# yijingru/KG_Instance_Segmentation

Measured on AMD Instinct MI355X. Metric: imgs/s (train fwd+bwd) at 512x512, higher is better.
Workload: dtype forward: f32-tolerance, hi + lo f16 planes (22 significant bits), 3 MFMA products / backward: f16 single planes, 1 MFMA product; f16 MFMA, fp32 accumulate; 1 GPU; KGnet train step fwd(dec+seg)+4xDetectionLossAll+SEG_loss+bwd+Adam, batch 8/GPU 3x512x512, 300 boxes/img, full HIP path; precision_policy=fp32, global_batch=8, parallelism=dp1, loss_readback=every step (train.py:156), grad_overflow=False

## Files before the change

### include/kgnet_hip.h

```cpp
#ifndef KGNET_HIP_H
#define KGNET_HIP_H
#ifdef __cplusplus
extern "C" {
#endif

typedef struct kg_planes {
    int a_planes, a_pstride;
    int b_planes, b_pstride;
    int c_planes, c_pstride;
    int y_planes, y_pstride;
    int w_planes;
    int reserved_;
    const float* scale;
    const float* oscale;
} kg_planes_t;

int kg_rows_format(void);

const char* kg_last_error(void);
const char* kg_last_kernel(void);
int kg_version(void);
int kg_device_arch(char* out, int cap);
int kg_tr_probe(void* out_u16x256, void* stream);
int kg_f64_probe(const double* a, const double* b, double* out5n, int n, void* stream);

int kg_conv2d_igemm(const void* x, const void* w, const float* bias, void* y, float* y_f32, const void* res,
                    const void* mask, const int* rowdesc, int M, int H, int W, int OH, int OW, int cin_pad, int ldx,
                    int Cout, int ldy, int ldres, int ldmask, int K, int KH, int KW, int stride, int pad, int dil,
                    int mode, int relu, int f32_C, int tile, const kg_planes_t* planes, void* stream);
int kg_conv2d_halo(const void* x, const void* w, const float* bias, void* y, float* y_f32, const void* res,
                   const void* mask, int N, int H, int W, int cin_pad, int ldx, int Cout, int ldy, int ldres, int ldmask,
                   int K, int KS, int flip, int relu, int f32_C, int wc, const int* tiletab, int ntiles, int total_rows,
                   const kg_planes_t* planes, void* stream);
int kg_conv2d_halo_heads2(const void* x, const void* w, const float* bias64, const int* vmap, float* kp, float* sh, float* md,
                          int N, int H, int W, int C, int ldx, int K, int kp_sigmoid, const kg_planes_t* planes, void* stream);
int kg_conv3x3_c64(const void* x, const void* w, const float* bias, void* y, const void* res, const void* mask, int N, int H, int W,
                   int ldx, int Cout, int ldy, int ldres, int ldmask, int K, int flip, int relu, const int* tiletab16, int ntiles,
                   void* stream);
int kg_conv7_narrow(const void* x, const void* w, void* y, const void* mask, int N, int H, int W, int ldx, int chan_lo, int chan_slot, int Cout, int ldy,
                    int ldmask, int K, int flip, void* stream);
int kg_conv3x3_ws(const void* x, const void* w, const float* bias, void* y, int N, int H, int W, int ldx, int ldy, int K, int relu,
                  const int* tiletab8, int ntiles, const kg_planes_t* planes, void* stream);
int kg_conv1x1(const void* x, const void* w, const float* bias, void* y, const void* res, const void* mask, long M, int K,
               int wK, int ldx, int Cout, int ldy, int ldres, int ldmask, int relu, void* stream);
int kg_pack_weight(const float* w, void* dst, int Cout, int Cin, int KH, int KW, int K, int cin_pad, int row0, int c0,
                   int transposed, int x_planes, int w_planes, void* stream);
int kg_pack_weight_rows(const float* w, void* dst, int Cout, int Cin, int KH, int KW, int K, int cin_pad, const int* rowmap,
                        int c0, int x_planes, int w_planes, int tap_stride, void* stream);
int kg_pack_weight_narrow(const float* w, void* dst, int Cout, int Cin, int KH, int KW, int K, int row0, int c0, int tap_stride, int tap_pitch,
                          void* stream);
int kg_pack_weight_batch(const void* jobs, int njobs, int total_blocks, void* stream);
int kg_im2col_small(const void* x, void* out, int N, int H, int W, int OH, int OW, int KH, int KW, int stride, int pad, int cin,
                    int ldx, int Kpad, void* stream);
int kg_conv2d_wgrad(const void* x, const void* dy, float* dwp, const int* rowdesc, int M, int H, int W, int OH, int OW,
                    int ldx, int lddy, int Cin, int Cout, int cin_lim, int cout_lim, int KH, int KW, int stride, int pad,
                    int dil, int mode, int nsplit, long split_stride, const kg_planes_t* planes, void* stream);
int kg_conv2d_wgrad_halo(const void* x, const void* dy, float* dwp, int N, int H, int W, int ldx, int lddy, int Cin, int Cout,
                         int cin_lim, int cout_lim, int KS, int nsplit, long split_stride, const int* tiletab16, int ntiles,
                         float* dbp, const kg_planes_t* planes, void* stream);
int kg_bias_grad_final(const float* part, float* db, int nsplit, int C, int accumulate, void* stream);
int kg_wgrad_reduce(const float* part, float* grad_oihw, int Cout, int Cin, int KH, int KW, int nsplit, long split_stride,
                    int accumulate, void* stream);
int kg_wgrad_reduce_multi(const float* part, float* const* grads_oihw, const int* counts, int ngrads, int Cin, int KH, int KW,
                          int nsplit, long split_stride, int accumulate, void* stream);
int kg_wgrad_reduce_bias(const float* part, float* const* grads_oihw, const int* counts, int ngrads, int Cin, int KH, int KW,
                         int nsplit, long split_stride, int accumulate, const float* bias_part, float* db, int bias_C, void* stream);
int kg_wgrad_reduce_defer(int on);
int kg_wgrad_reduce_pending(void);
int kg_wgrad_reduce_flush(void* stream);
int kg_bias_grad(const void* dy, float* db, float* scratch, int scratch_floats, int M, int C, int ld, int accumulate,
                 void* stream);
int kg_set_wgrad_tr(int use_transpose_read);

int kg_img_pack(const float* img_nchw, void* out_rows8, int ldout, int N, int C, int H, int W, const kg_planes_t* planes, void* stream);
int kg_bn_stats_train(const void* x, int ldx, int M, int C, const float* gamma, const float* beta, float* running_mean,
                      float* running_var, float momentum, float eps, float* mean_out, float* invstd_out, float* scale,
                      float* shift, float* scratch, int scratch_floats, const kg_planes_t* planes, void* stream);
int kg_conv_stats_begin(float* part, long cap_floats);
int kg_conv_stats_end(int* nb);
int kg_bn_finalize_train(const float* part, int nb, int M, int C, const float* gamma, const float* beta, float* running_mean,
                         float* running_var, float momentum, float eps, float* mean_out, float* invstd_out, float* scale,
                         float* shift, void* stream);
int kg_bn_scale_shift_eval(int C, const float* gamma, const float* beta, const float* running_mean,
                           const float* running_var, float eps, float* scale, float* shift, void* stream);
int kg_bn_apply(const void* x, int ldx, const float* scale, const float* shift, const void* res, int ldres, void* y,
                int ldy, int M, int C, int relu, const kg_planes_t* planes, void* stream);
int kg_bn_bwd(const void* x, int ldx, const void* dy, int lddy, const float* gamma, const float* mean,
              const float* invstd, float* dgamma, float* dbeta, int accumulate, void* dx, int lddx, int M, int C,
              float* scratch, int scratch_floats, const float* parts, int nb_parts, const float* parts_scale,
              const kg_planes_t* planes, void* stream);
int kg_conv_bstats_begin(float* part, long cap_floats, const void* x, int ldx, int x_planes, int x_pstride, const float* mean,
                         const float* invstd);
int kg_maxpool3s2_fwd(const void* x, int ldx, void* y, int ldy, void* argmax_u8, int N, int H, int W, int C, const kg_planes_t* planes, void* stream);
int kg_maxpool3s2_bwd(const void* x, int ldx, const void* dy, int lddy, void* dx, int lddx, const void* argmax_u8, int N, int H, int W, int C,
                      const kg_planes_t* planes, void* stream);
int kg_bilinear_fwd(const void* x, int ldx, void* y, int ldy, int N, int IH, int IW, int OH, int OW, int C,
                    const int* boxdesc, const int* row2box, long total_out_rows, const kg_planes_t* planes, void* stream);
int kg_bilinear_bwd(const void* dy, int lddy, void* dx, int lddx, int N, int IH, int IW, int OH, int OW, int C,
                    const int* boxdesc, const int* row2box, long total_in_rows, const void* mask, int ldmask,
                    const kg_planes_t* planes, void* stream);
int kg_add_rows(const void* a, int lda, const void* b, int ldb, const void* mask, int ldm, void* y, int ldy, long M,
                int C, const float* scale, const float* scale2, const kg_planes_t* planes, void* stream);
int kg_sigmoid_inplace(float* x, long n, void* stream);
int kg_grad_pack(const float* g_nchw, const float* prob, void* out_rows, int N, int C, int H, int W, int ld, int cpad,
                 const kg_planes_t* planes, void* stream);
int kg_grad_pack3(const float* g0_nchw, const float* g1_nchw, const float* g2_nchw, const float* prob0, void* out_rows, int N, int C0, int C1, int C2,
                  int H, int W, int ld, int pad0, int pad1, int pad2, const kg_planes_t* planes, void* stream);

int kg_detection_loss_fwd(const float* kp, const float* sh, const float* md, const float* gt, int N, int H, int W,
                          float kp_radius, const float* den_override, float* scratch, int scratch_floats, float* out8,
                          void* stream);
int kg_detection_loss_bwd(const float* kp, const float* sh, const float* md, const float* gt, int N, int H, int W,
                          float kp_radius, const float* fin8, const float* grad_out, float* g_kp, float* g_sh,
                          float* g_md, void* stream);
int kg_seg_loss(const float* prob, const void* tgt_u8, const int* patches, const void* pairs, int npatches, float* part,
                float* out1, const float* grad_out, float* gprob, void* stream);

int kg_postproc_timing_begin(void);
int kg_postproc_timing_end(float* ms4);
long kg_postproc_workspace_bytes(int H, int W, int peak_cap, int skel_cap);
int kg_postproc_scale(const float* kp, const float* soff, const float* mid, int H, int W, double thresh, void* ws,
                      long ws_bytes, int peak_cap, int skel_cap, double* skel, int* nskel, double* heat_out,
                      double* blur_out, int* peaks_out, double* peak_conf_out, int* npeaks_out, void* stream);
int kg_skeleton_boxes(const double* skel, const int* nskel, int skel_cap, double scale, int do_refine, double* boxes,
                      int* nbox, int box_cap, void* stream);
int kg_nms(const double* boxes, const int* nbox, int box_cap, double thresh, void* ws, long ws_bytes, double* out,
           int* nkeep, void* stream);

long kg_postproc_batch_workspace_bytes(int N, int H, int W, int peak_cap, int skel_cap);
int kg_postproc_batch(const float* kp, const float* soff, const float* mid, int N, int H, int W, double thresh, void* ws,
                      long ws_bytes, int peak_cap, int skel_cap, double* skel, int* nskel, void* stream);
int kg_skeleton_boxes_batch(int N, int nscales, const double* const* skel, const int* const* nskel, const int* skel_cap,
                            const double* scale, int do_refine, double* boxes, int* nbox, int box_cap, void* stream);
long kg_nms_batch_workspace_bytes(int N, int box_cap);
int kg_nms_batch(int N, const double* boxes, const int* nbox, int box_cap, double thresh, void* ws, long ws_bytes, double* out,
                 int* nkeep, void* stream);

int kg_gt_maps(const float* kps, int n, int H, int W, float* out, void* stream);

int kg_sp_image(const void* imgs, int N, int H, int W, float* out, void* stream);
int kg_sp_warp_masks(const void* imgs, const int* inst_img, int ntot, int H, int W, void* out, int* box, void* stream);
int kg_sp_boxes(const void* imgs, int N, const int* box, int ntot, int kp_radius, int* counts, float* gtb, float* kp, int* keep,
                void* stream);

int kg_adam_step(const void* jobs, int njobs, int total_blocks, float beta1, float beta2, float eps, float step_size, float bc2_sqrt,
                 float weight_decay, void* stream);

int kg_host_crop_masks(const float* const* masks, const int* work, int nwork, int H, int W, unsigned char* out);
int kg_crop_masks(const void* masks, const int* work, int nwork, int H, int W, void* out, void* stream);
int kg_host_tile_table(const int* h, const int* w, const long* row0, int nb, int th, int tw, int* out, int cap);
int kg_host_bin_csr(const int* tab, int nb, int BS, int BY, int BX, int nbins, int* bin_start, int* bin_boxes, int cap);
int kg_host_match_boxes(const float* pb, int P, const float* gb, int G, int gstride, float thresh, int* pairs, int cap, int* count);

int kg_mask_areas(const void* masks, int n, long ld, int* area, void* stream);
int kg_mask_inter_pairs(const void* a, const void* b, const int* pairs, int npairs, long ld, int* inter, void* stream);

long kg_mask_bits_ld(int H, int W);
int kg_mask_pack_bits(const void* masks, int src_is_f32, int n, int H, int W, void* words, long ld_words, void* stream);
int kg_mask_unpack_bits(const void* words, long ld_words, int n, int H, int W, void* out, int out_is_u8, void* stream);
int kg_bitmask_areas(const void* words, int n, long ld_words, int* area, void* stream);
int kg_bitmask_inter_pairs(const void* a, int na, const void* b, int nb, const int* pairs, int npairs, long ld_words, int* inter,
                           void* stream);

int kg_seg_build_rows(const int* boxtab8, int nb, int* rowdesc, int* row2box, int* srcrow, void* stream);
int kg_seg_build_rows_levels(int nlev, const int* const* boxtab8, const int* nb, int* const* rowdesc, int* const* row2box, int* const* srcrow,
                             void* stream);
int kg_rows_gather(const void* src, int ldsrc, const int* srcrow, void* dst, int lddst, long nrows, int C, void* stream);
int kg_rows_gather_planes(const void* src, int ldsrc, int src_pstride, const int* srcrow, void* dst, int lddst, int dst_pstride, long nrows, int C,
                          int P, void* stream);
int kg_seg_conv3_c1(const void* x, int ldx, int C, const float* w, const float* bias, const int* rowdesc, long M, float* y,
                    const kg_planes_t* planes, void* stream);
int kg_f32_to_bf16_rows(const float* acc, void* out, int C, long rows, int ldout, const void* addto, int ldadd,
                        void* stream);
int kg_rows_gather_f32(const float* src, int ldsrc, const int* srcrow, void* dst, int lddst, long nrows, int C,
                       const kg_planes_t* planes, void* stream);
int kg_planes_to_f32(const void* x, int ldx, float* out, int ldout, long rows, int C, const kg_planes_t* planes, void* stream);
int kg_f32_to_planes(const float* acc, int ldacc, void* out, int ldout, const void* addto, int ldadd, long rows, int C,
                     const kg_planes_t* planes, void* stream);
int kg_crop_grad_reduce(const void* ga, int lda, const void* gb, int ldb, long rows_a, const int* boxtab, const int* bin_start,
                        const int* bin_boxes, int bin_size, int N, int H, int W, int C, float* out, void* out_rows, int ldout,
                        const kg_planes_t* planes, void* stream);


int kg_mask_paste(const float* flat, const int* dets, int nd, int input_h, int input_w, int image_h, int image_w,
                  float seg_thresh, void* out, int out_is_u8, void* stream);
int kg_mask_paste_bits(const float* flat, const int* dets, int nd, int input_h, int input_w, int image_h, int image_w,
                       float seg_thresh, void* words, long ld_words, void* stream);

int kg_grad_scale(const void* const* ptrs, const void* const* probs, const long* counts, int n, int target_log2, void* scratch, float* out, void* stream);
int kg_scale_tensors(const void* jobs, int njobs, int total_blocks, int* nonfinite, void* stream);
int kg_rows_rescale(void* g, int ld, long M, int C, int target_log2, const float* cum_in, float* cum_out, float* r_out, void* scratch,
                    const kg_planes_t* planes, void* stream);
int kg_rows_scale(void* g, int ld, long M, int C, const float* r, const float* r2, const kg_planes_t* planes, void* stream);
int kg_rows_scale_multi(const long* desc, int n, const float* r, const float* r2, void* stream);

#ifdef __cplusplus
}
#endif
#endif
```

### kg_instance_segmentation_amd/_lib.py

```python
import ctypes
import os

_HERE = os.path.dirname(os.path.abspath(__file__))
LIB_PATH = os.environ.get("KG_LIB_PATH") or os.path.join(_HERE, "libkgnet_hip.so")
LIB_F16_PATH = os.environ.get("KG_LIB_F16_PATH") or os.path.join(os.path.dirname(LIB_PATH), "libkgnet_hip_f16.so")

c_int, c_long, c_float, c_double, c_void_p = ctypes.c_int, ctypes.c_long, ctypes.c_float, ctypes.c_double, ctypes.c_void_p
P = c_void_p

_SIGS = {
    "kg_version": [],
    "kg_rows_format": [],
    "kg_grad_scale": [P, P, P, c_int, c_int, P, P, P],
    "kg_scale_tensors": [P, c_int, c_int, P, P],
    "kg_rows_rescale": [P, c_int, c_long, c_int, c_int, P, P, P, P, P, P],
    "kg_rows_scale": [P, c_int, c_long, c_int, P, P, P, P],
    "kg_rows_scale_multi": [P, c_int, P, P, P],
    "kg_device_arch": [ctypes.c_char_p, c_int],
    "kg_tr_probe": [P, P],
    "kg_conv2d_igemm": [P, P, P, P, P, P, P, P] + [c_int] * 21 + [P, P],
    "kg_conv2d_halo": [P, P, P, P, P, P, P] + [c_int] * 15 + [P, c_int, c_int, P, P],
    "kg_conv1x1": [P, P, P, P, P, P, c_long] + [c_int] * 8 + [P],
    "kg_conv3x3_c64": [P, P, P, P, P, P] + [c_int] * 11 + [P, c_int, P],
    "kg_conv3x3_ws": [P, P, P, P] + [c_int] * 7 + [P, c_int, P, P],
    "kg_pack_weight": [P, P] + [c_int] * 11 + [P],
    "kg_pack_weight_rows": [P, P] + [c_int] * 6 + [P, c_int, c_int, c_int, c_int, P],
    "kg_pack_weight_batch": [P, c_int, c_int, P],
    "kg_pack_weight_narrow": [P, P] + [c_int] * 9 + [P],
    "kg_conv7_narrow": [P, P, P, P] + [c_int] * 11 + [P],
    "kg_im2col_small": [P, P] + [c_int] * 12 + [P],
    "kg_conv2d_halo_heads2": [P, P, P, P, P, P, P] + [c_int] * 7 + [P, P],
    "kg_set_wgrad_tr": [c_int],
    "kg_conv2d_wgrad": [P, P, P, P] + [c_int] * 18 + [c_long, P, P],
    "kg_conv2d_wgrad_halo": [P, P, P] + [c_int] * 11 + [c_long, P, c_int, P, P, P],
    "kg_bias_grad_final": [P, P, c_int, c_int, c_int, P],
    "kg_wgrad_reduce": [P, P, c_int, c_int, c_int, c_int, c_int, c_long, c_int, P],
    "kg_wgrad_reduce_multi": [P, P, P, c_int, c_int, c_int, c_int, c_int, c_long, c_int, P],
    "kg_wgrad_reduce_bias": [P, P, P, c_int, c_int, c_int, c_int, c_int, c_long, c_int, P, P, c_int, P],
    "kg_wgrad_reduce_defer": [c_int],
    "kg_wgrad_reduce_pending": [],
    "kg_wgrad_reduce_flush": [P],
    "kg_bias_grad": [P, P, P, c_int, c_int, c_int, c_int, c_int, P],
    "kg_img_pack": [P, P, c_int, c_int, c_int, c_int, c_int, P, P],
    "kg_bn_stats_train": [P, c_int, c_int, c_int, P, P, P, P, c_float, c_float, P, P, P, P, P, c_int, P, P],
    "kg_bn_scale_shift_eval": [c_int, P, P, P, P, c_float, P, P, P],
    "kg_conv_stats_begin": [P, c_long],
    "kg_conv_bstats_begin": [P, c_long, P, c_int, c_int, c_int, P, P],
    "kg_conv_stats_end": [P],
    "kg_bn_finalize_train": [P, c_int, c_int, c_int, P, P, P, P, c_float, c_float, P, P, P, P, P],
    "kg_bn_apply": [P, c_int, P, P, P, c_int, P, c_int, c_int, c_int, c_int, P, P],
    "kg_bn_bwd": [P, c_int, P, c_int, P, P, P, P, P, c_int, P, c_int, c_int, c_int, P, c_int, P, c_int, P, P, P],
    "kg_maxpool3s2_fwd": [P, c_int, P, c_int, P, c_int, c_int, c_int, c_int, P, P],
    "kg_maxpool3s2_bwd": [P, c_int, P, c_int, P, c_int, P, c_int, c_int, c_int, c_int, P, P],
    "kg_bilinear_fwd": [P, c_int, P, c_int, c_int, c_int, c_int, c_int, c_int, c_int, P, P, c_long, P, P],
    "kg_bilinear_bwd": [P, c_int, P, c_int, c_int, c_int, c_int, c_int, c_int, c_int, P, P, c_long, P, c_int, P, P],
    "kg_add_rows": [P, c_int, P, c_int, P, c_int, P, c_int, c_long, c_int, P, P, P, P],
    "kg_detection_loss_fwd": [P, P, P, P, c_int, c_int, c_int, c_float, P, P, c_int, P, P],
    "kg_detection_loss_bwd": [P, P, P, P, c_int, c_int, c_int, c_float, P, P, P, P, P, P],
    "kg_seg_loss": [P, P, P, P, c_int, P, P, P, P, P],
    "kg_sigmoid_inplace": [P, c_long, P],
    "kg_grad_pack": [P, P, P, c_int, c_int, c_int, c_int, c_int, c_int, P, P],
    "kg_grad_pack3": [P, P, P, P, P] + [c_int] * 10 + [P, P],
    "kg_postproc_workspace_bytes": [c_int, c_int, c_int, c_int],
    "kg_postproc_scale": [P, P, P, c_int, c_int, c_double, P, c_long, c_int, c_int, P, P, P, P, P, P, P, P],
    "kg_postproc_timing_begin": [],
    "kg_postproc_timing_end": [P],
    "kg_skeleton_boxes": [P, P, c_int, c_double, c_int, P, P, c_int, P],
    "kg_nms": [P, P, c_int, c_double, P, c_long, P, P, P],
    "kg_postproc_batch_workspace_bytes": [c_int, c_int, c_int, c_int, c_int],
    "kg_postproc_batch": [P, P, P, c_int, c_int, c_int, c_double, P, c_long, c_int, c_int, P, P, P],
    "kg_skeleton_boxes_batch": [c_int, c_int, P, P, P, P, c_int, P, P, c_int, P],
    "kg_nms_batch_workspace_bytes": [c_int, c_int],
    "kg_nms_batch": [c_int, P, P, c_int, c_double, P, c_long, P, P, P],
    "kg_gt_maps": [P, c_int, c_int, c_int, P, P],
    "kg_sp_image": [P, c_int, c_int, c_int, P, P],
    "kg_sp_warp_masks": [P, P, c_int, c_int, c_int, P, P, P],
    "kg_sp_boxes": [P, c_int, P, c_int, c_int, P, P, P, P, P],
    "kg_adam_step": [P, c_int, c_int, c_float, c_float, c_float, c_float, c_float, c_float, P],
    "kg_host_crop_masks": [P, P, c_int, c_int, c_int, P],
    "kg_crop_masks": [P, P, c_int, c_int, c_int, P, P],
    "kg_host_match_boxes": [P, c_int, P, c_int, c_int, c_float, P, c_int, P],
    "kg_host_tile_table": [P, P, P, c_int, c_int, c_int, P, c_int],
    "kg_host_bin_csr": [P, c_int, c_int, c_int, c_int, c_int, P, P, c_int],
    "kg_mask_areas": [P, c_int, c_long, P, P],
    "kg_mask_inter_pairs": [P, P, P, c_int, c_long, P, P],
    "kg_mask_bits_ld": [c_int, c_int],
    "kg_mask_pack_bits": [P, c_int, c_int, c_int, c_int, P, c_long, P],
    "kg_mask_unpack_bits": [P, c_long, c_int, c_int, c_int, P, c_int, P],
    "kg_bitmask_areas": [P, c_int, c_long, P, P],
    "kg_bitmask_inter_pairs": [P, c_int, P, c_int, P, c_int, c_long, P, P],
    "kg_f64_probe": [P, P, P, c_int, P],
    "kg_seg_build_rows": [P, c_int, P, P, P, P],
    "kg_seg_build_rows_levels": [c_int, P, P, P, P, P, P],
    "kg_rows_gather": [P, c_int, P, P, c_int, c_long, c_int, P],
    "kg_rows_gather_planes": [P, c_int, c_int, P, P, c_int, c_int, c_long, c_int, c_int, P],
    "kg_seg_conv3_c1": [P, c_int, c_int, P, P, P, c_long, P, P, P],
    "kg_f32_to_bf16_rows": [P, P, c_int, c_long, c_int, P, c_int, P],
    "kg_rows_gather_f32": [P, c_int, P, P, c_int, c_long, c_int, P, P],
    "kg_planes_to_f32": [P, c_int, P, c_int, c_long, c_int, P, P],
    "kg_f32_to_planes": [P, c_int, P, c_int, P, c_int, c_long, c_int, P, P],
    "kg_mask_paste": [P, P, c_int, c_int, c_int, c_int, c_int, c_float, P, c_int, P],
    "kg_mask_paste_bits": [P, P, c_int, c_int, c_int, c_int, c_int, c_float, P, c_long, P],
    "kg_crop_grad_reduce": [P, c_int, P, c_int, c_long, P, P, P, c_int, c_int, c_int, c_int, c_int, P, P, c_int, P, P],
}
_RESTYPE = {"kg_postproc_workspace_bytes": c_long, "kg_postproc_batch_workspace_bytes": c_long, "kg_nms_batch_workspace_bytes": c_long,
            "kg_mask_bits_ld": c_long}
SYMBOLS = tuple(_SIGS) + ("kg_last_error", "kg_last_kernel")

_lib = None
_lib_f16 = None


class KGLibraryError(RuntimeError):
    pass


def _open(path, must_have_all):
    if not os.path.exists(path):
        raise KGLibraryError(
            f"{path} is missing: build it with `python -m kg_instance_segmentation_amd.build` "
            "(hipcc --offload-arch=gfx950).  There is no CPU fallback for the KGnet hot path.")
    lib = ctypes.CDLL(path)
    lib.kg_last_error.restype = ctypes.c_char_p
    lib.kg_last_error.argtypes = []
    lib.kg_last_kernel.restype = ctypes.c_char_p
    lib.kg_last_kernel.argtypes = []
    for name, args in _SIGS.items():
        if must_have_all:
            fn = getattr(lib, name)
        else:
            fn = getattr(lib, name, None)
            if fn is None:
                continue
        fn.argtypes = args
        fn.restype = _RESTYPE.get(name, c_int)
    return lib


def load(fmt=0):
    global _lib, _lib_f16
    if fmt:
        if _lib_f16 is None:
            lib = _open(LIB_F16_PATH, False)
            if lib.kg_rows_format() != 1:
                raise KGLibraryError(f"{LIB_F16_PATH} is not the half-precision build (kg_rows_format() != 1)")
            _lib_f16 = lib
        return _lib_f16
    if _lib is None:
        _lib = _open(LIB_PATH, True)
    return _lib


def call(name, *args, fmt=0):
    lib = load(fmt)
    rc = getattr(lib, name)(*args)
    if rc != 0:
        raise KGLibraryError(f"{name} failed ({rc}): {lib.kg_last_error().decode()}")


def last_kernel(fmt=0):
    return load(fmt).kg_last_kernel().decode()


_RAW_STREAM = None


def stream_ptr():
    global _RAW_STREAM
    import torch
    if _RAW_STREAM is None:
        _RAW_STREAM = getattr(torch._C, "_cuda_getCurrentRawStream", False)
    if _RAW_STREAM:
        return c_void_p(_RAW_STREAM(torch.cuda.current_device()))
    return c_void_p(torch.cuda.current_stream().cuda_stream)


def ptr(t):
    return None if t is None else c_void_p(t.data_ptr())
```

### kg_instance_segmentation_amd/csrc/api.hip

```cpp
#include "kg_common.h"
#include <stdarg.h>

static thread_local char g_err[512] = "";

void kg_set_error(const char* fmt, ...) {
    va_list ap;
    va_start(ap, fmt);
    vsnprintf(g_err, sizeof(g_err), fmt, ap);
    va_end(ap);
}

extern "C" const char* kg_last_error(void) { return g_err; }

static thread_local const char* g_kernel = "";
void kg_note_kernel(const char* name) { g_kernel = name; }
extern "C" const char* kg_last_kernel(void) { return g_kernel; }
extern "C" int kg_version(void) { return 101; }
extern "C" int kg_rows_format(void) { return KG_ROWS_FORMAT; }

extern "C" int kg_device_arch(char* out, int cap) {
    hipDeviceProp_t p;
    int dev = 0;
    KG_HIP(hipGetDevice(&dev));
    KG_HIP(hipGetDeviceProperties(&p, dev));
    snprintf(out, cap, "%s", p.gcnArchName);
    return KG_OK;
}

typedef __attribute__((address_space(3))) bf16x4 lds_bf16x4;
__global__ void tr_probe_kernel(unsigned short* out) {
    __shared__ __attribute__((aligned(16))) unsigned short lds[64 * 4];
    const int l = threadIdx.x;
    for (int j = 0; j < 4; ++j) lds[l * 4 + j] = (unsigned short)(l * 4 + j);
    __syncthreads();
    bf16x4 v = KG_DS_READ_TR16((lds_bf16x4*)(&lds[l * 4]));
    *reinterpret_cast<uint2*>(&out[l * 4]) = __builtin_bit_cast(uint2, v);
}
extern "C" int kg_tr_probe(void* out, void* stream) {
    hipLaunchKernelGGL(tr_probe_kernel, dim3(1), dim3(64), 0, (hipStream_t)stream, (unsigned short*)out);
    KG_CHECK_LAUNCH("tr_probe");
    return KG_OK;
}

static thread_local KgConvStats g_conv_stats = {nullptr, 0, 0, {nullptr, 0, 0, 0, nullptr, nullptr}};
KgConvStats& kg_conv_stats() { return g_conv_stats; }
extern "C" int kg_conv_stats_begin(float* part, long cap_floats) {
    KG_CHECK_ARG(part && cap_floats > 0, "kg_conv_stats_begin: bad buffer");
    g_conv_stats = KgConvStats{part, cap_floats, 0, {nullptr, 0, 0, 0, nullptr, nullptr}};
    return KG_OK;
}
extern "C" int kg_conv_bstats_begin(float* part, long cap_floats, const void* x, int ldx, int x_planes, int x_pstride, const float* mean,
                                    const float* invstd) {
    KG_CHECK_ARG(part && cap_floats > 0 && x && mean && invstd && ldx % 8 == 0 && x_planes >= 1 && x_planes <= 3 && x_pstride % 8 == 0,
                 "kg_conv_bstats_begin: bad arguments");
    g_conv_stats = KgConvStats{part, cap_floats, 0, {(const unsigned short*)x, ldx, x_planes, x_pstride, mean, invstd}};
    return KG_OK;
}
extern "C" int kg_conv_stats_end(int* nb) {
    KG_CHECK_ARG(nb, "kg_conv_stats_end: null pointer");
    *nb = g_conv_stats.nb;
    g_conv_stats = KgConvStats{nullptr, 0, 0, {nullptr, 0, 0, 0, nullptr, nullptr}};
    return KG_OK;
}

extern "C" int kg_host_tile_table(const int* h, const int* w, const long* row0, int nb, int th, int tw, int* out, int cap) {
    if (!h || !w || !row0 || !out || nb < 0 || th < 1 || tw < 1) return -1;
    int n = 0;
    for (int b = 0; b < nb; ++b) {
        const int ny = (h[b] + th - 1) / th, nx = (w[b] + tw - 1) / tw;
        for (int ty = 0; ty < ny; ++ty)
            for (int tx = 0; tx < nx; ++tx) {
                if (n >= cap) return -1;
                int* o = out + 4 * (long)n++;
                o[0] = (int)row0[b]; o[1] = (h[b] << 16) | w[b]; o[2] = ((ty * th) << 16) | (tx * tw); o[3] = 0;
            }
    }
    return n;
}
extern "C" int kg_host_bin_csr(const int* tab, int nb, int BS, int BY, int BX, int nbins, int* bin_start, int* bin_boxes, int cap) {
    if (!tab || !bin_start || (!bin_boxes && cap > 0) || nb < 0 || BS < 1 || nbins < 0) return -1;
    for (int i = 0; i <= nbins; ++i) bin_start[i] = 0;
    long total = 0;
    for (int b = 0; b < nb; ++b) {
        const int* t = tab + 8 * (long)b;
        const int by0 = t[1] / BS, bx0 = t[2] / BS, by1 = (t[1] + t[3] - 1) / BS, bx1 = (t[2] + t[4] - 1) / BS;
        for (int by = by0; by <= by1; ++by)
            for (int bx = bx0; bx <= bx1; ++bx) {
                const long bin = ((long)t[0] * BY + by) * BX + bx;
                if (bin < 0 || bin >= nbins) return -1;
                ++bin_start[bin + 1]; ++total;
            }
    }
    if (total > cap) return -1;
    for (int i = 0; i < nbins; ++i) bin_start[i + 1] += bin_start[i];
    for (int b = 0; b < nb; ++b) {
        const int* t = tab + 8 * (long)b;
        const int by0 = t[1] / BS, bx0 = t[2] / BS, by1 = (t[1] + t[3] - 1) / BS, bx1 = (t[2] + t[4] - 1) / BS;
        for (int by = by0; by <= by1; ++by)
            for (int bx = bx0; bx <= bx1; ++bx) {
                const long bin = ((long)t[0] * BY + by) * BX + bx;
                bin_boxes[bin_start[bin]++] = b;
            }
    }
    for (int i = nbins; i > 0; --i) bin_start[i] = bin_start[i - 1];
    bin_start[0] = 0;
    return (int)total;
}

extern "C" int kg_host_match_boxes(const float* pb, int P, const float* gb, int G, int gstride, float thresh, int* pairs, int cap, int* count) {
#pragma clang fp contract(off)
    KG_CHECK_ARG(pb && gb && pairs && count && P >= 0 && G >= 0 && gstride >= 4 && cap >= 0, "kg_host_match_boxes: bad arguments");
    float* soa = (float*)malloc(sizeof(float) * 4 * (size_t)(G > 0 ? G : 1));
    unsigned char* ov = (unsigned char*)malloc((size_t)(G > 0 ? G : 1));
    if (!soa || !ov) { free(soa); free(ov); kg_set_error("kg_host_match_boxes: out of host memory"); return KG_ERR_ARG; }
    float *b0 = soa, *b1 = soa + G, *b2 = soa + 2 * (size_t)G, *b3 = soa + 3 * (size_t)G;
    for (int g = 0; g < G; ++g) {
        const float* b = gb + (long)g * gstride;
        b0[g] = b[0]; b1[g] = b[1]; b2[g] = b[2]; b3[g] = b[3];
    }
    const bool prefilter = thresh > 0.f;
    int n = 0, rc = KG_OK;
    for (int j = 0; j < P && rc == KG_OK; ++j) {
        const float a0 = pb[4 * j], a1 = pb[4 * j + 1], a2 = pb[4 * j + 2], a3 = pb[4 * j + 3];
        const float area_a = (a2 - a0) * (a3 - a1);
        for (int g = 0; g < G; ++g) {
            const float ih = (a2 < b2[g] ? a2 : b2[g]) - (a0 > b0[g] ? a0 : b0[g]);
            const float iw = (a3 < b3[g] ? a3 : b3[g]) - (a1 > b1[g] ? a1 : b1[g]);
            ov[g] = (unsigned char)((ih > 0.f) & (iw > 0.f));
        }
        for (int g = 0; g < G; ++g) {
            if (prefilter && !ov[g]) continue;
            const float area_b = (b2[g] - b0[g]) * (b3[g] - b1[g]);
            float ih = (a2 < b2[g] ? a2 : b2[g]) - (a0 > b0[g] ? a0 : b0[g]);
            float iw = (a3 < b3[g] ? a3 : b3[g]) - (a1 > b1[g] ? a1 : b1[g]);
            if (!(ih > 0.f)) ih = 0.f;
            if (!(iw > 0.f)) iw = 0.f;
            const float inter = ih * iw;
            const float uni = area_a + area_b - inter;
            const float iou = uni <= 2.f ? 0.f : inter / uni;
            if (iou >= thresh) {
                if (n >= cap) { kg_set_error("kg_host_match_boxes: more than %d matches", cap); rc = KG_ERR_ARG; break; }
                pairs[2 * n] = j; pairs[2 * n + 1] = g; ++n;
            }
        }
    }
    free(soa); free(ov);
    if (rc != KG_OK) return rc;
    *count = n;
    return KG_OK;
}

#include <math.h>
extern "C" int kg_host_crop_masks(const float* const* masks, const int* work, int nwork, int H, int W, unsigned char* out) {
    KG_CHECK_ARG(masks && work && out && nwork >= 0 && H > 0 && W > 0, "kg_host_crop_masks: bad arguments");
    for (int k = 0; k < nwork; ++k) {
        const int* w = work + 9 * k;
        const float* m = masks[w[0]] + (long)w[1] * H * W;
        int ya = w[2], yb = w[3], xa = w[4], xb = w[5];
        const int h1 = w[6], w1 = w[7];
        unsigned char* o = out + w[8];
        if (yb > H) yb = H;
        if (xb > W) xb = W;
        const int h0 = yb - ya, w0 = xb - xa;
        if (h0 <= 0 || w0 <= 0) { kg_set_error("kg_host_crop_masks: empty ground-truth crop (work item %d)", k); return KG_ERR_ARG; }
        const double fy = (double)h0 / h1, fx = (double)w0 / w1;
        for (int y = 0; y < h1; ++y) {
            int sy = y;
            if (h0 != h1 || w0 != w1) { sy = (int)floor(y * fy); if (sy > h0 - 1) sy = h0 - 1; }
            const float* row = m + (long)(ya + sy) * W + xa;
            for (int x = 0; x < w1; ++x) {
                int sx = x;
                if (h0 != h1 || w0 != w1) { sx = (int)floor(x * fx); if (sx > w0 - 1) sx = w0 - 1; }
                o[y * w1 + x] = (unsigned char)row[sx];
            }
        }
    }
    return KG_OK;
}
```

### kg_instance_segmentation_amd/csrc/kg_common.h

```cpp
#pragma once
#include <hip/hip_runtime.h>
#include <stdint.h>
#include <stdio.h>
#include <string.h>

typedef uint16_t bf16_t;
#ifdef KG_F16
typedef _Float16 kg_h16;
#define KG_MFMA16(a, b, c) __builtin_amdgcn_mfma_f32_16x16x32_f16(a, b, c, 0, 0, 0)
#define KG_WSCALE 4096.0f
#define KG_OSCALE (1.0f / 4096.0f)
#define KG_ACC(v) ((v) * KG_OSCALE)
#define KG_BIAS_ACC(b) ((b) * KG_WSCALE)
#define KG_ROWS_FORMAT 1
typedef __attribute__((ext_vector_type(4))) __fp16 kg_fp16x4_;
#define KG_DS_READ_TR16(p) __builtin_bit_cast(bf16x4_fwd_, __builtin_amdgcn_ds_read_tr16_b64_v4f16((__attribute__((address_space(3))) kg_fp16x4_*)(p)))
#else
typedef __bf16 kg_h16;
#define KG_MFMA16(a, b, c) __builtin_amdgcn_mfma_f32_16x16x32_bf16(a, b, c, 0, 0, 0)
#define KG_WSCALE 1.0f
#define KG_OSCALE 1.0f
#define KG_ACC(v) (v)
#define KG_BIAS_ACC(b) (b)
#define KG_ROWS_FORMAT 0
#define KG_DS_READ_TR16(p) __builtin_amdgcn_ds_read_tr16_b64_v4bf16(p)
#endif
typedef __attribute__((ext_vector_type(8))) kg_h16 bf16x8;
typedef __attribute__((ext_vector_type(4))) kg_h16 bf16x4;
typedef bf16x4 bf16x4_fwd_;
typedef __attribute__((ext_vector_type(4))) float f32x4;

#define KG_OK 0
#define KG_ERR_ARG 1
#define KG_ERR_HIP 2

void kg_set_error(const char* fmt, ...);
void kg_note_kernel(const char* name);
#define KG_KNAME(buf, fmt, ...) static char buf[96] = ""; if (!buf[0]) snprintf(buf, sizeof(buf), fmt, __VA_ARGS__)

struct KgPerDevice {
    bool done[32] = {};
    bool first() {
        int d = 0;
        if (hipGetDevice(&d) != hipSuccess || d < 0 || d >= 32) return true;
        if (done[d]) return false;
        done[d] = true;
        return true;
    }
};

#define KG_CHECK_ARG(cond, ...)                 \
    do {                                        \
        if (!(cond)) {                          \
            kg_set_error(__VA_ARGS__);          \
            return KG_ERR_ARG;                  \
        }                                       \
    } while (0)

#define KG_CHECK_LAUNCH(name)                                                        \
    do {                                                                             \
        hipError_t e_ = hipGetLastError();                                           \
        if (e_ != hipSuccess) {                                                      \
            kg_set_error("%s: launch failed: %s", name, hipGetErrorString(e_));      \
            return KG_ERR_HIP;                                                       \
        }                                                                            \
    } while (0)

#define KG_HIP(call)                                                                  \
    do {                                                                              \
        hipError_t e_ = (call);                                                       \
        if (e_ != hipSuccess) {                                                       \
            kg_set_error("%s failed: %s", #call, hipGetErrorString(e_));              \
            return KG_ERR_HIP;                                                        \
        }                                                                             \
    } while (0)

#ifdef KG_F16
__device__ __forceinline__ float bf2f(bf16_t v) { return (float)__builtin_bit_cast(_Float16, v); }
#else
__device__ __forceinline__ float bf2f(bf16_t v) { return __uint_as_float(((uint32_t)v) << 16); }
#endif
typedef __attribute__((ext_vector_type(2))) kg_h16 kg_bf16x2_t;
__device__ __forceinline__ bf16_t f2bf(float f) { return __builtin_bit_cast(bf16_t, (kg_h16)f); }
__device__ __forceinline__ uint32_t pack2bf(float lo, float hi) {
    const kg_bf16x2_t v = {(kg_h16)lo, (kg_h16)hi};
    return __builtin_bit_cast(uint32_t, v);
}

template <int OFF>
__device__ __forceinline__ void lds_rd128(bf16x8& d, unsigned addr) {
    asm volatile("ds_read_b128 %0, %1 offset:%2" : "=v"(d) : "v"(addr), "n"(OFF));
}
template <int N>
__device__ __forceinline__ void lgkm_wait(bf16x8 (&a)[4], bf16x8 (&b)[4]) {
    asm volatile("s_waitcnt lgkmcnt(%8)" : "+v"(a[0]), "+v"(a[1]), "+v"(a[2]), "+v"(a[3]), "+v"(b[0]), "+v"(b[1]), "+v"(b[2]), "+v"(b[3]) : "n"(N));
}

__device__ __forceinline__ float kg_relu(float v) { return v < 0.f ? 0.f : v; }

__device__ __forceinline__ unsigned lds_addr(const void* p) {
    return (unsigned)(unsigned long long)(__attribute__((address_space(3))) const unsigned char*)p;
}

static inline int kg_cdiv(long a, long b) { return (int)((a + b - 1) / b); }

__device__ __forceinline__ void kg_divmod(long i, int d, long* q, int* r) {
    if ((d & (d - 1)) == 0) {
        const int sh = __builtin_ctz((unsigned)d);
        *q = i >> sh; *r = (int)(i & (long)(d - 1));
    } else if ((unsigned long)i <= 0xffffffffUL) {
        const unsigned qi = (unsigned)i / (unsigned)d;
        *q = (long)qi; *r = (int)((unsigned)i - qi * (unsigned)d);
    } else {
        const long qq = i / d;
        *q = qq; *r = (int)(i - qq * d);
    }
}

struct KgBStat { const unsigned short* x; int ldx, P, ps; const float* mean; const float* invstd; };
struct KgConvStats { float* part; long cap_floats; int nb; KgBStat bs; };
KgConvStats& kg_conv_stats();
static inline float* kg_conv_stats_claim(int tiles, int Cout) {
    KgConvStats& st = kg_conv_stats();
    if (!st.part || st.nb != 0 || (long)tiles * Cout * 2 > st.cap_floats) return nullptr;
    st.nb = tiles;
    return st.part;
}

struct kg_planes_t {
    int a_planes, a_pstride;
    int b_planes, b_pstride;
    int c_planes, c_pstride;
    int y_planes, y_pstride;
    int w_planes;
    int reserved_;
    const float* scale;
    const float* oscale;
};
static inline kg_planes_t kg_planes_or_default(const kg_planes_t* p) {
    kg_planes_t d = {1, 0, 1, 0, 1, 0, 1, 0, 1, 0, nullptr, nullptr};
    if (p) {
        d = *p;
        if (d.a_planes < 1) d.a_planes = 1;
        if (d.b_planes < 1) d.b_planes = 1;
        if (d.c_planes < 1) d.c_planes = 1;
        if (d.y_planes < 1) d.y_planes = 1;
        if (d.w_planes < 1) d.w_planes = 1;
    }
    return d;
}
static inline bool kg_planes_ok(const kg_planes_t& d) {
    return d.a_planes <= 3 && d.b_planes <= 3 && d.c_planes <= 3 && d.y_planes <= 3 && d.w_planes <= 3 &&
           d.a_pstride % 8 == 0 && d.b_pstride % 8 == 0 && d.c_pstride % 8 == 0 && d.y_pstride % 8 == 0;
}

static inline int kg_plane_pairs(int xP, int wP, int* xi, int* wj) {
    const int T = xP > wP ? xP : wP;
    int n = 0;
    for (int sum = T - 1; sum >= 0; --sum)
        for (int j = wP - 1; j >= 0; --j) {
            const int i = sum - j;
            if (i >= 0 && i < xP) { xi[n] = i; wj[n] = j; ++n; }
        }
    return n;
}
struct KMap {
    int n;
    int total;
    int xps;
    int unit;
    unsigned xtab;
    __device__ __forceinline__ int xoff(int q) const {
        if (total == n) return q * unit;
        const int v = q / n;
        return (int)((xtab >> (2 * v)) & 3u) * xps + (q - v * n) * unit;
    }
};
static inline int kg_kmap_segs(int xP, int wP, int* s) {
    int xi[6], wj[6];
    (void)s;
    return kg_plane_pairs(xP, wP, xi, wj);
}
static inline KMap kg_make_kmap(int C, int unit, int xP, int xps, int wP) {
    int xi[6], wj[6];
    const int nv = kg_plane_pairs(xP, wP, xi, wj);
    KMap m;
    m.n = C / unit; m.unit = unit; m.xps = xps; m.total = nv * m.n; m.xtab = 0;
    for (int v = 0; v < nv; ++v) m.xtab |= (unsigned)xi[v] << (2 * v);
    return m;
}

struct WgPairs {
    int n;
    int xoff[6], doff[6];
};
static inline WgPairs kg_make_wgpairs(int xP, int xps, int dP, int dps) {
    WgPairs w;
    int xi[6], dj[6];
    w.n = kg_plane_pairs(xP < 1 ? 1 : xP, dP < 1 ? 1 : dP, xi, dj);
    for (int k = 0; k < 6; ++k) { w.xoff[k] = k < w.n ? xi[k] * xps : 0; w.doff[k] = k < w.n ? dj[k] * dps : 0; }
    return w;
}

template <int NV>
__device__ __forceinline__ void kg_store_planes(bf16_t* yp, int P, int ps, float (&v)[NV], bool vec) {
    static_assert(NV % 8 == 0, "stores are 16-byte chunks");
    for (int p = 0; p < P; ++p) {
        bf16_t h[NV];
#pragma unroll
        for (int e = 0; e < NV; ++e) h[e] = f2bf(v[e]);
        if (vec) {
#pragma unroll
            for (int q = 0; q < NV / 8; ++q) {
                uint4 o;
                o.x = (uint32_t)h[q * 8 + 0] | ((uint32_t)h[q * 8 + 1] << 16); o.y = (uint32_t)h[q * 8 + 2] | ((uint32_t)h[q * 8 + 3] << 16);
                o.z = (uint32_t)h[q * 8 + 4] | ((uint32_t)h[q * 8 + 5] << 16); o.w = (uint32_t)h[q * 8 + 6] | ((uint32_t)h[q * 8 + 7] << 16);
                *reinterpret_cast<uint4*>(yp + (long)p * ps + q * 8) = o;
            }
        } else {
#pragma unroll
            for (int e = 0; e < NV; ++e) yp[(long)p * ps + e] = h[e];
        }
        if (p + 1 < P) {
#pragma unroll
            for (int e = 0; e < NV; ++e) v[e] -= bf2f(h[e]);
        }
    }
}
template <int NV>
__device__ __forceinline__ void kg_store_planes_n(bf16_t* yp, int P, int ps, float (&v)[NV], int nvalid) {
    for (int p = 0; p < P; ++p) {
#pragma unroll
        for (int e = 0; e < NV; ++e) {
            const bf16_t h = f2bf(v[e]);
            if (e < nvalid) yp[(long)p * ps + e] = h;
            v[e] -= bf2f(h);
        }
    }
}
__device__ __forceinline__ void kg_load_planes8(const bf16_t* xp, int P, int ps, float (&v)[8]) {
    uint4 q = *reinterpret_cast<const uint4*>(xp + (long)(P - 1) * ps);
    const bf16_t* s = reinterpret_cast<const bf16_t*>(&q);
#pragma unroll
    for (int e = 0; e < 8; ++e) v[e] = bf2f(s[e]);
    for (int p = P - 2; p >= 0; --p) {
        q = *reinterpret_cast<const uint4*>(xp + (long)p * ps);
#pragma unroll
        for (int e = 0; e < 8; ++e) v[e] += bf2f(s[e]);
    }
}
__device__ __forceinline__ float kg_load_planes1(const bf16_t* xp, int P, int ps) {
    float v = bf2f(xp[(long)(P - 1) * ps]);
    for (int p = P - 2; p >= 0; --p) v += bf2f(xp[(long)p * ps]);
    return v;
}
```

### kg_instance_segmentation_amd/csrc/loss.hip

```cpp
#include "kg_common.h"

__constant__ int KG_MID_FROM[20] = {0, 0, 0, 0, 1, 1, 1, 2, 2, 3, 1, 2, 3, 4, 2, 3, 4, 3, 4, 4};

__device__ __forceinline__ float wave_sum(float v) {
#pragma unroll
    for (int o = 32; o > 0; o >>= 1) v += __shfl_down(v, o, 64);
    return v;
}

__device__ __forceinline__ float bce_elem(float p, float t) {
    float l1 = log1pf(-p); l1 = l1 > -100.f ? l1 : -100.f;
    float l0 = logf(p); l0 = l0 > -100.f ? l0 : -100.f;
    return (t - 1.f) * l1 - t * l0;
}
__device__ __forceinline__ float bce_grad(float p, float t) {
    float d = (1.f - p) * p;
    d = d > 1e-12f ? d : 1e-12f;
    return (p - t) / d;
}

__global__ __launch_bounds__(256) void det_loss_fwd_kernel(const float* __restrict__ kp, const float* __restrict__ sh,
                                                           const float* __restrict__ md, const float* __restrict__ gt,
                                                           int N, long HW, float inv_r, float* __restrict__ part) {
    float s[5] = {0.f, 0.f, 0.f, 0.f, 0.f};
    const long total = (long)N * HW;
    for (long i = blockIdx.x * (long)blockDim.x + threadIdx.x; i < total; i += (long)gridDim.x * blockDim.x) {
        long n = i / HW, p = i - n * HW;
        const float* g = gt + n * 55 * HW + p;
        float gk[5];
#pragma unroll
        for (int c = 0; c < 5; ++c) {
            gk[c] = g[c * HW];
            s[0] += bce_elem(kp[(n * 5 + c) * HW + p], gk[c]);
        }
#pragma unroll
        for (int c = 0; c < 10; ++c) {
            float m = gk[c >> 1];
            s[1] += fabsf(sh[(n * 10 + c) * HW + p] - g[(5 + c) * HW]) * inv_r * m;
            s[2] += m;
        }
#pragma unroll
        for (int c = 0; c < 40; ++c) {
            float m = gk[KG_MID_FROM[c >> 1]];
            s[3] += fabsf(md[(n * 40 + c) * HW + p] - g[(15 + c) * HW]) * inv_r * m;
            s[4] += m;
        }
    }
    __shared__ float red[4][5];
    const int lane = threadIdx.x & 63, wave = threadIdx.x >> 6;
#pragma unroll
    for (int k = 0; k < 5; ++k) {
        float v = wave_sum(s[k]);
        if (lane == 0) red[wave][k] = v;
    }
    __syncthreads();
    if (threadIdx.x < 5) part[blockIdx.x * 5 + threadIdx.x] = red[0][threadIdx.x] + red[1][threadIdx.x] + red[2][threadIdx.x] + red[3][threadIdx.x];
}
__global__ void det_loss_final_kernel(const float* __restrict__ part, int nb, double numel,
                                      const float* __restrict__ den_override, float* __restrict__ out) {
    if (blockIdx.x != 0) return;
    double s[5] = {0, 0, 0, 0, 0};
    for (int b = threadIdx.x; b < nb; b += 64)
        for (int k = 0; k < 5; ++k) s[k] += (double)part[b * 5 + k];
#pragma unroll
    for (int k = 0; k < 5; ++k)
#pragma unroll
        for (int o = 32; o > 0; o >>= 1) s[k] += __shfl_down(s[k], o, 64);
    if (threadIdx.x != 0) return;
    double m2 = s[2], m4 = s[4], ne = numel;
    if (den_override) { m2 = den_override[0]; m4 = den_override[1]; ne = den_override[2]; }
    float lkp = (float)(s[0] / ne);
    float lsh = (float)s[1] / ((float)m2 + 1e-10f);
    float lmd = (float)s[3] / ((float)m4 + 1e-10f);
    out[0] = lkp + lsh + 0.25f * lmd; out[1] = lkp; out[2] = lsh; out[3] = lmd;
    out[4] = (float)(1.0 / ne); out[5] = 1.f / ((float)m2 + 1e-10f); out[6] = 1.f / ((float)m4 + 1e-10f);
    out[7] = (float)m2;
}
__global__ __launch_bounds__(256) void det_loss_bwd_kernel(const float* __restrict__ kp, const float* __restrict__ sh,
                                                           const float* __restrict__ md, const float* __restrict__ gt,
                                                           int N, long HW, float inv_r, const float* __restrict__ fin,
                                                           const float* __restrict__ gout, float* __restrict__ g_kp,
                                                           float* __restrict__ g_sh, float* __restrict__ g_md) {
    const float go = gout ? gout[0] : 1.f;
    const float a_kp = go * fin[4], a_sh = go * fin[5] * inv_r, a_md = go * 0.25f * fin[6] * inv_r;
    const long total = (long)N * HW;
    for (long i = blockIdx.x * (long)blockDim.x + threadIdx.x; i < total; i += (long)gridDim.x * blockDim.x) {
        long n = i / HW, p = i - n * HW;
        const float* g = gt + n * 55 * HW + p;
        float gk[5];
#pragma unroll
        for (int c = 0; c < 5; ++c) {
            gk[c] = g[c * HW];
            long o = (n * 5 + c) * HW + p;
            g_kp[o] = bce_grad(kp[o], gk[c]) * a_kp;
        }
#pragma unroll
        for (int c = 0; c < 10; ++c) {
            long o = (n * 10 + c) * HW + p;
            float d = sh[o] - g[(5 + c) * HW];
            float sg = d > 0.f ? 1.f : (d < 0.f ? -1.f : 0.f);
            g_sh[o] = sg * gk[c >> 1] * a_sh;
        }
#pragma unroll
        for (int c = 0; c < 40; ++c) {
            long o = (n * 40 + c) * HW + p;
            float d = md[o] - g[(15 + c) * HW];
            float sg = d > 0.f ? 1.f : (d < 0.f ? -1.f : 0.f);
            g_md[o] = sg * gk[KG_MID_FROM[c >> 1]] * a_md;
        }
    }
}

extern "C" int kg_detection_loss_fwd(const float* kp, const float* sh, const float* md, const float* gt, int N, int H,
                                     int W, float kp_radius, const float* den_override, float* scratch,
                                     int scratch_floats, float* out8, void* stream) {
    KG_CHECK_ARG(kp && sh && md && gt && scratch && out8, "kg_detection_loss_fwd: null pointer");
    long total = (long)N * H * W;
    int nb = (int)((total + 255) / 256);
    if (nb > 1024) nb = 1024;
    if (nb > scratch_floats / 5) nb = scratch_floats / 5;
    KG_CHECK_ARG(nb >= 1, "kg_detection_loss_fwd: scratch too small");
    hipStream_t st = (hipStream_t)stream;
    hipLaunchKernelGGL(det_loss_fwd_kernel, dim3(nb), dim3(256), 0, st, kp, sh, md, gt, N, (long)H * W, 1.f / kp_radius, scratch);
    hipLaunchKernelGGL(det_loss_final_kernel, dim3(1), dim3(64), 0, st, scratch, nb, (double)total * 5.0, den_override, out8);
    KG_CHECK_LAUNCH("detection_loss_fwd");
    return KG_OK;
}
extern "C" int kg_detection_loss_bwd(const float* kp, const float* sh, const float* md, const float* gt, int N, int H,
                                     int W, float kp_radius, const float* fin8, const float* grad_out, float* g_kp,
                                     float* g_sh, float* g_md, void* stream) {
    KG_CHECK_ARG(kp && sh && md && gt && fin8 && g_kp && g_sh && g_md, "kg_detection_loss_bwd: null pointer");
    long total = (long)N * H * W;
    int nb = (int)((total + 255) / 256);
    if (nb > 4096) nb = 4096;
    hipLaunchKernelGGL(det_loss_bwd_kernel, dim3(nb), dim3(256), 0, (hipStream_t)stream, kp, sh, md, gt, N, (long)H * W,
                       1.f / kp_radius, fin8, grad_out, g_kp, g_sh, g_md);
    KG_CHECK_LAUNCH("detection_loss_bwd");
    return KG_OK;
}

struct SegPatch { int prob_off, npix, pair0, npairs; };
struct SegPair { int tgt_off; float weight; };
__global__ __launch_bounds__(256) void seg_loss_kernel(const float* __restrict__ prob, const uint8_t* __restrict__ tgt,
                                                       const SegPatch* __restrict__ patches,
                                                       const SegPair* __restrict__ pairs, float* __restrict__ part,
                                                       const float* __restrict__ gout, float* __restrict__ gprob) {
    const SegPatch pa = patches[blockIdx.x];
    const float go = gout ? gout[0] : 1.f;
    float s = 0.f;
    for (int i = threadIdx.x; i < pa.npix; i += blockDim.x) {
        float p = prob[pa.prob_off + i], g = 0.f;
        for (int k = 0; k < pa.npairs; ++k) {
            SegPair pr = pairs[pa.pair0 + k];
            float t = (float)tgt[pr.tgt_off + i];
            s += pr.weight * bce_elem(p, t);
            g += pr.weight * bce_grad(p, t);
        }
        if (gprob) gprob[pa.prob_off + i] = g * go;
    }
    __shared__ float red[4];
    float v = wave_sum(s);
    if ((threadIdx.x & 63) == 0) red[threadIdx.x >> 6] = v;
    __syncthreads();
    if (threadIdx.x == 0 && part) part[blockIdx.x] = red[0] + red[1] + red[2] + red[3];
}
__global__ void sum_final_kernel(const float* __restrict__ part, int n, float* __restrict__ out) {
    if (blockIdx.x != 0) return;
    double s = 0.;
    for (int i = threadIdx.x; i < n; i += 64) s += (double)part[i];
#pragma unroll
    for (int o = 32; o > 0; o >>= 1) s += __shfl_down(s, o, 64);
    if (threadIdx.x == 0) out[0] = (float)s;
}
extern "C" int kg_seg_loss(const float* prob, const void* tgt, const int* patches, const void* pairs, int npatches,
                           float* part, float* out1, const float* grad_out, float* gprob, void* stream) {
    KG_CHECK_ARG(prob && tgt && patches && pairs && npatches > 0, "kg_seg_loss: bad args");
    hipStream_t st = (hipStream_t)stream;
    hipLaunchKernelGGL(seg_loss_kernel, dim3(npatches), dim3(256), 0, st, prob, (const uint8_t*)tgt,
                       (const SegPatch*)patches, (const SegPair*)pairs, part, grad_out, gprob);
    if (part && out1) hipLaunchKernelGGL(sum_final_kernel, dim3(1), dim3(64), 0, st, part, npatches, out1);
    KG_CHECK_LAUNCH("seg_loss");
    return KG_OK;
}

__global__ void sigmoid_inplace_kernel(float* __restrict__ x, long n) {
    for (long i = blockIdx.x * (long)blockDim.x + threadIdx.x; i < n; i += (long)gridDim.x * blockDim.x)
        x[i] = 1.f / (1.f + expf(-x[i]));
}
extern "C" int kg_sigmoid_inplace(float* x, long n, void* stream) {
    KG_CHECK_ARG(x, "kg_sigmoid_inplace: null pointer");
    if (n == 0) return KG_OK;
    int blocks = (int)((n + 255) / 256); if (blocks > 8192) blocks = 8192;
    hipLaunchKernelGGL(sigmoid_inplace_kernel, dim3(blocks), dim3(256), 0, (hipStream_t)stream, x, n);
    KG_CHECK_LAUNCH("sigmoid_inplace");
    return KG_OK;
}
__global__ void grad_pack_kernel(const float* __restrict__ g, const float* __restrict__ prob, bf16_t* __restrict__ out,
                                 int N, int C, long HW, int ld, int cpad, int P, int ps, const float* __restrict__ scale) {
    long total = (long)N * HW;
    const float S = scale ? *scale : 1.f;
    for (long i = blockIdx.x * (long)blockDim.x + threadIdx.x; i < total; i += (long)gridDim.x * blockDim.x) {
        long n = i / HW, p = i - n * HW;
        for (int c0 = 0; c0 < cpad; c0 += 8) {
            float v[8];
#pragma unroll
            for (int e = 0; e < 8; ++e) {
                int c = c0 + e;
                float t = 0.f;
                if (c < C) {
                    long o = (n * C + c) * HW + p;
                    t = g[o];
                    if (prob) { float q = prob[o]; t *= q * (1.f - q); }
                }
                v[e] = t * S;
            }
            kg_store_planes<8>(out + i * ld + c0, P, ps, v, true);
        }
    }
}
__global__ __launch_bounds__(256) void grad_pack_tr_kernel(const float* __restrict__ g, const float* __restrict__ prob, bf16_t* __restrict__ out,
                                                           long total, int C, long HW, int ld, int cpad, int P, int ps, const float* __restrict__ scale) {
    extern __shared__ float gp_tile[];
    const float S = scale ? *scale : 1.f;
    const int t = threadIdx.x, K = cpad >> 3;
    for (long i0 = (long)blockIdx.x * 256; i0 < total; i0 += (long)gridDim.x * 256) {
        if ((HW & 3) == 0) {
            const int cs = t >> 6, pq = (t & 63) * 4;
            const long i = i0 + pq;
            if (i < total) {
                const long n = i / HW, p = i - n * HW;
#pragma unroll 2
                for (int c = cs; c < C; c += 4) {
                    const long o = (n * C + c) * HW + p;
                    f32x4 v = *reinterpret_cast<const f32x4*>(g + o);
                    if (prob) {
                        const f32x4 q = *reinterpret_cast<const f32x4*>(prob + o);
                        v[0] *= q[0] * (1.f - q[0]); v[1] *= q[1] * (1.f - q[1]); v[2] *= q[2] * (1.f - q[2]); v[3] *= q[3] * (1.f - q[3]);
                    }
#pragma unroll
                    for (int e = 0; e < 4; ++e) gp_tile[c * 257 + pq + e] = v[e] * S;
                }
            }
        } else {
            const long i = i0 + t;
            if (i < total) {
                const long n = i / HW, p = i - n * HW;
                for (int c = 0; c < C; ++c) {
                    const long o = (n * C + c) * HW + p;
                    float v = g[o];
                    if (prob) { const float q = prob[o]; v *= q * (1.f - q); }
                    gp_tile[c * 257 + t] = v * S;
                }
            }
        }
        for (int c = C; c < cpad; ++c) gp_tile[c * 257 + t] = 0.f;
        __syncthreads();
        for (int q = t; q < 256 * K; q += 256) {
            const int px = q / K, k8 = q - px * K;
            if (i0 + px < total) {
                float v[8];
#pragma unroll
                for (int e = 0; e < 8; ++e) v[e] = gp_tile[(k8 * 8 + e) * 257 + px];
                kg_store_planes<8>(out + (i0 + px) * ld + k8 * 8, P, ps, v, true);
            }
        }
        __syncthreads();
    }
}
struct GradPack3 { const float* g[3]; const float* prob; int C[3]; int off[3]; int end[3]; };
__global__ __launch_bounds__(256) void grad_pack3_tr_kernel(const GradPack3 a, bf16_t* __restrict__ out, long total, long HW, int ld, int cpad, int P, int ps,
                                                            const float* __restrict__ scale) {
    extern __shared__ float gp_tile[];
    const float S = scale ? *scale : 1.f;
    const int t = threadIdx.x, K = cpad >> 3;
    for (long i0 = (long)blockIdx.x * 256; i0 < total; i0 += (long)gridDim.x * 256) {
#pragma unroll
        for (int s = 0; s < 3; ++s) {
            for (int c = a.off[s] + a.C[s]; c < a.end[s]; ++c) gp_tile[c * 257 + t] = 0.f;
            const float* __restrict__ g = a.g[s];
            const float* __restrict__ prob = s == 0 ? a.prob : nullptr;
            const int C = a.C[s], r0 = a.off[s];
            if ((HW & 3) == 0) {
                const int cs = t >> 6, pq = (t & 63) * 4;
                const long i = i0 + pq;
                if (i < total) {
                    const long n = i / HW, p = i - n * HW;
#pragma unroll 2
                    for (int c = cs; c < C; c += 4) {
                        const long o = (n * C + c) * HW + p;
                        f32x4 v = *reinterpret_cast<const f32x4*>(g + o);
                        if (prob) {
                            const f32x4 q = *reinterpret_cast<const f32x4*>(prob + o);
                            v[0] *= q[0] * (1.f - q[0]); v[1] *= q[1] * (1.f - q[1]); v[2] *= q[2] * (1.f - q[2]); v[3] *= q[3] * (1.f - q[3]);
                        }
#pragma unroll
                        for (int e = 0; e < 4; ++e) gp_tile[(r0 + c) * 257 + pq + e] = v[e] * S;
                    }
                }
            } else {
                const long i = i0 + t;
                if (i < total) {
                    const long n = i / HW, p = i - n * HW;
                    for (int c = 0; c < C; ++c) {
                        const long o = (n * C + c) * HW + p;
                        float v = g[o];
                        if (prob) { const float q = prob[o]; v *= q * (1.f - q); }
                        gp_tile[(r0 + c) * 257 + t] = v * S;
                    }
                }
            }
        }
        __syncthreads();
        for (int q = t; q < 256 * K; q += 256) {
            const int px = q / K, k8 = q - px * K;
            if (i0 + px < total) {
                float v[8];
#pragma unroll
                for (int e = 0; e < 8; ++e) v[e] = gp_tile[(k8 * 8 + e) * 257 + px];
                kg_store_planes<8>(out + (i0 + px) * ld + k8 * 8, P, ps, v, true);
            }
        }
        __syncthreads();
    }
}
extern "C" int kg_grad_pack3(const float* g0, const float* g1, const float* g2, const float* prob0, void* out, int N, int C0, int C1, int C2, int H, int W,
                             int ld, int pad0, int pad1, int pad2, const kg_planes_t* planes, void* stream) {
    const int cpad = pad0 + pad1 + pad2;
    KG_CHECK_ARG(g0 && g1 && g2 && out && ld % 8 == 0 && pad0 % 8 == 0 && pad1 % 8 == 0 && pad2 % 8 == 0 && pad0 >= C0 && pad1 >= C1 && pad2 >= C2 &&
                 cpad <= 64 && C0 > 0 && C1 > 0 && C2 > 0, "kg_grad_pack3: bad args");
    const kg_planes_t pp = kg_planes_or_default(planes);
    KG_CHECK_ARG(kg_planes_ok(pp), "kg_grad_pack3: bad kg_planes_t");
    long total = (long)N * H * W;
    if (total == 0) return KG_OK;
    int blocks = (int)((total + 255) / 256); if (blocks > 2048) blocks = 2048;
    static KgPerDevice attr_done;
    if (attr_done.first()) {
        KG_HIP(hipFuncSetAttribute((const void*)grad_pack3_tr_kernel, hipFuncAttributeMaxDynamicSharedMemorySize, 64 * 257 * 4));
    }
    GradPack3 a;
    a.g[0] = g0; a.g[1] = g1; a.g[2] = g2; a.prob = prob0;
    a.C[0] = C0; a.C[1] = C1; a.C[2] = C2; a.off[0] = 0; a.off[1] = pad0; a.off[2] = pad0 + pad1;
    a.end[0] = pad0; a.end[1] = pad0 + pad1; a.end[2] = cpad;
    hipLaunchKernelGGL(grad_pack3_tr_kernel, dim3(blocks), dim3(256), cpad * 257 * 4, (hipStream_t)stream, a, (bf16_t*)out, total, (long)H * W, ld, cpad,
                       pp.y_planes, pp.y_pstride, pp.scale);
    KG_CHECK_LAUNCH("grad_pack3_tr");
    return KG_OK;
}
extern "C" int kg_grad_pack(const float* g, const float* prob, void* out, int N, int C, int H, int W, int ld, int cpad,
                            const kg_planes_t* planes, void* stream) {
    KG_CHECK_ARG(g && out && cpad % 8 == 0 && ld % 8 == 0 && cpad >= C, "kg_grad_pack: bad args");
    const kg_planes_t pp = kg_planes_or_default(planes);
    KG_CHECK_ARG(kg_planes_ok(pp), "kg_grad_pack: bad kg_planes_t");
    long total = (long)N * H * W;
    int blocks = (int)((total + 255) / 256); if (blocks > 8192) blocks = 8192;
    if (cpad <= 64) {
        const int smem = cpad * 257 * 4;
        static KgPerDevice attr_done;
        if (attr_done.first()) {
            KG_HIP(hipFuncSetAttribute((const void*)grad_pack_tr_kernel, hipFuncAttributeMaxDynamicSharedMemorySize, 64 * 257 * 4));
        }
        if (blocks > 2048) blocks = 2048;
        hipLaunchKernelGGL(grad_pack_tr_kernel, dim3(blocks), dim3(256), smem, (hipStream_t)stream, g, prob, (bf16_t*)out, total, C, (long)H * W, ld, cpad,
                           pp.y_planes, pp.y_pstride, pp.scale);
        KG_CHECK_LAUNCH("grad_pack_tr");
        return KG_OK;
    }
    hipLaunchKernelGGL(grad_pack_kernel, dim3(blocks), dim3(256), 0, (hipStream_t)stream, g, prob, (bf16_t*)out, N, C,
                       (long)H * W, ld, cpad, pp.y_planes, pp.y_pstride, pp.scale);
    KG_CHECK_LAUNCH("grad_pack");
    return KG_OK;
}
```

### kg_instance_segmentation_amd/csrc/norm_pool.hip

```cpp
#include "kg_common.h"

struct RowsR { const bf16_t* p; int ld, P, ps; };
struct RowsW { bf16_t* p; int ld, P, ps; };
__device__ __forceinline__ void rd8(const RowsR& t, long r, int c, float (&v)[8]) { kg_load_planes8(t.p + r * t.ld + c, t.P, t.ps, v); }
__device__ __forceinline__ void wr8(const RowsW& t, long r, int c, float (&v)[8]) { kg_store_planes<8>(t.p + r * t.ld + c, t.P, t.ps, v, true); }
#define KG_PLANES(pl)                                                       \
    const kg_planes_t pp = kg_planes_or_default(pl);                        \
    KG_CHECK_ARG(kg_planes_ok(pp), "bad kg_planes_t (at most 3 planes, strides multiples of 8)")

__global__ void img_pack_kernel(const float* __restrict__ img, RowsW out, int N, int C, int HW) {
    long total = (long)N * HW;
    for (long i = blockIdx.x * (long)blockDim.x + threadIdx.x; i < total; i += (long)gridDim.x * blockDim.x) {
        long n = i / HW, p = i - n * HW;
        float v[8];
#pragma unroll
        for (int c = 0; c < 8; ++c) v[c] = c < C ? img[(n * C + c) * HW + p] : 0.f;
        wr8(out, i, 0, v);
    }
}
extern "C" int kg_img_pack(const float* img, void* out, int ldout, int N, int C, int H, int W, const kg_planes_t* planes, void* stream) {
    KG_CHECK_ARG(img && out && C <= 8 && ldout >= 8 && ldout % 8 == 0, "kg_img_pack: bad args");
    KG_PLANES(planes);
    long total = (long)N * H * W;
    int blocks = (int)((total + 255) / 256); if (blocks > 8192) blocks = 8192;
    hipLaunchKernelGGL(img_pack_kernel, dim3(blocks), dim3(256), 0, (hipStream_t)stream, img, RowsW{(bf16_t*)out, ldout, pp.y_planes, pp.y_pstride}, N, C, H * W);
    KG_CHECK_LAUNCH("img_pack");
    return KG_OK;
}

template <int MODE>
__global__ __launch_bounds__(256) void colreduce_kernel(const RowsR x, const RowsR dy,
                                                        const float* __restrict__ mean,
                                                        const float* __restrict__ invstd, float* __restrict__ part,
                                                        int M, int C, int rows_per_block) {
    __shared__ float red[32][8][16];
    const int cl = threadIdx.x & 7, rl = threadIdx.x >> 3;
    const int c0 = blockIdx.y * 64 + cl * 8;
    float s0[8], s1[8];
#pragma unroll
    for (int e = 0; e < 8; ++e) s0[e] = s1[e] = 0.f;
    if (c0 < C) {
        float mu[8], is[8];
        if (MODE == 1) {
#pragma unroll
            for (int e = 0; e < 8; ++e) { mu[e] = mean[c0 + e]; is[e] = invstd[c0 + e]; }
        }
        int r0 = blockIdx.x * rows_per_block, r1 = r0 + rows_per_block;
        if (r1 > M) r1 = M;
        for (int r = r0 + rl; r < r1; r += 32) {
            float xs[8];
            rd8(x, r, c0, xs);
            if (MODE == 0) {
#pragma unroll
                for (int e = 0; e < 8; ++e) { float f = xs[e]; s0[e] += f; s1[e] += f * f; }
            } else {
                float ds[8];
                rd8(dy, r, c0, ds);
#pragma unroll
                for (int e = 0; e < 8; ++e) {
                    float d = ds[e], xh = (xs[e] - mu[e]) * is[e];
                    s0[e] += d; s1[e] += d * xh;
                }
            }
        }
    }
#pragma unroll
    for (int e = 0; e < 8; ++e) { red[rl][cl][e] = s0[e]; red[rl][cl][8 + e] = s1[e]; }
    __syncthreads();
    if (threadIdx.x < 128) {
        const int c = threadIdx.x & 63, q = threadIdx.x >> 6;
        float t = 0.f;
        for (int k = 0; k < 32; ++k) t += red[k][c >> 3][q * 8 + (c & 7)];
        const int cg = blockIdx.y * 64 + c;
        if (cg < C) part[((long)blockIdx.x * C + cg) * 2 + q] = t;
    }
}

__device__ __forceinline__ double wave_sum_d(double v) {
#pragma unroll
    for (int o = 32; o > 0; o >>= 1) v += __shfl_down(v, o, 64);
    return __shfl(v, 0, 64);
}

__global__ void bn_finalize_train_kernel(const float* __restrict__ part, int nb, int C, long M,
                                         const float* __restrict__ gamma, const float* __restrict__ beta,
                                         float* __restrict__ running_mean, float* __restrict__ running_var,
                                         float momentum, float eps, float* __restrict__ mean_out,
                                         float* __restrict__ invstd_out, float* __restrict__ scale,
                                         float* __restrict__ shift) {
    const int c = blockIdx.x;
    double s = 0., ss = 0.;
    for (int b = threadIdx.x; b < nb; b += 64) { s += part[((long)b * C + c) * 2]; ss += part[((long)b * C + c) * 2 + 1]; }
    s = wave_sum_d(s); ss = wave_sum_d(ss);
    if (threadIdx.x != 0) return;
    double mu = s / (double)M;
    double var = ss / (double)M - mu * mu;
    if (var < 0.) var = 0.;
    float is = (float)(1.0 / sqrt(var + (double)eps));
    mean_out[c] = (float)mu; invstd_out[c] = is;
    float sc = gamma[c] * is;
    scale[c] = sc; shift[c] = beta[c] - (float)mu * sc;
    if (running_mean) {
        double unb = M > 1 ? var * (double)M / (double)(M - 1) : var;
        running_mean[c] = (1.f - momentum) * running_mean[c] + momentum * (float)mu;
        running_var[c] = (1.f - momentum) * running_var[c] + momentum * (float)unb;
    }
}
__global__ void bn_finalize_eval_kernel(int C, const float* __restrict__ gamma, const float* __restrict__ beta,
                                        const float* __restrict__ running_mean,
                                        const float* __restrict__ running_var, float eps,
                                        float* __restrict__ scale, float* __restrict__ shift) {
    int c = blockIdx.x * blockDim.x + threadIdx.x;
    if (c >= C) return;
    float is = 1.f / sqrtf(running_var[c] + eps);
    float sc = gamma[c] * is;
    scale[c] = sc; shift[c] = beta[c] - running_mean[c] * sc;
}
__global__ void bn_finalize_bwd_kernel(const float* __restrict__ part, int nb, int C, long M,
                                       const float* __restrict__ gamma, const float* __restrict__ invstd,
                                       float* __restrict__ dgamma, float* __restrict__ dbeta, int accumulate,
                                       float* __restrict__ coef, const float* __restrict__ rs) {
    const int c = blockIdx.x;
    double s = 0., sx = 0.;
    for (int b = threadIdx.x; b < nb; b += 64) { s += part[((long)b * C + c) * 2]; sx += part[((long)b * C + c) * 2 + 1]; }
    s = wave_sum_d(s); sx = wave_sum_d(sx);
    if (threadIdx.x != 0) return;
    if (rs) { s *= (double)*rs; sx *= (double)*rs; }
    float db = (float)s, dg = (float)sx;
    dgamma[c] = accumulate ? dgamma[c] + dg : dg;
    dbeta[c] = accumulate ? dbeta[c] + db : db;
    float a = gamma[c] * invstd[c];
    coef[c] = a; coef[C + c] = (float)(-(double)a * sx / (double)M); coef[2 * C + c] = (float)(-(double)a * s / (double)M);
}

static int reduce_geometry(int M, int C, int scratch_floats, int* nb, int* rpb) {
    int n = scratch_floats / (2 * C);
    if (n > 512) n = 512;
    int need = (M + 255) / 256;
    if (n > need) n = need;
    if (n < 1) return 0;
    *rpb = (M + n - 1) / n;
    *nb = (M + *rpb - 1) / *rpb;
    return 1;
}

extern "C" int kg_bn_stats_train(const void* x, int ldx, int M, int C, const float* gamma, const float* beta,
                                 float* running_mean, float* running_var, float momentum, float eps,
                                 float* mean_out, float* invstd_out, float* scale, float* shift, float* scratch,
                                 int scratch_floats, const kg_planes_t* planes, void* stream) {
    KG_PLANES(planes);
    KG_CHECK_ARG(x && gamma && beta && mean_out && invstd_out && scale && shift && scratch, "kg_bn_stats_train: null pointer");
    KG_CHECK_ARG(C % 8 == 0 && ldx % 8 == 0, "kg_bn_stats_train: C/ld must be multiples of 8");
    int nb, rpb;
    KG_CHECK_ARG(reduce_geometry(M, C, scratch_floats, &nb, &rpb), "kg_bn_stats_train: scratch too small");
    hipStream_t st = (hipStream_t)stream;
    hipLaunchKernelGGL(colreduce_kernel<0>, dim3(nb, (C + 63) / 64), dim3(256), 0, st, RowsR{(const bf16_t*)x, ldx, pp.a_planes, pp.a_pstride},
                       RowsR{nullptr, 0, 1, 0}, (const float*)nullptr, (const float*)nullptr, scratch, M, C, rpb);
    hipLaunchKernelGGL(bn_finalize_train_kernel, dim3(C), dim3(64), 0, st, scratch, nb, C, (long)M, gamma,
                       beta, running_mean, running_var, momentum, eps, mean_out, invstd_out, scale, shift);
    KG_CHECK_LAUNCH("bn_stats_train");
    return KG_OK;
}
extern "C" int kg_bn_finalize_train(const float* part, int nb, int M, int C, const float* gamma, const float* beta, float* running_mean,
                                    float* running_var, float momentum, float eps, float* mean_out, float* invstd_out, float* scale,
                                    float* shift, void* stream) {
    KG_CHECK_ARG(part && gamma && beta && mean_out && invstd_out && scale && shift && nb >= 1 && M >= 1 && C >= 1, "kg_bn_finalize_train: bad arguments");
    hipLaunchKernelGGL(bn_finalize_train_kernel, dim3(C), dim3(64), 0, (hipStream_t)stream, part, nb, C, (long)M, gamma, beta, running_mean,
                       running_var, momentum, eps, mean_out, invstd_out, scale, shift);
    KG_CHECK_LAUNCH("bn_finalize_train");
    return KG_OK;
}
extern "C" int kg_bn_scale_shift_eval(int C, const float* gamma, const float* beta, const float* running_mean,
                                      const float* running_var, float eps, float* scale, float* shift, void* stream) {
    KG_CHECK_ARG(gamma && beta && running_mean && running_var && scale && shift, "kg_bn_scale_shift_eval: null pointer");
    hipLaunchKernelGGL(bn_finalize_eval_kernel, dim3((C + 127) / 128), dim3(128), 0, (hipStream_t)stream, C, gamma, beta,
                       running_mean, running_var, eps, scale, shift);
    KG_CHECK_LAUNCH("bn_scale_shift_eval");
    return KG_OK;
}

__global__ void bn_apply_kernel(const RowsR x, const float* __restrict__ scale,
                                const float* __restrict__ shift, const RowsR res,
                                const RowsW y, long M, int C8, int relu) {
    long total = M * C8;
    for (long i = blockIdx.x * (long)blockDim.x + threadIdx.x; i < total; i += (long)gridDim.x * blockDim.x) {
        long r; int c; kg_divmod(i, C8, &r, &c); c *= 8;
        float v[8];
        rd8(x, r, c, v);
#pragma unroll
        for (int e = 0; e < 8; ++e) v[e] = v[e] * scale[c + e] + shift[c + e];
        if (res.p) {
            float rs[8];
            rd8(res, r, c, rs);
#pragma unroll
            for (int e = 0; e < 8; ++e) v[e] += rs[e];
        }
        if (relu) {
#pragma unroll
            for (int e = 0; e < 8; ++e) v[e] = kg_relu(v[e]);
        }
        wr8(y, r, c, v);
    }
}
extern "C" int kg_bn_apply(const void* x, int ldx, const float* scale, const float* shift, const void* res, int ldres,
                           void* y, int ldy, int M, int C, int relu, const kg_planes_t* planes, void* stream) {
    KG_PLANES(planes);
    KG_CHECK_ARG(x && scale && shift && y, "kg_bn_apply: null pointer");
    KG_CHECK_ARG(C % 8 == 0 && ldx % 8 == 0 && ldy % 8 == 0 && (!res || ldres % 8 == 0), "kg_bn_apply: C/ld must be multiples of 8");
    long total = (long)M * (C / 8);
    int blocks = (int)((total + 255) / 256); if (blocks > 16384) blocks = 16384;
    hipLaunchKernelGGL(bn_apply_kernel, dim3(blocks), dim3(256), 0, (hipStream_t)stream, RowsR{(const bf16_t*)x, ldx, pp.a_planes, pp.a_pstride}, scale,
                       shift, RowsR{(const bf16_t*)res, ldres, pp.b_planes, pp.b_pstride}, RowsW{(bf16_t*)y, ldy, pp.y_planes, pp.y_pstride}, (long)M, C / 8, relu);
    KG_CHECK_LAUNCH("bn_apply");
    return KG_OK;
}

__global__ void bn_bwd_apply_kernel(const RowsR x, const RowsR dy,
                                    const float* __restrict__ mean, const float* __restrict__ invstd,
                                    const float* __restrict__ coef, const RowsW dx, long M, int C) {
    const int C8 = C / 8;
    long total = M * C8;
    for (long i = blockIdx.x * (long)blockDim.x + threadIdx.x; i < total; i += (long)gridDim.x * blockDim.x) {
        long r; int c; kg_divmod(i, C8, &r, &c); c *= 8;
        float xs[8], ds[8], v[8];
        rd8(x, r, c, xs); rd8(dy, r, c, ds);
#pragma unroll
        for (int e = 0; e < 8; ++e) {
            float xh = (xs[e] - mean[c + e]) * invstd[c + e];
            v[e] = coef[c + e] * ds[e] + coef[C + c + e] * xh + coef[2 * C + c + e];
        }
        wr8(dx, r, c, v);
    }
}
extern "C" int kg_bn_bwd(const void* x, int ldx, const void* dy, int lddy, const float* gamma, const float* mean,
                         const float* invstd, float* dgamma, float* dbeta, int accumulate, void* dx, int lddx, int M,
                         int C, float* scratch, int scratch_floats, const float* parts, int nb_parts, const float* parts_scale,
                         const kg_planes_t* planes, void* stream) {
    KG_PLANES(planes);
    const RowsR xr{(const bf16_t*)x, ldx, pp.a_planes, pp.a_pstride}, dyr{(const bf16_t*)dy, lddy, pp.b_planes, pp.b_pstride};
    KG_CHECK_ARG(x && dy && gamma && mean && invstd && dgamma && dbeta && dx && scratch, "kg_bn_bwd: null pointer");
    KG_CHECK_ARG(C % 8 == 0 && ldx % 8 == 0 && lddy % 8 == 0 && lddx % 8 == 0, "kg_bn_bwd: C/ld must be multiples of 8");
    int nb, rpb;
    hipStream_t st = (hipStream_t)stream;
    float* coef = scratch;
    if (parts && nb_parts > 0) {
        KG_CHECK_ARG(scratch_floats >= 3 * C, "kg_bn_bwd: scratch too small");
        hipLaunchKernelGGL(bn_finalize_bwd_kernel, dim3(C), dim3(64), 0, st, parts, nb_parts, C, (long)M, gamma, invstd, dgamma, dbeta, accumulate, coef,
                           parts_scale);
    } else {
        KG_CHECK_ARG(reduce_geometry(M, C, scratch_floats - 3 * C, &nb, &rpb), "kg_bn_bwd: scratch too small");
        float* part = scratch + 3 * C;
        hipLaunchKernelGGL(colreduce_kernel<1>, dim3(nb, (C + 63) / 64), dim3(256), 0, st, xr, dyr, mean, invstd, part, M, C, rpb);
        hipLaunchKernelGGL(bn_finalize_bwd_kernel, dim3(C), dim3(64), 0, st, part, nb, C, (long)M, gamma,
                           invstd, dgamma, dbeta, accumulate, coef, (const float*)nullptr);
    }
    long total = (long)M * (C / 8);
    int blocks = (int)((total + 255) / 256); if (blocks > 16384) blocks = 16384;
    hipLaunchKernelGGL(bn_bwd_apply_kernel, dim3(blocks), dim3(256), 0, st, xr, dyr,
                       mean, invstd, coef, RowsW{(bf16_t*)dx, lddx, pp.y_planes, pp.y_pstride}, (long)M, C);
    KG_CHECK_LAUNCH("bn_bwd");
    return KG_OK;
}

__device__ __forceinline__ void pool_window_max(const RowsR& x, long nbase, int H, int W,
                                                int oy, int ox, int c, float* best, int* arg) {
#pragma unroll
    for (int e = 0; e < 8; ++e) { best[e] = -INFINITY; arg[e] = -1; }
    for (int kh = 0; kh < 3; ++kh) {
        int iy = oy * 2 - 1 + kh;
        if ((unsigned)iy >= (unsigned)H) continue;
        for (int kw = 0; kw < 3; ++kw) {
            int ix = ox * 2 - 1 + kw;
            if ((unsigned)ix >= (unsigned)W) continue;
            float s[8];
            rd8(x, nbase + (long)iy * W + ix, c, s);
#pragma unroll
            for (int e = 0; e < 8; ++e) {
                float f = s[e];
                if (f > best[e] || arg[e] < 0) { best[e] = f; arg[e] = kh * 3 + kw; }
            }
        }
    }
}
__global__ void maxpool_fwd_kernel(const RowsR x, const RowsW y, unsigned char* __restrict__ argout, int N, int H,
                                   int W, int OH, int OW, int C8) {
    long total = (long)N * OH * OW * C8;
    for (long i = blockIdx.x * (long)blockDim.x + threadIdx.x; i < total; i += (long)gridDim.x * blockDim.x) {
        long p; int c; kg_divmod(i, C8, &p, &c); c *= 8;
        int ox, oy; long q, n; kg_divmod(p, OW, &q, &ox); kg_divmod(q, OH, &n, &oy);
        float best[8]; int arg[8];
        pool_window_max(x, n * H * W, H, W, oy, ox, c, best, arg);
        wr8(y, p, c, best);
        if (argout) {
            uint2 pk;
            pk.x = (unsigned)arg[0] | ((unsigned)arg[1] << 8) | ((unsigned)arg[2] << 16) | ((unsigned)arg[3] << 24);
            pk.y = (unsigned)arg[4] | ((unsigned)arg[5] << 8) | ((unsigned)arg[6] << 16) | ((unsigned)arg[7] << 24);
            *reinterpret_cast<uint2*>(argout + p * (long)(C8 * 8) + c) = pk;
        }
    }
}
__global__ void maxpool_bwd_kernel(const RowsR x, const RowsR dy, const unsigned char* __restrict__ argin,
                                   const RowsW dx, int N, int H, int W, int OH, int OW, int C8) {
    long total = (long)N * H * W * C8;
    for (long i = blockIdx.x * (long)blockDim.x + threadIdx.x; i < total; i += (long)gridDim.x * blockDim.x) {
        long p; int c; kg_divmod(i, C8, &p, &c); c *= 8;
        int ix, iy; long q, n; kg_divmod(p, W, &q, &ix); kg_divmod(q, H, &n, &iy);
        float g[8];
#pragma unroll
        for (int e = 0; e < 8; ++e) g[e] = 0.f;
        for (int oy = (iy) / 2; oy <= (iy + 1) / 2; ++oy) {
            if (oy >= OH) continue;
            int kh = iy - (oy * 2 - 1);
            if (kh < 0 || kh > 2) continue;
            for (int ox = (ix) / 2; ox <= (ix + 1) / 2; ++ox) {
                if (ox >= OW) continue;
                int kw = ix - (ox * 2 - 1);
                if (kw < 0 || kw > 2) continue;
                float best[8]; int arg[8];
                if (argin) {
                    const uint2 pk = *reinterpret_cast<const uint2*>(argin + ((n * OH + oy) * OW + ox) * (long)(C8 * 8) + c);
#pragma unroll
                    for (int e = 0; e < 4; ++e) { arg[e] = (pk.x >> (8 * e)) & 255; arg[4 + e] = (pk.y >> (8 * e)) & 255; }
                } else
                    pool_window_max(x, n * H * W, H, W, oy, ox, c, best, arg);
                float ds[8];
                rd8(dy, (n * OH + oy) * OW + ox, c, ds);
#pragma unroll
                for (int e = 0; e < 8; ++e)
                    if (arg[e] == kh * 3 + kw) g[e] += ds[e];
            }
        }
        wr8(dx, p, c, g);
    }
}
extern "C" int kg_maxpool3s2_fwd(const void* x, int ldx, void* y, int ldy, void* argmax, int N, int H, int W, int C, const kg_planes_t* planes, void* stream) {
    KG_CHECK_ARG(x && y && C % 8 == 0 && ldx % 8 == 0 && ldy % 8 == 0, "kg_maxpool3s2_fwd: bad args");
    KG_PLANES(planes);
    int OH = (H + 2 - 3) / 2 + 1, OW = (W + 2 - 3) / 2 + 1;
    long total = (long)N * OH * OW * (C / 8);
    int blocks = (int)((total + 255) / 256); if (blocks > 16384) blocks = 16384;
    hipLaunchKernelGGL(maxpool_fwd_kernel, dim3(blocks), dim3(256), 0, (hipStream_t)stream, RowsR{(const bf16_t*)x, ldx, pp.a_planes, pp.a_pstride},
                       RowsW{(bf16_t*)y, ldy, pp.y_planes, pp.y_pstride}, (unsigned char*)argmax, N, H, W, OH, OW, C / 8);
    KG_CHECK_LAUNCH("maxpool_fwd");
    return KG_OK;
}
extern "C" int kg_maxpool3s2_bwd(const void* x, int ldx, const void* dy, int lddy, void* dx, int lddx, const void* argmax, int N, int H,
                                 int W, int C, const kg_planes_t* planes, void* stream) {
    KG_CHECK_ARG(x && dy && dx && C % 8 == 0 && ldx % 8 == 0 && lddy % 8 == 0 && lddx % 8 == 0, "kg_maxpool3s2_bwd: bad args");
    KG_PLANES(planes);
    int OH = (H + 2 - 3) / 2 + 1, OW = (W + 2 - 3) / 2 + 1;
    long total = (long)N * H * W * (C / 8);
    int blocks = (int)((total + 255) / 256); if (blocks > 16384) blocks = 16384;
    hipLaunchKernelGGL(maxpool_bwd_kernel, dim3(blocks), dim3(256), 0, (hipStream_t)stream, RowsR{(const bf16_t*)x, ldx, pp.a_planes, pp.a_pstride},
                       RowsR{(const bf16_t*)dy, lddy, pp.b_planes, pp.b_pstride}, (const unsigned char*)argmax, RowsW{(bf16_t*)dx, lddx, pp.y_planes, pp.y_pstride}, N, H, W, OH, OW, C / 8);
    KG_CHECK_LAUNCH("maxpool_bwd");
    return KG_OK;
}

__device__ __forceinline__ void bil_src(int dst, float scale, int in, int* i0, int* i1, float* l1) {
    float s = scale * ((float)dst + 0.5f) - 0.5f;
    if (s < 0.f) s = 0.f;
    int a = (int)s;
    if (a > in - 1) a = in - 1;
    *i0 = a; *i1 = a + (a < in - 1 ? 1 : 0); *l1 = s - (float)a;
}
__device__ __forceinline__ float bil_mix(float w00, float w01, float w10, float w11, float a, float b, float d, float e) {
    return __builtin_fmaf(w11, e, __builtin_fmaf(w10, d, __builtin_fmaf(w01, b, w00 * a)));
}
struct BilBox { int in_row0, ih, iw, out_row0, oh, ow; };
__global__ void bilinear_fwd_kernel(const RowsR x, const RowsW y, int IH,
                                    int IW, int OH, int OW, int C8, long total_rows, const BilBox* __restrict__ desc,
                                    const int* __restrict__ row2box) {
    long total = total_rows * C8;
    for (long i = blockIdx.x * (long)blockDim.x + threadIdx.x; i < total; i += (long)gridDim.x * blockDim.x) {
        long p; int c; kg_divmod(i, C8, &p, &c); c *= 8;
        long in0; int ih, iw, oh, ow, oy, ox;
        if (desc) {
            BilBox b = desc[row2box[p]];
            int loc = (int)(p - b.out_row0);
            ih = b.ih; iw = b.iw; oh = b.oh; ow = b.ow; oy = loc / ow; ox = loc - oy * ow; in0 = b.in_row0;
        } else {
            ih = IH; iw = IW; oh = OH; ow = OW;
            long q, nimg; kg_divmod(p, OW, &q, &ox); kg_divmod(q, OH, &nimg, &oy); in0 = nimg * IH * IW;
        }
        int y0, y1, x0, x1; float ly, lx;
        bil_src(oy, (float)ih / (float)oh, ih, &y0, &y1, &ly);
        bil_src(ox, (float)iw / (float)ow, iw, &x0, &x1, &lx);
        float w00 = (1.f - ly) * (1.f - lx), w01 = (1.f - ly) * lx, w10 = ly * (1.f - lx), w11 = ly * lx;
        float pa[8], pb[8], pd[8], pe[8];
        rd8(x, in0 + (long)y0 * iw + x0, c, pa); rd8(x, in0 + (long)y0 * iw + x1, c, pb);
        rd8(x, in0 + (long)y1 * iw + x0, c, pd); rd8(x, in0 + (long)y1 * iw + x1, c, pe);
        float v[8];
#pragma unroll
        for (int e = 0; e < 8; ++e) v[e] = bil_mix(w00, w01, w10, w11, pa[e], pb[e], pd[e], pe[e]);
        wr8(y, p, c, v);
    }
}
constexpr int BIL2_ROWS = 8;
__global__ __launch_bounds__(256) void bilinear2x_fwd_kernel(const RowsR x, const RowsW y, int N, int IH, int IW, int C8) {
    const long per_img = (long)IW * C8;
    const int strips = (IH + BIL2_ROWS - 1) / BIL2_ROWS;
    const long total = (long)N * strips * per_img;
    const int OH = 2 * IH, OW = 2 * IW;
    for (long t = blockIdx.x * (long)blockDim.x + threadIdx.x; t < total; t += (long)gridDim.x * blockDim.x) {
        long q; int c; kg_divmod(t, C8, &q, &c); c *= 8;
        int j; long q2; kg_divmod(q, IW, &q2, &j);
        int strip; long n; kg_divmod(q2, strips, &n, &strip);
        const int i0 = strip * BIL2_ROWS, i1 = i0 + BIL2_ROWS < IH ? i0 + BIL2_ROWS : IH;
        const long in0 = n * IH * IW, out0 = n * OH * OW;
        const int jl = j > 0 ? j - 1 : 0, jr = j < IW - 1 ? j + 1 : IW - 1;
        const float lx0 = j == 0 ? 0.f : 0.75f;
        float prev[3][8], cur[3][8], next[3][8];
        {
            const long bp = in0 + (long)(i0 > 0 ? i0 - 1 : 0) * IW, bc = in0 + (long)i0 * IW;
            rd8(x, bp + jl, c, prev[0]); rd8(x, bp + j, c, prev[1]); rd8(x, bp + jr, c, prev[2]);
            rd8(x, bc + jl, c, cur[0]); rd8(x, bc + j, c, cur[1]); rd8(x, bc + jr, c, cur[2]);
        }
        auto mix = [&](const float (&pa)[8], const float (&pb)[8], const float (&pd)[8], const float (&pe)[8], float ly, float lx, long orow) {
            const float w00 = (1.f - ly) * (1.f - lx), w01 = (1.f - ly) * lx, w10 = ly * (1.f - lx), w11 = ly * lx;
            float v[8];
#pragma unroll
            for (int e = 0; e < 8; ++e) v[e] = bil_mix(w00, w01, w10, w11, pa[e], pb[e], pd[e], pe[e]);
            wr8(y, orow, c, v);
        };
        for (int i = i0; i < i1; ++i) {
            const long bn = in0 + (long)(i < IH - 1 ? i + 1 : IH - 1) * IW;
            rd8(x, bn + jl, c, next[0]); rd8(x, bn + j, c, next[1]); rd8(x, bn + jr, c, next[2]);
            const float ly0 = i == 0 ? 0.f : 0.75f;
            const long o0 = out0 + (long)(2 * i) * OW + 2 * j, o1 = o0 + OW;
            mix(prev[0], prev[1], cur[0], cur[1], ly0, lx0, o0);
            mix(prev[1], prev[2], cur[1], cur[2], ly0, 0.25f, o0 + 1);
            mix(cur[0], cur[1], next[0], next[1], 0.25f, lx0, o1);
            mix(cur[1], cur[2], next[1], next[2], 0.25f, 0.25f, o1 + 1);
#pragma unroll
            for (int k = 0; k < 3; ++k)
#pragma unroll
                for (int e = 0; e < 8; ++e) { prev[k][e] = cur[k][e]; cur[k][e] = next[k][e]; }
        }
    }
}
__device__ __forceinline__ void bil_cand(int i, float scale, int out, int* lo, int* hi) {
    float a = ((float)i - 0.5f) / scale - 0.5f, b = ((float)i + 1.5f) / scale - 0.5f;
    int l = (int)floorf(a) - 1, h = (int)ceilf(b) + 1;
    *lo = l < 0 ? 0 : l; *hi = h > out - 1 ? out - 1 : h;
}
__global__ void bilinear_bwd_kernel(const RowsR dy, const RowsW dx, int IH,
                                    int IW, int OH, int OW, int C8, long total_rows, const BilBox* __restrict__ desc,
                                    const int* __restrict__ row2box, const bf16_t* __restrict__ mask, int ldmask) {
    long total = total_rows * C8;
    for (long i = blockIdx.x * (long)blockDim.x + threadIdx.x; i < total; i += (long)gridDim.x * blockDim.x) {
        long p; int c; kg_divmod(i, C8, &p, &c); c *= 8;
        long out0; int ih, iw, oh, ow, iy, ix;
        if (desc) {
            BilBox b = desc[row2box[p]];
            int loc = (int)(p - b.in_row0);
            ih = b.ih; iw = b.iw; oh = b.oh; ow = b.ow; iy = loc / iw; ix = loc - iy * iw; out0 = b.out_row0;
        } else {
            ih = IH; iw = IW; oh = OH; ow = OW;
            long q, nimg; kg_divmod(p, IW, &q, &ix); kg_divmod(q, IH, &nimg, &iy); out0 = nimg * OH * OW;
        }
        const float sy = (float)ih / (float)oh, sx = (float)iw / (float)ow;
        int ylo, yhi, xlo, xhi;
        bil_cand(iy, sy, oh, &ylo, &yhi); bil_cand(ix, sx, ow, &xlo, &xhi);
        float g[8];
#pragma unroll
        for (int e = 0; e < 8; ++e) g[e] = 0.f;
        for (int oy = ylo; oy <= yhi; ++oy) {
            int y0, y1; float ly;
            bil_src(oy, sy, ih, &y0, &y1, &ly);
            float wy = (y0 == iy ? 1.f - ly : 0.f) + (y1 == iy ? ly : 0.f);
            if (y0 != iy && y1 != iy) continue;
            for (int ox = xlo; ox <= xhi; ++ox) {
                int x0, x1; float lx;
                bil_src(ox, sx, iw, &x0, &x1, &lx);
                if (x0 != ix && x1 != ix) continue;
                float wx = (x0 == ix ? 1.f - lx : 0.f) + (x1 == ix ? lx : 0.f);
                float w = wy * wx;
                float ds[8];
                rd8(dy, out0 + (long)oy * ow + ox, c, ds);
#pragma unroll
                for (int e = 0; e < 8; ++e) g[e] += w * ds[e];
            }
        }
        if (mask) {
            const uint4 mv = *reinterpret_cast<const uint4*>(mask + p * ldmask + c);
            const bf16_t* ms = reinterpret_cast<const bf16_t*>(&mv);
#pragma unroll
            for (int e = 0; e < 8; ++e) g[e] = bf2f(ms[e]) > 0.f ? g[e] : 0.f;
        }
        wr8(dx, p, c, g);
    }
}
extern "C" int kg_bilinear_fwd(const void* x, int ldx, void* y, int ldy, int N, int IH, int IW, int OH, int OW, int C,
                               const int* boxdesc, const int* row2box, long total_out_rows, const kg_planes_t* planes, void* stream) {
    KG_CHECK_ARG(x && y && C % 8 == 0 && ldx % 8 == 0 && ldy % 8 == 0, "kg_bilinear_fwd: bad args");
    KG_PLANES(planes);
    long rows = boxdesc ? total_out_rows : (long)N * OH * OW;
    if (rows == 0) return KG_OK;
    long total = rows * (C / 8);
    static const int fast2x = getenv("KG_BILINEAR_2X") ? atoi(getenv("KG_BILINEAR_2X")) : 1;
    if (fast2x && !boxdesc && OH == 2 * IH && OW == 2 * IW && IH >= 2 && IW >= 2) {
        const long threads = (long)N * ((IH + BIL2_ROWS - 1) / BIL2_ROWS) * IW * (C / 8);
        int blocks2 = (int)((threads + 255) / 256); if (blocks2 > 65536) blocks2 = 65536;
        hipLaunchKernelGGL(bilinear2x_fwd_kernel, dim3(blocks2), dim3(256), 0, (hipStream_t)stream, RowsR{(const bf16_t*)x, ldx, pp.a_planes, pp.a_pstride},
                           RowsW{(bf16_t*)y, ldy, pp.y_planes, pp.y_pstride}, N, IH, IW, C / 8);
        KG_CHECK_LAUNCH("bilinear2x_fwd");
        return KG_OK;
    }
    int blocks = (int)((total + 255) / 256); if (blocks > 16384) blocks = 16384;
    hipLaunchKernelGGL(bilinear_fwd_kernel, dim3(blocks), dim3(256), 0, (hipStream_t)stream, RowsR{(const bf16_t*)x, ldx, pp.a_planes, pp.a_pstride},
                       RowsW{(bf16_t*)y, ldy, pp.y_planes, pp.y_pstride}, IH, IW, OH, OW, C / 8, rows, (const BilBox*)boxdesc, row2box);
    KG_CHECK_LAUNCH("bilinear_fwd");
    return KG_OK;
}
extern "C" int kg_bilinear_bwd(const void* dy, int lddy, void* dx, int lddx, int N, int IH, int IW, int OH, int OW, int C,
                               const int* boxdesc, const int* row2box, long total_in_rows, const void* mask, int ldmask,
                               const kg_planes_t* planes, void* stream) {
    KG_CHECK_ARG(dy && dx && C % 8 == 0 && lddy % 8 == 0 && lddx % 8 == 0 && (!mask || ldmask % 8 == 0), "kg_bilinear_bwd: bad args");
    KG_PLANES(planes);
    long rows = boxdesc ? total_in_rows : (long)N * IH * IW;
    if (rows == 0) return KG_OK;
    long total = rows * (C / 8);
    int blocks = (int)((total + 255) / 256); if (blocks > 16384) blocks = 16384;
    hipLaunchKernelGGL(bilinear_bwd_kernel, dim3(blocks), dim3(256), 0, (hipStream_t)stream, RowsR{(const bf16_t*)dy, lddy, pp.a_planes, pp.a_pstride},
                       RowsW{(bf16_t*)dx, lddx, pp.y_planes, pp.y_pstride}, IH, IW, OH, OW, C / 8, rows, (const BilBox*)boxdesc, row2box, (const bf16_t*)mask, ldmask);
    KG_CHECK_LAUNCH("bilinear_bwd");
    return KG_OK;
}

__global__ void add_rows_kernel(const RowsR a, const RowsR b,
                                const bf16_t* __restrict__ m, int ldm, const RowsW y, long M, int C8, const float* __restrict__ sc,
                                const float* __restrict__ sc2) {
    long total = M * C8;
    const float s = sc ? *sc * (sc2 ? *sc2 : 1.f) : 1.f;
    for (long i = blockIdx.x * (long)blockDim.x + threadIdx.x; i < total; i += (long)gridDim.x * blockDim.x) {
        long r; int c; kg_divmod(i, C8, &r, &c); c *= 8;
        float v[8];
        rd8(a, r, c, v);
        if (b.p) {
            float bs[8];
            rd8(b, r, c, bs);
#pragma unroll
            for (int e = 0; e < 8; ++e) v[e] += bs[e];
        }
        if (s != 1.f) {
#pragma unroll
            for (int e = 0; e < 8; ++e) v[e] *= s;
        }
        if (m) {
            uint4 mv = *reinterpret_cast<const uint4*>(m + r * ldm + c);
            const bf16_t* ms = (const bf16_t*)&mv;
#pragma unroll
            for (int e = 0; e < 8; ++e) v[e] = bf2f(ms[e]) > 0.f ? v[e] : 0.f;
        }
        wr8(y, r, c, v);
    }
}
// ... 154 lines not shown
```

### kg_instance_segmentation_amd/engine.py

```python
import os

import torch

from . import arch, ops
from .ops import BF16, PT, PackedWeight

PRECISIONS = {
    "fp32": (2, 2, 2, 2, 1),
    "fp32b2": (2, 2, 2, 2, 2),
    "half": (1, 1, 1, 1, 1),
    "halfmix": (2, 1, 1, 1, 1),
    "fp32bf": (3, 3, 3, 3, 2),
    "fp32bf_full": (3, 3, 3, 3, 3),
    "fp32bf_w1d1": (3, 3, 3, 3, 2, 1, 1),
    "fp32bf_b1": (3, 3, 3, 3, 1),
    "trunk2": (2, 2, 1, 1, 1), "mixed": (2, 1, 1, 1, 1), "bf16": (1, 1, 1, 1, 1),
}
HALF_POLICIES = ("fp32", "fp32b2", "half", "halfmix")
DEFAULT_PRECISION = "fp32"
PRE = [0]
NARROW_HEADS_DGRAD = int(os.environ.get("KG_NARROW_HEADS_DGRAD", "2"))
BN_BWD_STATS = True


# ... 190 lines not shown
            v = self.grad_store.get(key)
            if v is not None:
                ops.flush_wgrad()
                v.copy_(g)
                return v
        return g

    def spec(self, key, cin, cout, k, stride=1, pad=0, bias=True, fused=None, P=None, gP=None):
        P = self.bpt if P is None else P
        s = self.specs.get((key, P))
        if s is None:
            names = fused if fused else [key]
            couts = [cout] * len(names) if fused else [cout]
            s = ConvSpec(names, cin, couts, k, stride, pad, bias, P, min(P, self.pg) if gP is None else gP)
            self.specs[(key, P)] = s
        return s

    def prepare_all(self, train):
        ops.PACKQ.defer = True
        try:
            mode = self.m.training
            for s in self.specs.values():
                if s.used and mode in s.modes:
                    self.prepare(s, need_T=train and s.need_T_last)
            for lvl, (C, dev) in self.heads2_seen.items():
                self.prepare_heads2(lvl, C, dev, train)
        finally:
            ops.PACKQ.defer = False

    def prepack(self):
        if not self.m.training or not self.specs:
            return
        PRE[0] += 1
        stamp = ("p", PRE[0], 0)
        saved, self.stamp = self.stamp, stamp
        seg = self.m._seg
        seg_saved, seg.stamp = seg.stamp, stamp
        self.fast_stamp = seg.fast_stamp = None
        try:
            self.prepare_all(True)
            seg.prepare_all(True)
            ops.flush_packs(hold=True)
        finally:
            self.stamp, seg.stamp = saved, seg_saved
        self.prepack_state = {"epoch": ops.PARAM_EPOCH[0], "stamp": stamp, "fp": self.fingerprint()}

    def fingerprint(self):
        ts = [self.m.get_tensor(k) for k in self.m._param_keys]
        return tuple(t._version for t in ts), tuple(t.data_ptr() for t in ts)

    def prepare(self, s, need_T):
        s.used, s.need_T_last = True, need_T
        s.modes.add(self.m.training)
        if (self.fast_stamp is not None and s.versions is not None and s.versions[:3] == self.fast_stamp
                and (not need_T or (s.pwT is not None and not getattr(s.pwT, "stale", True)))):
            return
        ws = [self.P(n + ".weight") for n in s.names]
        ver = self.stamp + tuple(w._version for w in ws) + tuple(w.data_ptr() for w in ws)
        dev = ws[0].device
        taps = s.k * s.k
        if s.pw is None or s.versions != ver or s.pw.buf.device != dev:
            if s.pw is None or s.pw.buf.device != dev:
                s.pw = PackedWeight(s.cout, taps, s.cin_pad, dev, xP=s.P, wP=s.P, dtype=self.dt)
                s.pw.cin_real = s.cin
                s.pwT = None
            r = 0
            for w, co in zip(ws, s.couts):
                s.pw.pack(w.detach(), row0=r)
                r += co
            if s.has_bias:
                bs = [self.P(n + ".bias").detach() for n in s.names]
                s.bias_cat = bs[0] if len(bs) == 1 else torch.cat(bs)
            s.versions = ver
            if s.pwT is not None:
                s.pwT.stale = True
        if need_T and (s.pwT is None or getattr(s.pwT, "stale", True)):
            if s.pwT is None:
                s.pwT = PackedWeight(s.cin, taps, ops.round_up(s.cout, 8), dev, xP=s.gP, wP=min(s.P, s.gP, self.pdw), dtype=self.dt)
                s.pwT.cin_real = s.cout
            r = 0
            for w, co in zip(ws, s.couts):
                s.pwT.pack(w.detach(), c0=r, transposed=True)
                r += co
            s.pwT.stale = False

    def conv(self, xv, s, N, H, W, relu, out=None, y_f32=None, tile=0, oP=None, bn_stats=False, affine=None, res=None):
        train = self.tape is not None
        assert not (train and (affine is not None or res is not None))
        xv.uses += 1
        self.prepare(s, need_T=train and xv.req)
        OH = (H + 2 * s.pad - s.k) // s.stride + 1
        OW = (W + 2 * s.pad - s.k) // s.stride + 1
        M = N * OH * OW
        dev = xv.t.device
        oP = s.P if oP is None else oP
        if y_f32 is None and out is None:
            out = ops.alloc_pt(M, s.cout, oP, dev, dtype=self.dt)
        geom = (M, H, W, OH, OW, s.k, s.k, s.stride, s.pad)
        xin = trunc(xv.t, s.P)
        arm = bn_stats and ops.CONV_BN_STATS and self.m.training and y_f32 is None and not relu
        part = ops.conv_stats_begin(dev, self.fmt) if arm else None
        nb = 0
        try:
            if affine is not None:
                assert not s.has_bias
                ops.conv_auto(xin, s.pw, s.cout, geom, N, y=out, bias=affine[1], oscale=affine[0], res=res.t if res is not None else None, relu=relu, tile=tile)
            else:
                ops.conv_auto(xin, s.pw, s.cout, geom, N, y=out, y_f32=y_f32, bias=s.bias_cat if s.has_bias else None, relu=relu, tile=tile, tiny=not arm)
        finally:
            if arm:
                nb = ops.conv_stats_end(self.fmt)
        yv = Var(out, s.cout, relu=relu, gP=s.gP)
        if arm:
            yv.bn_part = (part, nb) if nb > 0 else None
        if train:
            def bwd():
                g = yv.take_grad()
                if g is None:
                    return
                if yv.boundary:
                    self.renormalise(g, yv.C)
                g = trunc(g, s.gP)
                grads, off = [], 0
                for n, co in zip(s.names, s.couts):
                    w = self.P(n + ".weight")
                    gw = self.new_grad(n + ".weight", w)
                    self.param_grads[n + ".weight"] = gw
                    grads.append((gw, off, co))
                    off += co
                db = torch.empty(s.cout, dtype=torch.float32, device=dev) if s.has_bias else None
                ops.conv_wgrad(trunc(xin, min(s.gP, self.pw)), trunc(g, self.pw), s.cin, s.cout, geom, grads, N=N, bias_out=db)
                if s.has_bias:
                    off = 0
                    for n, co in zip(s.names, s.couts):
                        self.param_grads[n + ".bias"] = self.place_grad(n + ".bias", db[off:off + co])
                        off += co
                if xv.req:
                    existing = xv.grad if xv.parent is None else None
                    if existing is not None:
                        xv.to_current_scale()
                    dx = existing if existing is not None else xv.alloc_grad()
                    gin = (N * H * W, OH, OW, H, W, s.k, s.k, s.stride, s.pad)
                    arm = (BN_BWD_STATS and xv.bn_in is not None and xv.parent is None and xv.pending is None and xv.ngot == xv.uses - 1
                           and (existing is not None or xv.uses == 1) and s.cin % 64 == 0)
                    part = ops.conv_bstats_begin(xv.bn_in[0], xv.bn_in[1], xv.bn_in[2], N * H * W, s.cin, N) if arm else None
                    try:
                        ops.conv_auto(g, s.pwT, s.cin, gin, N, y=dx, res=existing, mask=xv.t.hi() if xv.relu else None, transposed=True, tiny=not arm)
                    finally:
                        if arm:
                            nb = ops.conv_stats_end(self.fmt)
                            xv.bstat = (part, nb) if nb > 0 else None
                    if existing is None:
                        xv.add_grad(dx, masked=xv.relu)
                    else:
                        xv.ngot += 1
                        xv.masked = xv.masked or xv.relu
            self.tape.append(bwd)
        return yv, OH, OW

    def bn_eval_affine(self, p, C):
        gamma, beta = self.P(p + ".weight"), self.P(p + ".bias")
        rm, rv = self.P(p + ".running_mean"), self.P(p + ".running_var")
        ver = self.stamp + tuple(t._version for t in (gamma, beta, rm, rv)) + tuple(t.data_ptr() for t in (gamma, beta, rm, rv))
        hit = self.bn_eval.get(p)
        if hit is None or hit[0] != ver:
            hit = (ver, ops.bn_scale_shift_eval(C, gamma.detach(), beta.detach(), rm, rv))
            self.bn_eval[p] = hit
        return hit[1]

    def conv_bn(self, xv, s, bnp, N, H, W, relu, res=None, out=None, bn_stats=True):
        if self.tape is None and not self.m.training and self.fuse_eval_bn:
            if out is None:
                OH, OW = (H + 2 * s.pad - s.k) // s.stride + 1, (W + 2 * s.pad - s.k) // s.stride + 1
                out = ops.alloc_pt(N * OH * OW, s.cout, self.bpt, xv.t.device, dtype=self.dt)
            yv, OH, OW = self.conv(xv, s, N, H, W, relu, out=out, affine=self.bn_eval_affine(bnp, s.cout), res=res)
            yv.gP = min(self.bpt, self.pg)
            return yv, OH, OW
        y, OH, OW = self.conv(xv, s, N, H, W, False, bn_stats=bn_stats)
        return self.bn(y, bnp, relu, res=res, out=out), OH, OW

    def bn(self, xv, p, relu, res=None, out=None):
        C = xv.C
        dev = xv.t.device
        gamma, beta = self.P(p + ".weight"), self.P(p + ".bias")
        rm, rv = self.P(p + ".running_mean"), self.P(p + ".running_var")
        if out is None:
            out = ops.alloc_pt(xv.rows, C, self.bpt, dev, dtype=self.dt)
        if self.m.training:
            bp = getattr(xv, "bn_part", None)
            if bp is not None:
                mean, invstd, scale, shift = ops.bn_finalize_train(bp[0], bp[1], xv.rows, C, gamma.detach(), beta.detach(), rm, rv)
                xv.bn_part = None
            else:
                mean, invstd, scale, shift = ops.bn_stats_train(xv.t, C, gamma.detach(), beta.detach(), rm, rv)
            self.nbt.append(self.P(p + ".num_batches_tracked"))
            self.stats_written = True
        else:
            scale, shift = self.bn_eval_affine(p, C)
            mean = invstd = None
        ops.bn_apply(xv.t, C, scale, shift, out, res=res.t if res is not None else None, relu=relu)
        yv = Var(out, C, relu=relu, gP=min(self.bpt, self.pg))
        xv.uses += 1
        if res is not None:
            res.uses += 1
        if self.tape is not None:
            if mean is None:
                raise NotImplementedError("backward through eval-mode BatchNorm is not supported; call model.train()")
            yv.bn_in = (xv.t, mean, invstd)

            def bwd():
                bst, yv.bstat = yv.bstat, None
                if bst is not None and (yv.pending is not None or (yv.relu and not (yv.masked and yv.pmasked))
                                        or (self.gscale is not None and yv.gsc is not None and yv.gsc is not self.gscale)):
                    bst = None
                g = yv.take_grad()
                if g is None:
                    return
                r = self.renormalise(g, yv.C) if yv.boundary else None
                dg = self.new_grad(p + ".weight", gamma)
                db = self.new_grad(p + ".bias", beta)
                dx = ops.alloc_pt(xv.rows, C, xv.gP, dev, dtype=self.dt)
                ops.bn_bwd(xv.t, g, C, gamma.detach(), mean, invstd, dg, db, dx, parts=bst, parts_scale=r if bst is not None else None)
                self.param_grads[p + ".weight"] = dg
                self.param_grads[p + ".bias"] = db
                xv.add_grad(dx, masked=True)
                if res is not None:
                    res.add_grad(g, masked=False)
            self.tape.append(bwd)
        return yv

    def maxpool(self, xv, N, H, W):
        C = xv.C
        OH, OW = (H - 1) // 2 + 1, (W - 1) // 2 + 1
        out = ops.alloc_pt(N * OH * OW, C, xv.P, xv.t.device, dtype=self.dt)
        arg = torch.empty(N * OH * OW, C, dtype=torch.uint8, device=xv.t.device) if self.tape is not None else None
        ops.maxpool_fwd(xv.t, out, N, H, W, C, argmax=arg)
        xv.uses += 1
        yv = Var(out, C, relu=False, gP=xv.gP)
        if self.tape is not None:
            def bwd():
                g = yv.take_grad()
                if g is None:
                    return
                dx = ops.alloc_pt(xv.rows, C, xv.gP, xv.t.device, dtype=self.dt)
                ops.maxpool_bwd(xv.t, g, dx, N, H, W, C, argmax=arg)
                xv.add_grad(dx, masked=False)
            self.tape.append(bwd)
        return yv, OH, OW

    def upsample(self, xv, N, IH, IW, OH, OW, P=None):
        C = xv.C
        out = ops.alloc_pt(N * OH * OW, C, xv.P if P is None else P, xv.t.device, dtype=self.dt)
        ops.bilinear_fwd(xv.t, out, N, IH, IW, OH, OW, C)
        xv.uses += 1
        yv = Var(out, C, relu=False, gP=min(out.P, self.pg))
        if self.tape is not None:
            def bwd():
                g = yv.take_grad()
                if g is None:
                    return
                dx = ops.alloc_pt(xv.rows, C, xv.gP, xv.t.device, dtype=self.dt)
                ops.bilinear_bwd(g, dx, N, IH, IW, OH, OW, C)
                xv.add_grad(dx, masked=False)
            self.tape.append(bwd)
        return yv

    def concat(self, buf, parts):
        cv = Var(buf, buf.shape[1], relu=all(p.relu for p in parts), gP=max(p.gP for p in parts))
        for p in parts:
            p.uses += 1
        if self.tape is not None:
            def bwd():
                g = cv.take_grad()
                if g is None:
                    return
                c = 0
                for p in parts:
                    p.add_grad(g.cols(c, c + p.C), masked=cv.relu)
                    c += p.C
            self.tape.append(bwd)
        return cv

    def bottleneck(self, xv, p, N, H, W, inplanes, planes, stride, has_ds, out=None):
        a, _, _ = self.conv_bn(xv, self.spec(p + ".conv1", inplanes, planes, 1, bias=False), p + ".bn1", N, H, W, True)
        b, OH, OW = self.conv_bn(a, self.spec(p + ".conv2", planes, planes, 3, stride, 1, bias=False), p + ".bn2", N, H, W, True)
        if has_ds:
            idt, _, _ = self.conv_bn(xv, self.spec(p + ".downsample.0", inplanes, planes * 4, 1, stride, 0, bias=False), p + ".downsample.1", N, H, W, False)
        else:
            idt = xv
        y, _, _ = self.conv_bn(b, self.spec(p + ".conv3", planes, planes * 4, 1, bias=False), p + ".bn3", N, OH, OW, True, res=idt, out=out)
        return y, OH, OW

    def _phase(self, label):
        if self.phase_hook is not None:
            self.phase_marks.append((label, len(self.tape) if self.tape is not None else 0))
            self.phase_hook("fwd", label)

    def forward_dec(self, img, record):
        N, _, H, W = img.shape
        dev = img.device
        if record and self.raw_kp_logits:
            raise RuntimeError("raw_kp_logits is an inference-only test hook (the losses expect probabilities)")
        ops.launch_held_packs()
        self.tape = [] if record else None
        self.generation += 1
        self.param_grads = {}
        self.nbt = []
        self.stats_written = False
        if record:
            self.train_steps += 1
            if self.grad_store is not None:
                self.grad_store.begin_step()
        self.stamp = ("t" if record else "e", self.train_steps, ops.PARAM_EPOCH[0])
        pre, self.prepack_state = self.prepack_state, None
        self.m._seg.prepack_stamp = None
        self.fast_stamp = None
        if record and pre is not None and pre["epoch"] == ops.PARAM_EPOCH[0]:
            self.stamp = pre["stamp"]
            self.m._seg.prepack_stamp = pre["stamp"]
            if pre.get("fp") == self.fingerprint():
                self.fast_stamp = pre["stamp"]
        self.m._seg.fast_stamp = self.fast_stamp
        if self.fast_stamp is None:
            self.prepare_all(record)
        self.bpt = self.pt if (self.m.training or not self.eval_downgrade) else min(self.pt, max(self.pd, 1))
        pt, pd = self.bpt, self.pd
        self.phase_marks = []
        self._phase("c0_conv")
        x8 = Var(ops.img_pack(img, max(pt, pd), dtype=self.dt), 8, relu=False, req=False)
        dims = [(H, W)]
        cat0 = ops.alloc_pt(N * H * W, 128, pd, dev, dtype=self.dt)
        c0a, _, _ = self.conv(x8, self.spec("c0_conv.0", 3, 64, 3, 1, 1, P=pd), N, H, W, True)
        c0, _, _ = self.conv(c0a, self.spec("c0_conv.2", 64, 64, 3, 1, 1, P=pd), N, H, W, True, out=cat0.cols(64, 128))
        self._phase("stem")
        H1, W1 = (H + 6 - 7) // 2 + 1, (W + 6 - 7) // 2 + 1
        cat1 = ops.alloc_pt(N * H1 * W1, 128, pt, dev, dtype=self.dt)
        c1, _, _ = self.conv_bn(x8, self.spec("conv1", 3, 64, 7, 2, 3, bias=False), "bn1", N, H, W, True, out=cat1.cols(64, 128), bn_stats=False)
        f, Hc, Wc = self.maxpool(c1, N, H1, W1)
        dims.append((H1, W1))
        feats = [c0, c1]
        cats = [cat0, cat1]
        for li, (name, inplanes, planes, blocks, stride) in enumerate(self.m.layers_tab):
            self._phase(name)
            for b in range(blocks):
                st = stride if b == 0 else 1
                Ho, Wo = (Hc - 1) // st + 1, (Wc - 1) // st + 1
                out = None
                if b == blocks - 1 and li < 2:
                    catb = ops.alloc_pt(N * Ho * Wo, planes * 8, pt, dev, dtype=self.dt)
                    cats.append(catb)
                    out = catb.cols(planes * 4, planes * 8)
                f, Hc, Wc = self.bottleneck(f, f"{name}.{b}", N, Hc, Wc, inplanes if b == 0 else planes * 4, planes, st, b == 0, out=out)
                f.boundary = True
            feats.append(f)
            dims.append((Hc, Wc))
        self._phase("decoder")
        cur = feats[4]
        catv = {}
        up_ch = {3: (1024, 512), 2: (512, 256), 1: (256, 64), 0: (64, 64)}
        for lvl in (3, 2, 1, 0):
            (IH, IW), (OH, OW) = dims[lvl + 1], dims[lvl]
            cin, cu = up_ch[lvl]
            u_in = self.upsample(cur, N, IH, IW, OH, OW, P=pd)
            buf = cats[lvl]
            u, _, _ = self.conv(u_in, self.spec(f"c{lvl + 1}_up_conv.0", cin, cu, 3, 1, 1, P=pd), N, OH, OW, True, out=buf.cols(0, cu), oP=buf.P)
            cv = self.concat(buf, [u, feats[lvl]])
            cur, _, _ = self.conv(cv, self.spec(f"c{lvl}_cat_refine.0", buf.shape[1], cu, 1, P=pd), N, OH, OW, True)
            cur.boundary = lvl > 0
            catv[lvl] = cur
        maps = []
        self.head_slots = []
        for lvl in range(4):
            self._phase(f"heads_c{lvl}")
            C = arch.HEAD_CH[lvl]
            Hh, Wh = dims[lvl]
            fused = [f"{h}_head_c{lvl}.0" for h, _ in arch.HEADS]
            hid, _, _ = self.conv(catv[lvl], self.spec(f"heads_c{lvl}.0", C, C, 7, 1, 3, fused=fused, P=self.ph), N, Hh, Wh, True)
            if self.keep_head_hidden:
                self.head_hidden[lvl] = hid.t
            outs = self.heads_second(hid, lvl, C, N, Hh, Wh)
            maps.extend(outs)
        self._phase("end")
        if self.nbt:
            torch._foreach_add_(self.nbt, 1)
            self.nbt = []
        if self.stats_written:
            ops.PARAM_EPOCH[0] += 1
        self.feats, self.dims, self.N, self.maps = feats, dims, N, maps
        for fv in feats:
            fv.uses += 1 << 20
        feats[1].boundary = True
        return maps, feats, dims

    HEAD_OFF = (0, 8, 24)
    HEAD_PAD = (8, 16, 40)

    def heads2_tables(self, dev):
        t = getattr(self, "_heads2", None)
        if t is None or t["vmap"].device != dev:
            rows, vmap = ops.heads2_layout()
            vm = torch.tensor(vmap, dtype=torch.int32)
            t = {"rows": [torch.tensor(r, dtype=torch.int32, device=dev) for r in rows], "vmap": vm.to(dev),
                 "bias_idx": torch.where(vm < 0, torch.full_like(vm, 55), vm).long().to(dev),
                 "zero1": torch.zeros(1, dtype=torch.float32, device=dev)}
            self._heads2 = t
        return t

    def prepare_heads2(self, lvl, C, dev, train):
        self.heads2_seen[lvl] = (C, dev)
        key = f"heads_c{lvl}.2F"
        ent = self.fusedT.get(key)
        if self.fast_stamp is not None and ent is not None and ent[0][:3] == self.fast_stamp and ent[1].buf.device == dev:
            entT = self.fusedT.get(f"heads_c{lvl}.2T") if train else None
            if not train or (entT is not None and entT[0][:3] == self.fast_stamp and entT[1].buf.device == dev):
                return ent[1], ent[2], (entT[1], entT[2]) if train else None
        ph = self.ph
        specs = [self.spec(f"{h}_head_c{lvl}.2", C, co, 7, 1, 3, P=ph) for h, co in arch.HEADS]
        ws = [self.P(s.names[0] + ".weight") for s in specs]
        bs = [self.P(s.names[0] + ".bias") for s in specs]
        ver = self.stamp + tuple(t._version for t in ws + bs) + tuple(t.data_ptr() for t in ws + bs)
        if ent is None or ent[0] != ver or ent[1].buf.device != dev:
            lay = self.heads2_tables(dev)
            pwF = ent[1] if ent is not None and ent[1].buf.device == dev else PackedWeight(64, 49, C, dev, xP=ph, wP=ph, groups=3, dtype=self.dt)
            for k, w in enumerate(ws):
                pwF.pack_rows(w.detach(), lay["rows"][k], group=k)
            bias64 = torch.cat([b.detach() for b in bs] + [lay["zero1"]])[lay["bias_idx"]]
            self.fusedT[key] = (ver, pwF, bias64)
        _, pwF, bias64 = self.fusedT[key]
        pwT = None
        if train:
            key = f"heads_c{lvl}.2T"
            ent = self.fusedT.get(key)
            ver = self.stamp + tuple(w._version for w in ws) + tuple(w.data_ptr() for w in ws)
            if ent is None or ent[0] != ver or ent[1].buf.device != dev:
                gph = min(ph, self.pg)
                reuse = ent is not None and ent[1].buf.device == dev
                pwT = ent[1] if reuse else PackedWeight(3 * C, 49, 64, dev, xP=gph, wP=min(gph, self.pdw), dtype=self.dt)
                narrow = NARROW_HEADS_DGRAD and gph == 1 and min(gph, self.pdw) == 1
                pwN = None
                if narrow:
                    pwN = ent[2] if reuse and ent[2] is not None else (PackedWeight(C, 7, 64, dev, dtype=self.dt), PackedWeight(C, 14, 64, dev, dtype=self.dt))
                    pwN[0].pack_narrow(ws[0].detach(), 8)
                    pwN[1].pack_narrow(ws[1].detach(), 16)
                for k, w in enumerate(ws):
                    if narrow and k < 2:
                        continue
                    pwT.pack(w.detach(), row0=k * C, c0=self.HEAD_OFF[k], transposed=True)
                self.fusedT[key] = (ver, pwT, pwN)
            pwT = (self.fusedT[key][1], self.fusedT[key][2])
        return pwF, bias64, pwT

    def heads_second(self, hid, lvl, C, N, H, W):
        dev = hid.t.device
        train = self.tape is not None
        specs = [self.spec(f"{h}_head_c{lvl}.2", C, co, 7, 1, 3, P=self.ph) for h, co in arch.HEADS]
        pwF, bias64, pwTN = self.prepare_heads2(lvl, C, dev, train)
        pwT, pwN = pwTN if pwTN is not None else (None, None)
        outs = [torch.empty(N, co, H, W, dtype=torch.float32, device=dev) for _, co in arch.HEADS]
        ops.conv_halo_heads2(hid.t, pwF, bias64, self.heads2_tables(dev)["vmap"], outs[0], outs[1], outs[2], N, H, W, C,
                             kp_sigmoid=not self.raw_kp_logits)
        if self.keep_kp_logits:
            side = [torch.empty_like(o) for o in outs]
            ops.conv_halo_heads2(hid.t, pwF, bias64, self.heads2_tables(dev)["vmap"], side[0], side[1], side[2], N, H, W, C, kp_sigmoid=False)
            self.kp_logits[lvl] = side[0]
        slot = {"grad": None}
        self.head_slots.append((slot, lvl, N, H, W))
        if train:
            geom = (N * H * W, H, W, H, W, 7, 7, 1, 3)

            def bwd():
                g = slot["grad"]
                if g is None:
                    return
                for k, ((h, co), s) in enumerate(zip(arch.HEADS, specs)):
                    gk = g.cols(self.HEAD_OFF[k], self.HEAD_OFF[k] + self.HEAD_PAD[k])
                    w = self.P(s.names[0] + ".weight")
                    gw = self.new_grad(s.names[0] + ".weight", w)
                    db = self.new_grad(s.names[0] + ".bias", self.P(s.names[0] + ".bias"))
                    ops.conv_wgrad(trunc(hid.t, min(hid.gP, self.pw)).cols(k * C, (k + 1) * C), trunc(gk, self.pw), C, co, geom, [(gw, 0, co)], N=N, bias_out=db)
                    self.param_grads[s.names[0] + ".weight"] = gw
                    self.param_grads[s.names[0] + ".bias"] = db
                dh = ops.alloc_pt(hid.rows, 3 * C, hid.gP, dev, dtype=self.dt)
                if pwN is not None and g.P == 1 and NARROW_HEADS_DGRAD >= 2 and dh.P == 1:
                    ops.conv7_narrow(g, pwN[0], C, N, H, W, dh.cols(0, C), mask=hid.t.hi()[:, :C], chan_lo=0, chan_slot=8, algo_cin=5)
                    ops.conv7_narrow(g, pwN[1], C, N, H, W, dh.cols(C, 2 * C), mask=hid.t.hi()[:, C:2 * C], chan_lo=8, chan_slot=16, algo_cin=10)
                elif pwN is not None and g.P == 1:
                    ops.conv_halo(g, pwN[0], C, N, H, W, 7, y=dh.cols(0, C), mask=hid.t.hi()[:, :C], flip=True, narrow=8, algo_cin=5)
                    ops.conv_halo(g, pwN[1], C, N, H, W, 7, y=dh.cols(C, 2 * C), mask=hid.t.hi()[:, C:2 * C], flip=True, narrow=16, algo_cin=10)
                else:
                    ops.conv_halo(g, pwT, 2 * C, N, H, W, 7, y=dh.cols(0, 2 * C), mask=hid.t.hi()[:, :2 * C], flip=True, k1skip=True, algo_cin=7.5)
                ops.conv_halo(g, pwT.rows_from(2 * C), C, N, H, W, 7, y=dh.cols(2 * C, 3 * C), mask=hid.t.hi()[:, 2 * C:], flip=True, algo_cin=40)
                hid.add_grad(dh, masked=True)
            self.tape.append(bwd)
        return outs

    def export_feats(self):
        outs = []
        for fv, (h, w) in zip(self.feats, self.dims):
            o = torch.empty(fv.rows, fv.C, dtype=torch.float32, device=fv.t.device)
            ops.planes_to_f32(fv.t, fv.C, o)
            outs.append(o.view(self.N, h, w, fv.C).permute(0, 3, 1, 2))
        return outs

    def backward_dec(self, map_grads, feat_grads, gscale=None):
        if gscale is not None:
            self.gscale = gscale
            Var.ENG = self
        gsc = self.gscale[0:1] if self.gscale is not None else None
        if self.grad_store is not None:
            self.grad_store.dense_backward_started()
        for (slot, lvl, N, Hh, Wh) in self.head_slots:
            gs = map_grads[3 * lvl:3 * lvl + 3]
            if all(g is None for g in gs):
                continue
            dev = self.maps[3 * lvl].device
            packed = ops.alloc_pt(N * Hh * Wh, 64, min(self.ph, self.pg), dev, dtype=self.dt)
            if all(g is not None for g in gs) and self.HEAD_OFF == (0, 8, 24) and sum(self.HEAD_PAD) == 64:
                ops.grad_pack3([g.contiguous().float() for g in gs], self.maps[3 * lvl], packed, N, [co for _, co in arch.HEADS], Hh, Wh, self.HEAD_PAD, scale=gsc)
                slot["grad"] = packed
                continue
            for k, g in enumerate(gs):
                co = arch.HEADS[k][1]
                view = packed.cols(self.HEAD_OFF[k], self.HEAD_OFF[k] + self.HEAD_PAD[k])
                if g is None:
                    for p in range(view.P):
                        view.plane(p).zero_()
                else:
                    prob = self.maps[3 * lvl] if k == 0 else None
                    ops.grad_pack(g.contiguous().float(), prob, view, N, co, Hh, Wh, self.HEAD_PAD[k], scale=gsc)
            slot["grad"] = packed
        for fv, g in zip(self.feats, feat_grads):
            if g is None:
                continue
            if isinstance(g, PT):
                fv.add_grad(g, masked=False)
                continue
            gp = ops.alloc_pt(fv.rows, fv.C, fv.gP, g.device, dtype=self.dt)
            ops.f32_to_planes(g, gp, fv.C, scale=gsc)
            fv.add_grad(gp, masked=False)
        hook = self.grad_hook
        tape, self.tape = self.tape, None
        ops.WGQ.begin()
        try:
            marks = list(self.phase_marks) if self.phase_hook is not None else None
            while tape:
                if marks is not None:
                    while marks and marks[-1][1] >= len(tape):
                        marks.pop()
                    if marks and marks[-1][0] != getattr(self, "_bwd_phase", None):
                        self._bwd_phase = marks[-1][0]
                        self.phase_hook("bwd", self._bwd_phase)
                fn = tape.pop()
                n0 = len(self.param_grads)
                fn()
                del fn
                if hook is not None and len(self.param_grads) > n0:
                    hook(list(self.param_grads.items())[n0:], False)
            if hook is not None:
                hook([], True)
            if marks is not None:
                self._bwd_phase = None
                self.phase_hook("bwd", "end")
        except BaseException:
            self.gscale, self.param_gsc = None, {}
            if self.grad_store is not None:
                self.grad_store.unscale_of = None
            raise
        finally:
            Var.ENG = None
            ops.WGQ.end()
        grads = self.param_grads
        self.param_grads = {}
        return grads
```

### kg_instance_segmentation_amd/ops.py

```python
import functools
import math
import os

import torch

from . import _lib
from ._lib import c_int, c_long, c_float, c_double, ptr, stream_ptr

BF16 = torch.bfloat16
F16 = torch.float16
_scratch = {}
PARAM_EPOCH = [0]


def scratch_f32(nfloats, dev, tag="default"):
    key = (str(dev), tag)
    t = _scratch.get(key)
    if t is None or t.numel() < nfloats:
        t = torch.empty(max(int(nfloats), 1 << 16), dtype=torch.float32, device=dev)
        _scratch[key] = t
    return t


class WgradReduceQueue:
# ... 294 lines not shown
        assert w.dtype == torch.float32 and w.is_contiguous() and rowmap.dtype == torch.int32 and rowmap.numel() == Cout
        c0 = group * self.vp * self.cin_pad
        if PACKQ.defer:
            (PACKQ16 if fmt_of(self) else PACKQ).add(w, self, 0, c0, False, rowmap, self.tap_stride)
            return
        _lib.call("kg_pack_weight_rows", ptr(w), ptr(self.buf), Cout, Cin, KH, KW, self.K, self.cin_pad, ptr(rowmap), c0,
                  self.xP, self.wP, self.tap_stride, stream_ptr(), fmt=fmt_of(self))


def heads2_layout():
    grp = [[16 * q + 4 * i + r for q in range(4) for r in range(4)] for i in range(4)]
    rows = [grp[0][:5], grp[1][:10], grp[2] + grp[3] + grp[0][5:13]]
    vmap = [-1] * 64
    base = (0, 5, 15)
    for h in range(3):
        for c, v in enumerate(rows[h]):
            vmap[v] = base[h] + c
    return rows, vmap


def conv_halo_heads2(x, pw, bias64, vmap, kp, sh, md, N, H, W, C, kp_sigmoid=True):
    flush_packs()
    assert kp.is_contiguous() and sh.is_contiguous() and md.is_contiguous() and vmap.dtype == torch.int32
    assert nplanes(x)[0] == pw.xP and pw.groups == 3
    _lib.call("kg_conv2d_halo_heads2", ptr(_rows(x)), ptr(pw.buf), ptr(bias64), ptr(vmap), ptr(kp), ptr(sh), ptr(md), N, H, W, C,
              ld(x), pw.K, 1 if kp_sigmoid else 0, pl(a=x, w=pw.wP), stream_ptr(), fmt=fmt_of(x))


def conv_igemm(x, pw, cout, geom, y=None, y_f32=None, bias=None, res=None, mask=None, relu=False, mode=0,
               rowdesc=None, tile=0, oscale=None):
    flush_packs()
    M, H, W, OH, OW, KH, KW, stride, pad = geom
    assert nplanes(x)[0] == pw.xP, (nplanes(x), pw.xP)
    f32_C = 0
    if y_f32 is not None:
        assert y_f32.dtype == torch.float32 and y_f32.is_contiguous()
        f32_C = y_f32.shape[1] if y_f32.dim() == 4 else 1
    _lib.call("kg_conv2d_igemm", ptr(_rows(x)), ptr(pw.buf), ptr(bias), ptr(base(y)), ptr(y_f32), ptr(base(res)), ptr(base(mask)), ptr(rowdesc),
              M, H, W, OH, OW, pw.cin_pad, ld(x), cout, ld(y) if y is not None else 0,
              ld(res) if res is not None else 0, ld(mask) if mask is not None else 0, pw.K, KH, KW, stride, pad, 1,
              mode, 1 if relu else 0, f32_C, tile, pl(a=x, b=res, y=y, w=pw.wP, oscale=oscale), stream_ptr(), fmt=fmt_of(x))


def conv7_narrow(x, pw, cout, N, H, W, y, mask=None, chan_lo=0, chan_slot=8, flip=True, algo_cin=None):
    flush_packs()
    assert nplanes(x)[0] == 1 and nplanes(y)[0] == 1 and pw.xP == pw.wP == 1 and chan_slot in (8, 16)
    xb, yb, mb = _rows(x), base(y), base(mask)
    _lib.call("kg_conv7_narrow", ptr(xb), ptr(pw.buf), ptr(yb), ptr(mb), N, H, W, ld(xb), chan_lo, chan_slot, cout, ld(yb),
              ld(mb) if mb is not None else 0, pw.K, 1 if flip else 0, stream_ptr(), fmt=fmt_of(xb))


USE_HALO = True
WGRAD128 = True
USE_C3 = True
IM2COL_WGRAD = True


HALO_WC = 0


USE_WS = True


def conv_halo(x, pw, cout, N, H, W, KS, y=None, y_f32=None, bias=None, res=None, mask=None, relu=False, flip=False, wc=0,
              tiletab=None, total_rows=0, k1skip=False, algo_cin=None, tiletab16=None, oscale=None, tiletab8=None, narrow=0):
    flush_packs()
    assert nplanes(x)[0] == pw.xP, (nplanes(x), pw.xP)
    if (USE_WS and KS == 3 and pw.cin_pad == 64 and cout == 64 and pw.xP == 2 and pw.wP == 2 and y is not None and y_f32 is None and res is None
            and mask is None and not flip and oscale is None and wc == 0 and HALO_WC == 0 and (tiletab is None or tiletab8 is not None)
            and nplanes(y)[0] <= 2 and not conv_stats_armed()):
        _lib.call("kg_conv3x3_ws", ptr(_rows(x)), ptr(pw.buf), ptr(bias), ptr(base(y)), N, H, W, ld(x), ld(y), pw.K, 1 if relu else 0,
                  ptr(tiletab8), tiletab8.shape[0] if tiletab8 is not None else 0, pl(a=x, y=y, w=pw.wP), stream_ptr(), fmt=fmt_of(x))
        return
    planes = pl(a=x, b=res, y=y, w=pw.wP, oscale=oscale)
    x, y, res, mask = base(x), base(y), base(res), base(mask)
    if (USE_C3 and planes is None and KS == 3 and pw.cin_pad == 64 and y is not None and y_f32 is None and wc == 0 and HALO_WC == 0
            and (tiletab is None or tiletab16 is not None)):
        flush_packs()
        _lib.call("kg_conv3x3_c64", ptr(_rows(x)), ptr(pw.buf), ptr(bias), ptr(y), ptr(res), ptr(mask), N, H, W, ld(x), cout, ld(y),
                  ld(res) if res is not None else 0, ld(mask) if mask is not None else 0, pw.K, 1 if flip else 0, 1 if relu else 0,
                  ptr(tiletab16), tiletab16.shape[0] if tiletab16 is not None else 0, stream_ptr(), fmt=fmt_of(x))
        return
    wc = wc or HALO_WC
    if k1skip:
        assert KS == 7 and wc in (0, 1)
        wc = 1 | 256
    if narrow:
        assert KS == 7 and wc in (0, 1) and flip and narrow in (8, 16) and planes is None and tiletab is None and y is not None and y_f32 is None
        wc = 1 | (512 if narrow == 8 else 1024)
    f32_C = 0
    if y_f32 is not None:
        f32_C = y_f32.shape[1] if y_f32.dim() == 4 else 1
    _lib.call("kg_conv2d_halo", ptr(_rows(x)), ptr(pw.buf), ptr(bias), ptr(y), ptr(y_f32), ptr(res), ptr(mask), N, H, W,
              pw.cin_pad, ld(x), cout, ld(y) if y is not None else 0, ld(res) if res is not None else 0,
              ld(mask) if mask is not None else 0, pw.K, KS, 1 if flip else 0, 1 if relu else 0, f32_C, wc, ptr(tiletab),
              tiletab.shape[0] if tiletab is not None else 0, total_rows, planes, stream_ptr(), fmt=fmt_of(x))


USE_1X1 = True
GATHER_1X1 = True


def conv1x1(x, pw, cout, y, bias=None, res=None, mask=None, relu=False):
    flush_packs()
    assert pw.vp == 1 and all(nplanes(t)[0] == 1 for t in (x, y, res))
    x, y, res, mask = base(x), base(y), base(res), base(mask)
    _lib.call("kg_conv1x1", ptr(_rows(x)), ptr(pw.buf), ptr(bias), ptr(_rows(y)), ptr(res), ptr(mask), c_long(x.shape[0]),
              pw.cin_pad, pw.K, ld(x), cout, ld(y), ld(res) if res is not None else 0, ld(mask) if mask is not None else 0,
              1 if relu else 0, stream_ptr(), fmt=fmt_of(x))


def can_1x1(x, pw, KH, stride, pad, y, y_f32, res=None):
    if pw.vp > 1 or any(nplanes(t)[0] > 1 for t in (x, y, res)):
        return False
    if GATHER_1X1 and pw.cin_pad >= 192 and pw.rows > 64:
        return False
    return (USE_1X1 and KH == 1 and stride == 1 and pad == 0 and y is not None and y_f32 is None and pw.cin_pad % 64 == 0
            and 64 <= pw.cin_pad <= 1024 and x.shape[1] >= pw.cin_pad and y.shape[0] == x.shape[0])


CONV_TINY_WGS = 96
CONV_TINY_TILES = 384


def conv_auto(x, pw, cout, geom, N, y=None, y_f32=None, bias=None, res=None, mask=None, relu=False, transposed=False, tile=0, oscale=None,
              tiny=True):
    M, H, W, OH, OW, KH, KW, stride, pad = geom
    halo_ok = (USE_HALO and stride == 1 and KH == KW and KH in (3, 7) and pad == KH // 2 and pw.cin_pad % 64 == 0
               and x.shape[1] >= pw.cin_pad and not (y_f32 is not None and (res is not None or mask is not None)))
    if tiny and tile == 0 and CONV_TINY_WGS and y is not None and y_f32 is None and pw.cin_pad % 64 == 0 and x.shape[1] >= pw.cin_pad and KH * KW <= 9:
        wgs = (N * math.ceil(OH / 16) * math.ceil(OW / 32) * math.ceil(cout / 64)) if halo_ok else math.ceil(M / 256) * math.ceil(cout / 128)
        tiles = math.ceil(M / 64) * math.ceil(cout / 64)
        if wgs < CONV_TINY_WGS and wgs < tiles <= CONV_TINY_TILES:
            conv_igemm(x, pw, cout, geom, y=y, bias=bias, res=res, mask=mask, relu=relu, mode=1 if transposed else 0, tile=6, oscale=oscale)
            return "tiny"
    if (USE_HALO and stride == 1 and KH == KW and KH in (3, 7) and pad == KH // 2 and pw.cin_pad % 64 == 0
            and x.shape[1] >= pw.cin_pad and not (y_f32 is not None and (res is not None or mask is not None))):
        conv_halo(x, pw, cout, N, OH, OW, KH, y=y, y_f32=y_f32, bias=bias, res=res, mask=mask, relu=relu, flip=transposed, oscale=oscale)
        return "halo"
    if KH == KW and oscale is None and can_1x1(x, pw, KH, stride, pad, y, y_f32, res):
        conv1x1(x, pw, cout, y, bias=bias, res=res, mask=mask, relu=relu)
        return "1x1"
    conv_igemm(x, pw, cout, geom, y=y, y_f32=y_f32, bias=bias, res=res, mask=mask, relu=relu, mode=1 if transposed else 0, tile=tile, oscale=oscale)
    return "igemm"


WGRAD_RING = True
WGRAD_RING_WGS = 256


WGRAD_TR = [True]


def set_wgrad_tr(on):
    WGRAD_TR[0] = bool(on)
    for fmt in (0, 1):
        _lib.call("kg_set_wgrad_tr", 1 if on else 0, fmt=fmt)


def wgrad_splits(M, cin_lim, cout_lim, taps, nelem):
    chunks = math.ceil(M / 64)
    if WGRAD_RING and WGRAD_TR[0] and cin_lim >= 128 and cout_lim >= 64:
        base = math.ceil(cin_lim / 128) * math.ceil(cout_lim / (256 if cout_lim >= 256 else 128)) * taps
        s = max(1, min(WGRAD_RING_WGS // base if base <= WGRAD_RING_WGS else 1, max(1, chunks // 3)))
        while s > 1 and s * nelem * 4 > (768 << 20):
            s -= 1
        return s
    t = 128 if (WGRAD128 and WGRAD_TR[0] and cin_lim >= 128 and cout_lim >= 128) else 64
    base = math.ceil(cin_lim / t) * math.ceil(cout_lim / t) * taps
    s = max(1, min(math.ceil(2048 / base), max(1, chunks // 4)))
    while s > 1 and s * nelem * 4 > (768 << 20):
        s -= 1
    return s


@functools.lru_cache(maxsize=4096)
def halo_wgrad_splits(nblk, tiles, cit, taps, nelem, cus=256):
    tile_us = 256 * 64 * cit * taps * 2 / 5.3e6
    best, best_t = 1, None
    for S in range(1, max(1, min(tiles, 2048 // nblk if nblk <= 2048 else 1)) + 1):
        if S > 1 and S * nelem * 4 > (768 << 20):
            break
        rounds = math.ceil(nblk * S / cus)
        t = rounds * (math.ceil(tiles / S) * tile_us + 10.0) + S * nelem * 8 / 3e6
        if S >= 8 and S % 8 == 0:
            t *= 0.97
        if best_t is None or t < best_t:
            best, best_t = S, t
    return best


def wgrad_pairs(x, dy):
    xP, dP = nplanes(x)[0], nplanes(dy)[0]
    T = max(xP, dP)
    return sorted(((i, j) for j in range(dP) for i in range(xP) if i + j < T), key=lambda p: -(p[0] + p[1]))


def conv_wgrad(x, dy, cin, cout, geom, grads, mode=0, rowdesc=None, accumulate=False, N=None, tiletab16=None, bias_out=None):
    M, H, W, OH, OW, KH, KW, stride, pad = geom
    pairs = wgrad_pairs(x, dy)
    xps, dps = nplanes(x)[1], nplanes(dy)[1]
    planed = len(pairs) > 1 or nplanes(x)[0] > 1 or nplanes(dy)[0] > 1
    xb, dyb = _rows(x), _rows(dy)
    if IM2COL_WGRAD and mode == 0 and N is not None and cin <= 4 and KH * KW >= 25 and len(grads) == 1 and not accumulate:
        Kc = KH * KW * cin
        Kpad = round_up(Kc, 8)
        xP = nplanes(x)[0]
        col = alloc_pt(M, Kpad, xP, xb.device, zero=Kpad != Kc, dtype=xb.dtype)
        for p_ in range(xP):
            _lib.call("kg_im2col_small", ctypes_offset(xb, p_ * xps), ctypes_offset(col.t, p_ * col.ps), N, H, W, OH, OW, KH, KW, stride, pad, cin,
                      ld(xb), ld(col), stream_ptr(), fmt=fmt_of(xb))
        g, off, cnt = grads[0]
        tmp = torch.empty(cout, Kc, 1, 1, dtype=torch.float32, device=xb.device)
        conv_wgrad(col if xP > 1 else col.t, dy, Kc, cout, (M, OH, OW, OH, OW, 1, 1, 1, 0), [(tmp, off, cnt)])
        flush_wgrad()
        g.copy_(tmp.view(cnt, KH * KW, cin).permute(0, 2, 1).reshape(g.shape))
        if bias_out is not None:
            bias_grad(dy, cout, bias_out)
        return "im2col"
    cin_lim = min(round_up(cin, 8), xb.shape[1])
    cout_lim = min(round_up(cout, 8), dyb.shape[1])
    nelem = cout * KH * KW * cin
    halo = (USE_HALO and stride == 1 and KH == KW and KH in (3, 7) and pad == KH // 2
            and ((mode == 0 and N is not None) or (mode == 2 and tiletab16 is not None)))
    np_ = len(pairs)
    planes = pl(a=x, b=dy)
    if halo:
        cit = (32 if (cout_lim <= 16 and cin_lim >= 32 and bias_out is not None and not planed) else 16) if KH == 7 else 64
        nblk = math.ceil(cin_lim / cit) * math.ceil(cout_lim / 64)
        tiles = tiletab16.shape[0] if tiletab16 is not None else N * math.ceil(H / 16) * math.ceil(W / 16)
        S = halo_wgrad_splits(nblk, tiles * np_, cit, KH * KW, nelem)
        fused_bias = bias_out is not None and not planed
        part, big = WGQ.alloc(S * nelem, xb.device, "wgrad", extra=S * cout if fused_bias else 0)
        dbp = None
        if fused_bias:
            dbp, big2 = WGQ.alloc(S * cout, xb.device, "wgrad_bias")
            big = big or big2
        _lib.call("kg_conv2d_wgrad_halo", ptr(xb), ptr(dyb), ptr(part), N or 0, H, W, ld(xb), ld(dyb), cin, cout, cin_lim, cout_lim, KH, S,
                  c_long(nelem), ptr(tiletab16), tiletab16.shape[0] if tiletab16 is not None else 0, ptr(dbp), planes, stream_ptr(), fmt=fmt_of(x))
        if dbp is None and bias_out is not None:
            bias_grad(dy, cout, bias_out, accumulate=accumulate)
    else:
        dbp = None
        S = wgrad_splits(M * np_, cin_lim, cout_lim, KH * KW, nelem)
        part, big = WGQ.alloc(S * nelem, xb.device, "wgrad")
        _lib.call("kg_conv2d_wgrad", ptr(xb), ptr(dyb), ptr(part), ptr(rowdesc), M, H, W, OH, OW, ld(xb), ld(dyb), cin, cout, cin_lim, cout_lim,
                  KH, KW, stride, pad, 1, mode, S, c_long(nelem), planes, stream_ptr(), fmt=fmt_of(xb))
        if bias_out is not None:
            bias_grad(dy, cout, bias_out, accumulate=accumulate)
    contiguous = all(grads[i][1] + grads[i][2] == grads[i + 1][1] for i in range(len(grads) - 1))
    import ctypes
    acc = 1 if accumulate else 0
    if len(grads) <= 4 and contiguous:
        gp = (ctypes.c_void_p * len(grads))(*[g.data_ptr() for g, _, _ in grads])
        cn = (ctypes.c_int * len(grads))(*[cnt for _, _, cnt in grads])
        _lib.call("kg_wgrad_reduce_bias", ctypes_offset(part, grads[0][1] * KH * KW * cin), gp, cn, len(grads), cin, KH, KW, S,
                  c_long(nelem), acc, ptr(dbp), ptr(bias_out) if dbp is not None else None, cout if dbp is not None else 0, stream_ptr())
    else:
        if dbp is not None:
            _lib.call("kg_bias_grad_final", ptr(dbp), ptr(bias_out), S, cout, acc, stream_ptr())
        for g, off, cnt in grads:
            _lib.call("kg_wgrad_reduce", ctypes_offset(part, off * KH * KW * cin), ptr(g), cnt, cin, KH, KW, S, c_long(nelem), acc, stream_ptr())
    if big:
        WGQ.flush()
    return "halo" if halo else "gather"


def wgrad_halo(x, dy, part, N, H, W, cin, cout, cin_lim, cout_lim, KS, S, nelem, tiletab16=None, dbp=None):
    _lib.call("kg_conv2d_wgrad_halo", ptr(x), ptr(dy), ptr(part), N, H, W, ld(x), ld(dy), cin, cout, cin_lim, cout_lim, KS, S,
              c_long(nelem), ptr(tiletab16), tiletab16.shape[0] if tiletab16 is not None else 0, ptr(dbp), None, stream_ptr(), fmt=fmt_of(x))


def ctypes_offset(t, elem_off):
    return _lib.c_void_p(t.data_ptr() + elem_off * t.element_size())


def bias_grad(dy, C, db, accumulate=False):
    P, ps = nplanes(dy)
    dyb = _rows(dy)
    sc = scratch_f32(2048 * max(C, 1), dyb.device, "bias")
    for p in range(P):
        _lib.call("kg_bias_grad", ctypes_offset(dyb, p * ps), ptr(db), ptr(sc), sc.numel(), dyb.shape[0], C, ld(dyb),
                  1 if (accumulate or p > 0) else 0, stream_ptr(), fmt=fmt_of(dyb))


def img_pack(img, P=1, dtype=BF16):
    N, C, H, W = img.shape
    img = img.contiguous().float()
    out = alloc_pt(N * H * W, 8, P, img.device, dtype=dtype)
    _lib.call("kg_img_pack", ptr(img), ptr(out.t), ld(out), N, C, H, W, pl(y=out), stream_ptr(), fmt=fmt_of(out))
    return out if P > 1 else out.t


def bn_stats_train(x, C, gamma, beta, rmean, rvar, momentum=0.1, eps=1e-5):
    xb = _rows(x)
    dev = xb.device
    st = torch.empty(4, C, dtype=torch.float32, device=dev)
    sc = scratch_f32(2 * C * 512, dev, "bn")
    _lib.call("kg_bn_stats_train", ptr(xb), ld(xb), xb.shape[0], C, ptr(gamma), ptr(beta), ptr(rmean), ptr(rvar),
              c_float(momentum), c_float(eps), ptr(st[0]), ptr(st[1]), ptr(st[2]), ptr(st[3]), ptr(sc), sc.numel(), pl(a=x), stream_ptr(), fmt=fmt_of(xb))
    return st[0], st[1], st[2], st[3]


CONV_BN_STATS = True


_STATS_ARMED = [False]


def conv_stats_armed():
    return _STATS_ARMED[0]


def conv_stats_begin(dev, fmt=0):
    part = scratch_f32(1 << 21, dev, "bnpart")
    _lib.call("kg_conv_stats_begin", ptr(part), c_long(part.numel()), fmt=fmt)
    _STATS_ARMED[0] = True
    return part


def conv_bstats_begin(x, mean, invstd, M, C, N=1):
    xb = _rows(x)
    P, ps = nplanes(x)
    tiles = 4 * math.ceil(M / 256) + 4 * N + 8
    part = torch.empty(tiles * C * 2, dtype=torch.float32, device=xb.device)
    _lib.call("kg_conv_bstats_begin", ptr(part), c_long(part.numel()), ptr(xb), ld(x), P, ps, ptr(mean), ptr(invstd), fmt=fmt_of(x))
    _STATS_ARMED[0] = True
    return part


def conv_stats_end(fmt=0):
    import ctypes
    nb = ctypes.c_int(0)
    _STATS_ARMED[0] = False
    _lib.call("kg_conv_stats_end", ctypes.byref(nb), fmt=fmt)
    return nb.value


def bn_finalize_train(part, nb, M, C, gamma, beta, rmean, rvar, momentum=0.1, eps=1e-5):
    st = torch.empty(4, C, dtype=torch.float32, device=part.device)
    _lib.call("kg_bn_finalize_train", ptr(part), nb, M, C, ptr(gamma), ptr(beta), ptr(rmean), ptr(rvar), c_float(momentum), c_float(eps),
              ptr(st[0]), ptr(st[1]), ptr(st[2]), ptr(st[3]), stream_ptr())
    return st[0], st[1], st[2], st[3]


def bn_scale_shift_eval(C, gamma, beta, rmean, rvar, eps=1e-5):
    st = torch.empty(2, C, dtype=torch.float32, device=gamma.device)
    _lib.call("kg_bn_scale_shift_eval", C, ptr(gamma), ptr(beta), ptr(rmean), ptr(rvar), c_float(eps), ptr(st[0]), ptr(st[1]), stream_ptr())
    return st[0], st[1]


def bn_apply(x, C, scale, shift, y, res=None, relu=False):
    _lib.call("kg_bn_apply", ptr(_rows(x)), ld(x), ptr(scale), ptr(shift), ptr(base(res)), ld(res) if res is not None else 0, ptr(_rows(y)), ld(y),
              base(x).shape[0], C, 1 if relu else 0, pl(a=x, b=res, y=y), stream_ptr(), fmt=fmt_of(x))


def bn_bwd(x, dy, C, gamma, mean, invstd, dgamma, dbeta, dx, accumulate=False, parts=None, parts_scale=None):
    sc = scratch_f32(2 * C * 512 + 3 * C, base(x).device, "bn")
    pt, nbp = parts if parts is not None else (None, 0)
    _lib.call("kg_bn_bwd", ptr(_rows(x)), ld(x), ptr(_rows(dy)), ld(dy), ptr(gamma), ptr(mean), ptr(invstd), ptr(dgamma), ptr(dbeta),
              1 if accumulate else 0, ptr(_rows(dx)), ld(dx), base(x).shape[0], C, ptr(sc), sc.numel(), ptr(pt), nbp, ptr(parts_scale),
              pl(a=x, b=dy, y=dx), stream_ptr(), fmt=fmt_of(x))


def maxpool_fwd(x, y, N, H, W, C, argmax=None):
    _lib.call("kg_maxpool3s2_fwd", ptr(_rows(x)), ld(x), ptr(_rows(y)), ld(y), ptr(argmax), N, H, W, C, pl(a=x, y=y), stream_ptr(), fmt=fmt_of(x))


def maxpool_bwd(x, dy, dx, N, H, W, C, argmax=None):
    _lib.call("kg_maxpool3s2_bwd", ptr(_rows(x)), ld(x), ptr(_rows(dy)), ld(dy), ptr(_rows(dx)), ld(dx), ptr(argmax), N, H, W, C,
              pl(a=x, b=dy, y=dx), stream_ptr(), fmt=fmt_of(dy))


def bilinear_fwd(x, y, N, IH, IW, OH, OW, C, boxdesc=None, row2box=None):
    rows = base(y).shape[0] if boxdesc is not None else 0
    _lib.call("kg_bilinear_fwd", ptr(_rows(x)), ld(x), ptr(_rows(y)), ld(y), N, IH, IW, OH, OW, C, ptr(boxdesc), ptr(row2box),
              c_long(rows), pl(a=x, y=y), stream_ptr(), fmt=fmt_of(x))


def bilinear_bwd(dy, dx, N, IH, IW, OH, OW, C, boxdesc=None, row2box=None, mask=None):
    rows = base(dx).shape[0] if boxdesc is not None else 0
    _lib.call("kg_bilinear_bwd", ptr(_rows(dy)), ld(dy), ptr(_rows(dx)), ld(dx), N, IH, IW, OH, OW, C, ptr(boxdesc), ptr(row2box),
              c_long(rows), ptr(base(mask)), ld(mask) if mask is not None else 0, pl(a=dy, y=dx), stream_ptr(), fmt=fmt_of(dy))


def add_rows(a, b, y, C, mask=None, scale=None):
    r, r2 = scale if scale is not None else (None, None)
    _lib.call("kg_add_rows", ptr(_rows(a)), ld(a), ptr(base(b)), ld(b) if b is not None else 0, ptr(base(mask)),
              ld(mask) if mask is not None else 0, ptr(_rows(y)), ld(y), c_long(base(a).shape[0]), C, ptr(r), ptr(r2), pl(a=a, b=b, y=y), stream_ptr(),
              fmt=fmt_of(a))


def planes_to_f32(x, C, out):
    _lib.call("kg_planes_to_f32", ptr(_rows(x)), ld(x), ptr(out), out.stride(0), c_long(base(x).shape[0]), C, pl(a=x), stream_ptr(), fmt=fmt_of(x))


def f32_to_planes(acc, y, C, addto=None, scale=None):
    _lib.call("kg_f32_to_planes", ptr(acc), acc.stride(0), ptr(_rows(y)), ld(y), ptr(base(addto)), ld(addto) if addto is not None else 0,
              c_long(acc.shape[0]), C, pl(b=addto, y=y, scale=scale), stream_ptr(), fmt=fmt_of(y))


def sigmoid_(x):
    _lib.call("kg_sigmoid_inplace", ptr(x), c_long(x.numel()), stream_ptr())
    return x


def grad_pack(g, prob, out, N, C, H, W, cpad, scale=None):
    _lib.call("kg_grad_pack", ptr(g), ptr(prob), ptr(_rows(out)), N, C, H, W, ld(out), cpad, pl(y=out, scale=scale), stream_ptr(), fmt=fmt_of(out))


def grad_pack3(gs, prob0, out, N, Cs, H, W, pads, scale=None):
    _lib.call("kg_grad_pack3", ptr(gs[0]), ptr(gs[1]), ptr(gs[2]), ptr(prob0), ptr(_rows(out)), N, Cs[0], Cs[1], Cs[2], H, W, ld(out),
              pads[0], pads[1], pads[2], pl(y=out, scale=scale), stream_ptr(), fmt=fmt_of(out))


GRAD_TARGET_LOG2 = int(__import__("os").environ.get("KG_GRAD_TARGET_LOG2", "4"))
_gs_state = {}


def grad_scale(tensors, probs=None):
    import ctypes
    probs = probs or [None] * len(tensors)
    pairs = [(t, q) for t, q in zip(tensors, probs) if t is not None and t.numel() > 0]
    ts = [t for t, _ in pairs]
    qs = [q for _, q in pairs]
    assert 1 <= len(ts) <= 24 and all(t.dtype == torch.float32 and t.is_contiguous() for t in ts)
    assert all(q is None or (q.dtype == torch.float32 and q.is_contiguous() and q.numel() == t.numel()) for t, q in pairs)
    dev = ts[0].device
    scr = _gs_state.get(str(dev))
    if scr is None:
        scr = torch.zeros(2, dtype=torch.int32, device=dev)
        _gs_state[str(dev)] = scr
    out = torch.empty(2, dtype=torch.float32, device=dev)
    ptrs = (ctypes.c_void_p * len(ts))(*[t.data_ptr() for t in ts])
    prbs = (ctypes.c_void_p * len(ts))(*[q.data_ptr() if q is not None else None for q in qs])
    cnts = (ctypes.c_long * len(ts))(*[t.numel() for t in ts])
    _lib.call("kg_grad_scale", ptrs, prbs, cnts, len(ts), GRAD_TARGET_LOG2, ptr(scr), ptr(out), stream_ptr())
    return out


def scale_tensors(tensors, scale, flag=None):
    import numpy as np
    flush_wgrad()
    scales = scale if isinstance(scale, (list, tuple)) else [scale] * len(tensors)
    pairs = [(t, sc) for t, sc in zip(tensors, scales) if t is not None and t.numel() > 0]
    if not pairs:
        return
    dt = np.dtype([("p", "<u8"), ("n", "<i8"), ("scale", "<u8"), ("blk0", "<i4"), ("pad", "<i4")])
    arr = np.zeros(len(pairs), dt)
    blk = 0
    for i, (t, sc) in enumerate(pairs):
        assert t.dtype == torch.float32 and t.is_contiguous() and sc.dtype == torch.float32
        arr[i] = (t.data_ptr(), t.numel(), sc.data_ptr(), blk, 0)
        blk += (t.numel() + 4095) // 4096
    tab = h2d(arr.view(np.uint8).reshape(-1), pairs[0][0].device)
    _lib.call("kg_scale_tensors", ptr(tab), len(pairs), blk, ptr(flag), stream_ptr())


def rows_rescale(g, C, cum_in, target_log2=None):
    dev = base(g).device
    scr = _gs_state.get(str(dev))
    if scr is None:
        scr = torch.zeros(2, dtype=torch.int32, device=dev)
        _gs_state[str(dev)] = scr
    out = torch.empty(3, dtype=torch.float32, device=dev)
    _lib.call("kg_rows_rescale", ptr(_rows(g)), ld(g), c_long(base(g).shape[0]), C, GRAD_TARGET_LOG2 if target_log2 is None else target_log2,
              ptr(cum_in), ptr(out[0:2]), ptr(out[2:3]), ptr(scr), pl(a=g), stream_ptr(), fmt=fmt_of(g))
    return out[2:3], out[0:2]


def rows_scale_multi(items, r, r2=None):
    import ctypes
    items = [(g, C) for g, C in items if base(g).shape[0] > 0]
    for i in range(0, len(items), 8):
        chunk = items[i:i + 8]
        desc = (ctypes.c_long * (6 * len(chunk)))()
        for k, (g, C) in enumerate(chunk):
            P, ps = nplanes(g)
            desc[6 * k:6 * k + 6] = [_rows(g).data_ptr(), ld(g), base(g).shape[0], C, P, ps]
        _lib.call("kg_rows_scale_multi", desc, len(chunk), ptr(r), ptr(r2), stream_ptr(), fmt=fmt_of(chunk[0][0]))


def rows_scale(g, C, r, r2=None):
    _lib.call("kg_rows_scale", ptr(_rows(g)), ld(g), c_long(base(g).shape[0]), C, ptr(r), ptr(r2), pl(a=g), stream_ptr(), fmt=fmt_of(g))
```

Before: 129.1 imgs/s.

## Fuse reduction finalize into partial-sum kernels via last-block-arrives counters

Replaces the separate single-block finalize launches after the BN stats, BN backward, detection-loss and seg-loss reductions with an in-kernel last-arriver pattern. Blocks publish partials with agent-scope atomics, bump a per-launch counter drawn from a per-stream arena, and the last block computes the final statistics. The arena is memset once per forward or backward pass. This removes one kernel launch and its dependency bubble per reduction, at the cost of atomics, fences and a serialized tail inside the last block.

Result: no change. 129.0 imgs/s (-0.1%).

```diff
diff --git a/include/kgnet_hip.h b/include/kgnet_hip.h
--- a/include/kgnet_hip.h
+++ b/include/kgnet_hip.h
@@ -20,6 +20,9 @@
 const char* kg_last_error(void);
 const char* kg_last_kernel(void);
 int kg_version(void);
+int kg_fused_finalize_begin(void);
+int kg_set_fused_finalize(int on);
+long kg_fused_finalize_launches(void);
 int kg_device_arch(char* out, int cap);
 int kg_tr_probe(void* out_u16x256, void* stream);
 int kg_f64_probe(const double* a, const double* b, double* out5n, int n, void* stream);
diff --git a/kg_instance_segmentation_amd/_lib.py b/kg_instance_segmentation_amd/_lib.py
--- a/kg_instance_segmentation_amd/_lib.py
+++ b/kg_instance_segmentation_amd/_lib.py
@@ -11,6 +11,9 @@
 _SIGS = {
     "kg_version": [],
     "kg_rows_format": [],
+    "kg_fused_finalize_begin": [],
+    "kg_set_fused_finalize": [c_int],
+    "kg_fused_finalize_launches": [],
     "kg_grad_scale": [P, P, P, c_int, c_int, P, P, P],
     "kg_scale_tensors": [P, c_int, c_int, P, P],
     "kg_rows_rescale": [P, c_int, c_long, c_int, c_int, P, P, P, P, P, P],
@@ -104,7 +107,7 @@
     "kg_crop_grad_reduce": [P, c_int, P, c_int, c_long, P, P, P, c_int, c_int, c_int, c_int, c_int, P, P, c_int, P, P],
 }
 _RESTYPE = {"kg_postproc_workspace_bytes": c_long, "kg_postproc_batch_workspace_bytes": c_long, "kg_nms_batch_workspace_bytes": c_long,
-            "kg_mask_bits_ld": c_long}
+            "kg_mask_bits_ld": c_long, "kg_fused_finalize_launches": c_long}
 SYMBOLS = tuple(_SIGS) + ("kg_last_error", "kg_last_kernel")
 
 _lib = None
diff --git a/kg_instance_segmentation_amd/csrc/api.hip b/kg_instance_segmentation_amd/csrc/api.hip
--- a/kg_instance_segmentation_amd/csrc/api.hip
+++ b/kg_instance_segmentation_amd/csrc/api.hip
@@ -62,6 +62,54 @@
     g_conv_stats = KgConvStats{nullptr, 0, 0, {nullptr, 0, 0, 0, nullptr, nullptr}};
     return KG_OK;
 }
+
+#include <stdlib.h>
+namespace {
+constexpr int KG_FIN_ARENA = 4096;
+constexpr int KG_FIN_SLOTS = 8;
+struct FinArena { int dev; hipStream_t st; unsigned* base; int used; bool dirty; };
+thread_local FinArena g_fin[KG_FIN_SLOTS] = {};
+thread_local int g_fin_n = 0;
+thread_local long g_fin_launches = 0;
+int g_fin_switch = -1;
+}
+static int fin_enabled() {
+    static const int env = getenv("KG_FUSED_FINALIZE") ? atoi(getenv("KG_FUSED_FINALIZE")) : 1;
+    return g_fin_switch >= 0 ? g_fin_switch : env;
+}
+unsigned* kg_fin_counters(int n, hipStream_t st) {
+    if (!fin_enabled() || n < 1 || n > KG_FIN_ARENA) return nullptr;
+    int dev = 0;
+    if (hipGetDevice(&dev) != hipSuccess) return nullptr;
+    FinArena* a = nullptr;
+    for (int i = 0; i < g_fin_n; ++i)
+        if (g_fin[i].dev == dev && g_fin[i].st == st) a = &g_fin[i];
+    if (!a) {
+        if (g_fin_n == KG_FIN_SLOTS) return nullptr;
+        unsigned* p = nullptr;
+        if (hipMalloc((void**)&p, KG_FIN_ARENA * sizeof(unsigned)) != hipSuccess) { (void)hipGetLastError(); return nullptr; }
+        a = &g_fin[g_fin_n++];
+        *a = FinArena{dev, st, p, 0, true};
+    }
+    if (a->dirty || a->used + n > KG_FIN_ARENA) {
+        if (hipMemsetAsync(a->base, 0, KG_FIN_ARENA * sizeof(unsigned), st) != hipSuccess) { (void)hipGetLastError(); return nullptr; }
+        a->used = 0; a->dirty = false;
+    }
+    unsigned* c = a->base + a->used;
+    a->used += n;
+    ++g_fin_launches;
+    return c;
+}
+extern "C" int kg_fused_finalize_begin(void) {
+    for (int i = 0; i < g_fin_n; ++i)
+        if (g_fin[i].used > 0) g_fin[i].dirty = true;
+    return KG_OK;
+}
+extern "C" int kg_set_fused_finalize(int on) {
+    g_fin_switch = on < 0 ? -1 : (on ? 1 : 0);
+    return KG_OK;
+}
+extern "C" long kg_fused_finalize_launches(void) { return g_fin_launches; }
 
 extern "C" int kg_host_tile_table(const int* h, const int* w, const long* row0, int nb, int th, int tw, int* out, int cap) {
     if (!h || !w || !row0 || !out || nb < 0 || th < 1 || tw < 1) return -1;
diff --git a/kg_instance_segmentation_amd/csrc/kg_common.h b/kg_instance_segmentation_amd/csrc/kg_common.h
--- a/kg_instance_segmentation_amd/csrc/kg_common.h
+++ b/kg_instance_segmentation_amd/csrc/kg_common.h
@@ -127,6 +127,27 @@
     return st.part;
 }
 
+__device__ __forceinline__ void kg_publish_f32(float* p, float v) {
+    __hip_atomic_store((__attribute__((address_space(1))) float*)p, v, __ATOMIC_RELAXED, __HIP_MEMORY_SCOPE_AGENT);
+}
+__device__ __forceinline__ bool kg_last_arriver(unsigned* counter, unsigned expected, unsigned* lds_word) {
+    asm volatile("s_waitcnt vmcnt(0)" ::: "memory");
+    __syncthreads();
+    if (threadIdx.x == 0) {
+        const unsigned ticket = __hip_atomic_fetch_add((__attribute__((address_space(1))) unsigned*)counter, 1u, __ATOMIC_RELAXED, __HIP_MEMORY_SCOPE_AGENT);
+        const bool last = ticket == expected - 1u;
+        if (last) {
+            __builtin_amdgcn_fence(__ATOMIC_ACQUIRE, "agent");
+            asm volatile("s_waitcnt vmcnt(0)" ::: "memory");
+        }
+        *lds_word = last ? 1u : 0u;
+    }
+    __syncthreads();
+    return *lds_word != 0u;
+}
+unsigned* kg_fin_counters(int n, hipStream_t st);
+#define KG_FIN_MAX_BYTES (64 << 10)
+
 struct kg_planes_t {
     int a_planes, a_pstride;
     int b_planes, b_pstride;
diff --git a/kg_instance_segmentation_amd/csrc/loss.hip b/kg_instance_segmentation_amd/csrc/loss.hip
--- a/kg_instance_segmentation_amd/csrc/loss.hip
+++ b/kg_instance_segmentation_amd/csrc/loss.hip
@@ -19,54 +19,17 @@
     return (p - t) / d;
 }
 
-__global__ __launch_bounds__(256) void det_loss_fwd_kernel(const float* __restrict__ kp, const float* __restrict__ sh,
-                                                           const float* __restrict__ md, const float* __restrict__ gt,
-                                                           int N, long HW, float inv_r, float* __restrict__ part) {
-    float s[5] = {0.f, 0.f, 0.f, 0.f, 0.f};
-    const long total = (long)N * HW;
-    for (long i = blockIdx.x * (long)blockDim.x + threadIdx.x; i < total; i += (long)gridDim.x * blockDim.x) {
-        long n = i / HW, p = i - n * HW;
-        const float* g = gt + n * 55 * HW + p;
-        float gk[5];
-#pragma unroll
-        for (int c = 0; c < 5; ++c) {
-            gk[c] = g[c * HW];
-            s[0] += bce_elem(kp[(n * 5 + c) * HW + p], gk[c]);
-        }
-#pragma unroll
-        for (int c = 0; c < 10; ++c) {
-            float m = gk[c >> 1];
-            s[1] += fabsf(sh[(n * 10 + c) * HW + p] - g[(5 + c) * HW]) * inv_r * m;
-            s[2] += m;
-        }
-#pragma unroll
-        for (int c = 0; c < 40; ++c) {
-            float m = gk[KG_MID_FROM[c >> 1]];
-            s[3] += fabsf(md[(n * 40 + c) * HW + p] - g[(15 + c) * HW]) * inv_r * m;
-            s[4] += m;
-        }
-    }
-    __shared__ float red[4][5];
-    const int lane = threadIdx.x & 63, wave = threadIdx.x >> 6;
-#pragma unroll
-    for (int k = 0; k < 5; ++k) {
-        float v = wave_sum(s[k]);
-        if (lane == 0) red[wave][k] = v;
-    }
-    __syncthreads();
-    if (threadIdx.x < 5) part[blockIdx.x * 5 + threadIdx.x] = red[0][threadIdx.x] + red[1][threadIdx.x] + red[2][threadIdx.x] + red[3][threadIdx.x];
-}
-__global__ void det_loss_final_kernel(const float* __restrict__ part, int nb, double numel,
-                                      const float* __restrict__ den_override, float* __restrict__ out) {
-    if (blockIdx.x != 0) return;
+__device__ __forceinline__ void det_loss_final_wave(const float* part, int nb, double numel, const float* den_override, float* out, int lane) {
     double s[5] = {0, 0, 0, 0, 0};
-    for (int b = threadIdx.x; b < nb; b += 64)
+#pragma unroll 4
+    for (int b = lane; b < nb; b += 64)
+#pragma unroll
         for (int k = 0; k < 5; ++k) s[k] += (double)part[b * 5 + k];
 #pragma unroll
     for (int k = 0; k < 5; ++k)
 #pragma unroll
         for (int o = 32; o > 0; o >>= 1) s[k] += __shfl_down(s[k], o, 64);
-    if (threadIdx.x != 0) return;
+    if (lane != 0) return;
     double m2 = s[2], m4 = s[4], ne = numel;
     if (den_override) { m2 = den_override[0]; m4 = den_override[1]; ne = den_override[2]; }
     float lkp = (float)(s[0] / ne);
@@ -75,6 +38,56 @@
     out[0] = lkp + lsh + 0.25f * lmd; out[1] = lkp; out[2] = lsh; out[3] = lmd;
     out[4] = (float)(1.0 / ne); out[5] = 1.f / ((float)m2 + 1e-10f); out[6] = 1.f / ((float)m4 + 1e-10f);
     out[7] = (float)m2;
+}
+__global__ __launch_bounds__(256) void det_loss_fwd_kernel(const float* __restrict__ kp, const float* __restrict__ sh,
+                                                           const float* __restrict__ md, const float* __restrict__ gt,
+                                                           int N, long HW, float inv_r, float* part, unsigned* cnt, double numel,
+                                                           const float* __restrict__ den_override, float* out8) {
+    float s[5] = {0.f, 0.f, 0.f, 0.f, 0.f};
+    const long total = (long)N * HW;
+    for (long i = blockIdx.x * (long)blockDim.x + threadIdx.x; i < total; i += (long)gridDim.x * blockDim.x) {
+        long n = i / HW, p = i - n * HW;
+        const float* g = gt + n * 55 * HW + p;
+        float gk[5];
+#pragma unroll
+        for (int c = 0; c < 5; ++c) {
+            gk[c] = g[c * HW];
+            s[0] += bce_elem(kp[(n * 5 + c) * HW + p], gk[c]);
+        }
+#pragma unroll
+        for (int c = 0; c < 10; ++c) {
+            float m = gk[c >> 1];
+            s[1] += fabsf(sh[(n * 10 + c) * HW + p] - g[(5 + c) * HW]) * inv_r * m;
+            s[2] += m;
+        }
+#pragma unroll
+        for (int c = 0; c < 40; ++c) {
+            float m = gk[KG_MID_FROM[c >> 1]];
+            s[3] += fabsf(md[(n * 40 + c) * HW + p] - g[(15 + c) * HW]) * inv_r * m;
+            s[4] += m;
+        }
+    }
+    __shared__ float red[4][5];
+    const int lane = threadIdx.x & 63, wave = threadIdx.x >> 6;
+#pragma unroll
+    for (int k = 0; k < 5; ++k) {
+        float v = wave_sum(s[k]);
+        if (lane == 0) red[wave][k] = v;
+    }
+    __syncthreads();
+    if (threadIdx.x < 5) {
+        const float t = red[0][threadIdx.x] + red[1][threadIdx.x] + red[2][threadIdx.x] + red[3][threadIdx.x];
+        if (cnt) kg_publish_f32(&part[blockIdx.x * 5 + threadIdx.x], t);
+        else part[blockIdx.x * 5 + threadIdx.x] = t;
+    }
+    if (!cnt) return;
+    if (!kg_last_arriver(cnt, gridDim.x, reinterpret_cast<unsigned*>(&red[0][0]))) return;
+    if (threadIdx.x < 64) det_loss_final_wave(part, gridDim.x, numel, den_override, out8, threadIdx.x);
+}
+__global__ void det_loss_final_kernel(const float* __restrict__ part, int nb, double numel,
+                                      const float* __restrict__ den_override, float* __restrict__ out) {
+    if (blockIdx.x != 0) return;
+    det_loss_final_wave(part, nb, numel, den_override, out, threadIdx.x);
 }
 __global__ __launch_bounds__(256) void det_loss_bwd_kernel(const float* __restrict__ kp, const float* __restrict__ sh,
                                                            const float* __restrict__ md, const float* __restrict__ gt,
@@ -121,8 +134,10 @@
     if (nb > scratch_floats / 5) nb = scratch_floats / 5;
     KG_CHECK_ARG(nb >= 1, "kg_detection_loss_fwd: scratch too small");
     hipStream_t st = (hipStream_t)stream;
-    hipLaunchKernelGGL(det_loss_fwd_kernel, dim3(nb), dim3(256), 0, st, kp, sh, md, gt, N, (long)H * W, 1.f / kp_radius, scratch);
-    hipLaunchKernelGGL(det_loss_final_kernel, dim3(1), dim3(64), 0, st, scratch, nb, (double)total * 5.0, den_override, out8);
+    unsigned* cnt = kg_fin_counters(1, st);
+    hipLaunchKernelGGL(det_loss_fwd_kernel, dim3(nb), dim3(256), 0, st, kp, sh, md, gt, N, (long)H * W, 1.f / kp_radius, scratch, cnt,
+                       (double)total * 5.0, den_override, out8);
+    if (!cnt) hipLaunchKernelGGL(det_loss_final_kernel, dim3(1), dim3(64), 0, st, scratch, nb, (double)total * 5.0, den_override, out8);
     KG_CHECK_LAUNCH("detection_loss_fwd");
     return KG_OK;
 }
@@ -141,10 +156,18 @@
 
 struct SegPatch { int prob_off, npix, pair0, npairs; };
 struct SegPair { int tgt_off; float weight; };
+__device__ __forceinline__ void sum_final_wave(const float* part, int n, float* out, int lane) {
+    double s = 0.;
+#pragma unroll 8
+    for (int i = lane; i < n; i += 64) s += (double)part[i];
+#pragma unroll
+    for (int o = 32; o > 0; o >>= 1) s += __shfl_down(s, o, 64);
+    if (lane == 0) out[0] = (float)s;
+}
 __global__ __launch_bounds__(256) void seg_loss_kernel(const float* __restrict__ prob, const uint8_t* __restrict__ tgt,
                                                        const SegPatch* __restrict__ patches,
-                                                       const SegPair* __restrict__ pairs, float* __restrict__ part,
-                                                       const float* __restrict__ gout, float* __restrict__ gprob) {
+                                                       const SegPair* __restrict__ pairs, float* part,
+                                                       const float* __restrict__ gout, float* __restrict__ gprob, unsigned* cnt, float* out1) {
     const SegPatch pa = patches[blockIdx.x];
     const float go = gout ? gout[0] : 1.f;
     float s = 0.f;
@@ -162,23 +185,27 @@
     float v = wave_sum(s);
     if ((threadIdx.x & 63) == 0) red[threadIdx.x >> 6] = v;
     __syncthreads();
-    if (threadIdx.x == 0 && part) part[blockIdx.x] = red[0] + red[1] + red[2] + red[3];
+    if (threadIdx.x == 0 && part) {
+        const float t = red[0] + red[1] + red[2] + red[3];
+        if (cnt) kg_publish_f32(&part[blockIdx.x], t);
+        else part[blockIdx.x] = t;
+    }
+    if (!cnt) return;
+    if (!kg_last_arriver(cnt, gridDim.x, reinterpret_cast<unsigned*>(red))) return;
+    if (threadIdx.x < 64) sum_final_wave(part, gridDim.x, out1, threadIdx.x);
 }
 __global__ void sum_final_kernel(const float* __restrict__ part, int n, float* __restrict__ out) {
     if (blockIdx.x != 0) return;
-    double s = 0.;
-    for (int i = threadIdx.x; i < n; i += 64) s += (double)part[i];
-#pragma unroll
-    for (int o = 32; o > 0; o >>= 1) s += __shfl_down(s, o, 64);
-    if (threadIdx.x == 0) out[0] = (float)s;
+    sum_final_wave(part, n, out, threadIdx.x);
 }
 extern "C" int kg_seg_loss(const float* prob, const void* tgt, const int* patches, const void* pairs, int npatches,
                            float* part, float* out1, const float* grad_out, float* gprob, void* stream) {
     KG_CHECK_ARG(prob && tgt && patches && pairs && npatches > 0, "kg_seg_loss: bad args");
     hipStream_t st = (hipStream_t)stream;
+    unsigned* cnt = part && out1 && (long)npatches * sizeof(float) <= KG_FIN_MAX_BYTES ? kg_fin_counters(1, st) : nullptr;
     hipLaunchKernelGGL(seg_loss_kernel, dim3(npatches), dim3(256), 0, st, prob, (const uint8_t*)tgt,
-                       (const SegPatch*)patches, (const SegPair*)pairs, part, grad_out, gprob);
-    if (part && out1) hipLaunchKernelGGL(sum_final_kernel, dim3(1), dim3(64), 0, st, part, npatches, out1);
+                       (const SegPatch*)patches, (const SegPair*)pairs, part, grad_out, gprob, cnt, out1);
+    if (part && out1 && !cnt) hipLaunchKernelGGL(sum_final_kernel, dim3(1), dim3(64), 0, st, part, npatches, out1);
     KG_CHECK_LAUNCH("seg_loss");
     return KG_OK;
 }
diff --git a/kg_instance_segmentation_amd/csrc/norm_pool.hip b/kg_instance_segmentation_amd/csrc/norm_pool.hip
--- a/kg_instance_segmentation_amd/csrc/norm_pool.hip
+++ b/kg_instance_segmentation_amd/csrc/norm_pool.hip
@@ -28,11 +28,85 @@
     return KG_OK;
 }
 
-template <int MODE>
+__device__ __forceinline__ double wave_sum_d(double v) {
+#pragma unroll
+    for (int o = 32; o > 0; o >>= 1) v += __shfl_down(v, o, 64);
+    return __shfl(v, 0, 64);
+}
+
+struct BnFinF {
+    const float* gamma; const float* beta; float* running_mean; float* running_var; float momentum, eps;
+    float* mean_out; float* invstd_out; float* scale; float* shift;
+};
+__device__ __forceinline__ void bn_train_finish(double s, double ss, long M, int c, const BnFinF& f) {
+    double mu = s / (double)M;
+    double var = ss / (double)M - mu * mu;
+    if (var < 0.) var = 0.;
+    float is = (float)(1.0 / sqrt(var + (double)f.eps));
+    f.mean_out[c] = (float)mu; f.invstd_out[c] = is;
+    float sc = f.gamma[c] * is;
+    f.scale[c] = sc; f.shift[c] = f.beta[c] - (float)mu * sc;
+    if (f.running_mean) {
+        double unb = M > 1 ? var * (double)M / (double)(M - 1) : var;
+        f.running_mean[c] = (1.f - f.momentum) * f.running_mean[c] + f.momentum * (float)mu;
+        f.running_var[c] = (1.f - f.momentum) * f.running_var[c] + f.momentum * (float)unb;
+    }
+}
+__device__ __forceinline__ void bn_finalize_train_channel(const float* part, int nb, int C, long M, int c, int lane, const BnFinF& f) {
+    double s = 0., ss = 0.;
+    for (int b = lane; b < nb; b += 64) { s += part[((long)b * C + c) * 2]; ss += part[((long)b * C + c) * 2 + 1]; }
+    s = wave_sum_d(s); ss = wave_sum_d(ss);
+    if (lane == 0) bn_train_finish(s, ss, M, c, f);
+}
+struct BnFinB {
+    const float* gamma; const float* invstd; float* dgamma; float* dbeta; int accumulate; float* coef; const float* rs;
+};
+__device__ __forceinline__ void bn_bwd_finish(double s, double sx, int C, long M, int c, const BnFinB& f) {
+    if (f.rs) { s *= (double)*f.rs; sx *= (double)*f.rs; }
+    float db = (float)s, dg = (float)sx;
+    f.dgamma[c] = f.accumulate ? f.dgamma[c] + dg : dg;
+    f.dbeta[c] = f.accumulate ? f.dbeta[c] + db : db;
+    float a = f.gamma[c] * f.invstd[c];
+    f.coef[c] = a; f.coef[C + c] = (float)(-(double)a * sx / (double)M); f.coef[2 * C + c] = (float)(-(double)a * s / (double)M);
+}
+__device__ __forceinline__ void bn_finalize_bwd_channel(const float* part, int nb, int C, long M, int c, int lane, const BnFinB& f) {
+    double s = 0., sx = 0.;
+    for (int b = lane; b < nb; b += 64) { s += part[((long)b * C + c) * 2]; sx += part[((long)b * C + c) * 2 + 1]; }
+    s = wave_sum_d(s); sx = wave_sum_d(sx);
+    if (lane == 0) bn_bwd_finish(s, sx, C, M, c, f);
+}
+__device__ __forceinline__ void bn_partials_sum8(const float* part, int nb, int C, int c0, int lane, double& s_out, double& q_out) {
+    double s[8], q[8];
+#pragma unroll
+    for (int k = 0; k < 8; ++k) s[k] = q[k] = 0.;
+    for (int b0 = lane; b0 < nb; b0 += 128) {
+        const bool two = b0 + 64 < nb;
+        const f32x4* p0 = reinterpret_cast<const f32x4*>(part + ((long)b0 * C + c0) * 2);
+        const f32x4* p1 = reinterpret_cast<const f32x4*>(part + ((long)(two ? b0 + 64 : b0) * C + c0) * 2);
+        f32x4 v0[4], v1[4];
+#pragma unroll
+        for (int k = 0; k < 4; ++k) { v0[k] = p0[k]; v1[k] = p1[k]; }
+#pragma unroll
+        for (int k = 0; k < 8; ++k) { s[k] += (double)v0[k >> 1][(k & 1) * 2]; q[k] += (double)v0[k >> 1][(k & 1) * 2 + 1]; }
+        if (two) {
+#pragma unroll
+            for (int k = 0; k < 8; ++k) { s[k] += (double)v1[k >> 1][(k & 1) * 2]; q[k] += (double)v1[k >> 1][(k & 1) * 2 + 1]; }
+        }
+    }
+    s_out = q_out = 0.;
+#pragma unroll
+    for (int k = 0; k < 8; ++k) {
+        const double a = wave_sum_d(s[k]), b = wave_sum_d(q[k]);
+        if (lane == k) { s_out = a; q_out = b; }
+    }
+}
+
+template <int MODE, bool FIN>
 __global__ __launch_bounds__(256) void colreduce_kernel(const RowsR x, const RowsR dy,
                                                         const float* __restrict__ mean,
-                                                        const float* __restrict__ invstd, float* __restrict__ part,
-                                                        int M, int C, int rows_per_block) {
+                                                        const float* __restrict__ invstd, float* part,
+                                                        int M, int C, int rows_per_block, unsigned* cnt,
+                                                        const BnFinF ff, const BnFinB fb) {
     __shared__ float red[32][8][16];
     const int cl = threadIdx.x & 7, rl = threadIdx.x >> 3;
     const int c0 = blockIdx.y * 64 + cl * 8;
@@ -72,39 +146,27 @@
         float t = 0.f;
         for (int k = 0; k < 32; ++k) t += red[k][c >> 3][q * 8 + (c & 7)];
         const int cg = blockIdx.y * 64 + c;
-        if (cg < C) part[((long)blockIdx.x * C + cg) * 2 + q] = t;
-    }
-}
-
-__device__ __forceinline__ double wave_sum_d(double v) {
-#pragma unroll
-    for (int o = 32; o > 0; o >>= 1) v += __shfl_down(v, o, 64);
-    return __shfl(v, 0, 64);
-}
-
-__global__ void bn_finalize_train_kernel(const float* __restrict__ part, int nb, int C, long M,
-                                         const float* __restrict__ gamma, const float* __restrict__ beta,
-                                         float* __restrict__ running_mean, float* __restrict__ running_var,
-                                         float momentum, float eps, float* __restrict__ mean_out,
-                                         float* __restrict__ invstd_out, float* __restrict__ scale,
-                                         float* __restrict__ shift) {
-    const int c = blockIdx.x;
-    double s = 0., ss = 0.;
-    for (int b = threadIdx.x; b < nb; b += 64) { s += part[((long)b * C + c) * 2]; ss += part[((long)b * C + c) * 2 + 1]; }
-    s = wave_sum_d(s); ss = wave_sum_d(ss);
-    if (threadIdx.x != 0) return;
-    double mu = s / (double)M;
-    double var = ss / (double)M - mu * mu;
-    if (var < 0.) var = 0.;
-    float is = (float)(1.0 / sqrt(var + (double)eps));
-    mean_out[c] = (float)mu; invstd_out[c] = is;
-    float sc = gamma[c] * is;
-    scale[c] = sc; shift[c] = beta[c] - (float)mu * sc;
-    if (running_mean) {
-        double unb = M > 1 ? var * (double)M / (double)(M - 1) : var;
-        running_mean[c] = (1.f - momentum) * running_mean[c] + momentum * (float)mu;
-        running_var[c] = (1.f - momentum) * running_var[c] + momentum * (float)unb;
-    }
+        if (cg < C) {
+            if (FIN) kg_publish_f32(&part[((long)blockIdx.x * C + cg) * 2 + q], t);
+            else part[((long)blockIdx.x * C + cg) * 2 + q] = t;
+        }
+    }
+    if (!FIN) return;
+    if (!kg_last_arriver(cnt + blockIdx.y, gridDim.x, reinterpret_cast<unsigned*>(&red[0][0][0]))) return;
+    const int lane = threadIdx.x & 63;
+    for (int g = threadIdx.x >> 6; g < 8; g += 4) {
+        const int cg = blockIdx.y * 64 + g * 8;
+        if (cg >= C) break;
+        double s, q;
+        bn_partials_sum8(part, gridDim.x, C, cg, lane, s, q);
+        if (lane < 8) {
+            if (MODE == 0) bn_train_finish(s, q, (long)M, cg + lane, ff);
+            else bn_bwd_finish(s, q, C, (long)M, cg + lane, fb);
+        }
+    }
+}
+__global__ void bn_finalize_train_kernel(const float* __restrict__ part, int nb, int C, long M, const BnFinF f) {
+    bn_finalize_train_channel(part, nb, C, M, blockIdx.x, threadIdx.x, f);
 }
 __global__ void bn_finalize_eval_kernel(int C, const float* __restrict__ gamma, const float* __restrict__ beta,
                                         const float* __restrict__ running_mean,
@@ -116,23 +178,13 @@
     float sc = gamma[c] * is;
     scale[c] = sc; shift[c] = beta[c] - running_mean[c] * sc;
 }
-__global__ void bn_finalize_bwd_kernel(const float* __restrict__ part, int nb, int C, long M,
-                                       const float* __restrict__ gamma, const float* __restrict__ invstd,
-                                       float* __restrict__ dgamma, float* __restrict__ dbeta, int accumulate,
-                                       float* __restrict__ coef, const float* __restrict__ rs) {
-    const int c = blockIdx.x;
-    double s = 0., sx = 0.;
-    for (int b = threadIdx.x; b < nb; b += 64) { s += part[((long)b * C + c) * 2]; sx += part[((long)b * C + c) * 2 + 1]; }
-    s = wave_sum_d(s); sx = wave_sum_d(sx);
-    if (threadIdx.x != 0) return;
-    if (rs) { s *= (double)*rs; sx *= (double)*rs; }
-    float db = (float)s, dg = (float)sx;
-    dgamma[c] = accumulate ? dgamma[c] + dg : dg;
-    dbeta[c] = accumulate ? dbeta[c] + db : db;
-    float a = gamma[c] * invstd[c];
-    coef[c] = a; coef[C + c] = (float)(-(double)a * sx / (double)M); coef[2 * C + c] = (float)(-(double)a * s / (double)M);
-}
-
+__global__ void bn_finalize_bwd_kernel(const float* __restrict__ part, int nb, int C, long M, const BnFinB f) {
+    bn_finalize_bwd_channel(part, nb, C, M, blockIdx.x, threadIdx.x, f);
+}
+
+static bool colreduce_fin_ok(int nb, const float* part) {
+    return (long)nb * 64 * 2 * sizeof(float) <= KG_FIN_MAX_BYTES && (reinterpret_cast<uintptr_t>(part) & 15) == 0;
+}
 static int reduce_geometry(int M, int C, int scratch_floats, int* nb, int* rpb) {
     int n = scratch_floats / (2 * C);
     if (n > 512) n = 512;
@@ -154,10 +206,17 @@
     int nb, rpb;
     KG_CHECK_ARG(reduce_geometry(M, C, scratch_floats, &nb, &rpb), "kg_bn_stats_train: scratch too small");
     hipStream_t st = (hipStream_t)stream;
-    hipLaunchKernelGGL(colreduce_kernel<0>, dim3(nb, (C + 63) / 64), dim3(256), 0, st, RowsR{(const bf16_t*)x, ldx, pp.a_planes, pp.a_pstride},
-                       RowsR{nullptr, 0, 1, 0}, (const float*)nullptr, (const float*)nullptr, scratch, M, C, rpb);
-    hipLaunchKernelGGL(bn_finalize_train_kernel, dim3(C), dim3(64), 0, st, scratch, nb, C, (long)M, gamma,
-                       beta, running_mean, running_var, momentum, eps, mean_out, invstd_out, scale, shift);
+    const BnFinF ff{gamma, beta, running_mean, running_var, momentum, eps, mean_out, invstd_out, scale, shift};
+    const RowsR xr{(const bf16_t*)x, ldx, pp.a_planes, pp.a_pstride}, none{nullptr, 0, 1, 0};
+    unsigned* cnt = colreduce_fin_ok(nb, scratch) ? kg_fin_counters((C + 63) / 64, st) : nullptr;
+    if (cnt) {
+        hipLaunchKernelGGL((colreduce_kernel<0, true>), dim3(nb, (C + 63) / 64), dim3(256), 0, st, xr, none, (const float*)nullptr, (const float*)nullptr,
+                           scratch, M, C, rpb, cnt, ff, BnFinB{});
+    } else {
+        hipLaunchKernelGGL((colreduce_kernel<0, false>), dim3(nb, (C + 63) / 64), dim3(256), 0, st, xr, none, (const float*)nullptr, (const float*)nullptr,
+                           scratch, M, C, rpb, cnt, ff, BnFinB{});
+        hipLaunchKernelGGL(bn_finalize_train_kernel, dim3(C), dim3(64), 0, st, scratch, nb, C, (long)M, ff);
+    }
     KG_CHECK_LAUNCH("bn_stats_train");
     return KG_OK;
 }
@@ -165,8 +224,8 @@
                                     float* running_var, float momentum, float eps, float* mean_out, float* invstd_out, float* scale,
                                     float* shift, void* stream) {
     KG_CHECK_ARG(part && gamma && beta && mean_out && invstd_out && scale && shift && nb >= 1 && M >= 1 && C >= 1, "kg_bn_finalize_train: bad arguments");
-    hipLaunchKernelGGL(bn_finalize_train_kernel, dim3(C), dim3(64), 0, (hipStream_t)stream, part, nb, C, (long)M, gamma, beta, running_mean,
-                       running_var, momentum, eps, mean_out, invstd_out, scale, shift);
+    hipLaunchKernelGGL(bn_finalize_train_kernel, dim3(C), dim3(64), 0, (hipStream_t)stream, part, nb, C, (long)M,
+                       BnFinF{gamma, beta, running_mean, running_var, momentum, eps, mean_out, invstd_out, scale, shift});
     KG_CHECK_LAUNCH("bn_finalize_train");
     return KG_OK;
 }
@@ -245,14 +304,19 @@
     float* coef = scratch;
     if (parts && nb_parts > 0) {
         KG_CHECK_ARG(scratch_floats >= 3 * C, "kg_bn_bwd: scratch too small");
-        hipLaunchKernelGGL(bn_finalize_bwd_kernel, dim3(C), dim3(64), 0, st, parts, nb_parts, C, (long)M, gamma, invstd, dgamma, dbeta, accumulate, coef,
-                           parts_scale);
+        hipLaunchKernelGGL(bn_finalize_bwd_kernel, dim3(C), dim3(64), 0, st, parts, nb_parts, C, (long)M,
+                           BnFinB{gamma, invstd, dgamma, dbeta, accumulate, coef, parts_scale});
     } else {
         KG_CHECK_ARG(reduce_geometry(M, C, scratch_floats - 3 * C, &nb, &rpb), "kg_bn_bwd: scratch too small");
         float* part = scratch + 3 * C;
-        hipLaunchKernelGGL(colreduce_kernel<1>, dim3(nb, (C + 63) / 64), dim3(256), 0, st, xr, dyr, mean, invstd, part, M, C, rpb);
-        hipLaunchKernelGGL(bn_finalize_bwd_kernel, dim3(C), dim3(64), 0, st, part, nb, C, (long)M, gamma,
-                           invstd, dgamma, dbeta, accumulate, coef, (const float*)nullptr);
+        const BnFinB fb{gamma, invstd, dgamma, dbeta, accumulate, coef, nullptr};
+        unsigned* cnt = colreduce_fin_ok(nb, part) ? kg_fin_counters((C + 63) / 64, st) : nullptr;
+        if (cnt) {
+            hipLaunchKernelGGL((colreduce_kernel<1, true>), dim3(nb, (C + 63) / 64), dim3(256), 0, st, xr, dyr, mean, invstd, part, M, C, rpb, cnt, BnFinF{}, fb);
+        } else {
+            hipLaunchKernelGGL((colreduce_kernel<1, false>), dim3(nb, (C + 63) / 64), dim3(256), 0, st, xr, dyr, mean, invstd, part, M, C, rpb, cnt, BnFinF{}, fb);
+            hipLaunchKernelGGL(bn_finalize_bwd_kernel, dim3(C), dim3(64), 0, st, part, nb, C, (long)M, fb);
+        }
     }
     long total = (long)M * (C / 8);
     int blocks = (int)((total + 255) / 256); if (blocks > 16384) blocks = 16384;
diff --git a/kg_instance_segmentation_amd/engine.py b/kg_instance_segmentation_amd/engine.py
--- a/kg_instance_segmentation_amd/engine.py
+++ b/kg_instance_segmentation_amd/engine.py
@@ -516,6 +516,7 @@
         if record and self.raw_kp_logits:
             raise RuntimeError("raw_kp_logits is an inference-only test hook (the losses expect probabilities)")
         ops.launch_held_packs()
+        ops.fused_finalize_begin()
         self.tape = [] if record else None
         self.generation += 1
         self.param_grads = {}
@@ -717,6 +718,7 @@
         return outs
 
     def backward_dec(self, map_grads, feat_grads, gscale=None):
+        ops.fused_finalize_begin()
         if gscale is not None:
             self.gscale = gscale
             Var.ENG = self
diff --git a/kg_instance_segmentation_amd/ops.py b/kg_instance_segmentation_amd/ops.py
--- a/kg_instance_segmentation_amd/ops.py
+++ b/kg_instance_segmentation_amd/ops.py
@@ -620,6 +620,12 @@
     return st[0], st[1], st[2], st[3]
 
 
+def fused_finalize_begin():
+    _lib.call("kg_fused_finalize_begin")
+    if _lib._lib_f16 is not None:
+        _lib.call("kg_fused_finalize_begin", fmt=1)
+
+
 CONV_BN_STATS = True
 
 
```
